# ScottHCL/recommend

Measured on AMD Instinct MI355X. Metric: ranked samples/sec (fwd+bwd) at B=4096 seq=128; AUC parity vs ref, higher is better.
Workload: dtype f32-emulated (fp16-pair / split-bf16); 1 GPU; C2: OneTrans 4L d128 H4 f512 L_NS12 L_S128 (seq 3x42), Criteo-shape 13 dense + 26 ids, replicated tables, fwd+bwd+optimizer; global_batch=4096, per_gpu_batch=4096, seq_len=128, parallelism=dp1

## Files before the change

### include/onetrans_hip.h

```cpp
#ifndef ONETRANS_HIP_H
#define ONETRANS_HIP_H

#include <stddef.h>
#include <stdint.h>

#ifdef __cplusplus
extern "C" {
#endif

#define OT_OK 0
#define OT_ERR_INVALID_ARG 1
#define OT_ERR_UNSUPPORTED 2
#define OT_ERR_HIP 3

#define OT_GEMM_NN 0
#define OT_GEMM_NT 1

#define OT_AX_NONE 0
#define OT_AX_RMSNORM 1
#define OT_AX_GELU 2
#define OT_AX_BF16 4
#define OT_AX_BF16_RMSNORM 5

#define OT_EPI_BIAS 1
#define OT_EPI_GELU_BWD 2
#define OT_EPI_GELU 4
#define OT_EPI_DROPOUT 8
#define OT_EPI_RESIDUAL 16
#define OT_EPI_ACCUMULATE 32
#define OT_EPI_ROW_RSTD 64
#define OT_EPI_ROWDOT 256
#define OT_EPI_RMSNORM_BWD 128
#define OT_EPI_C_BF16 512
#define OT_EPI_AUX_BF16 1024
#define OT_WG_D_BF16 8

int ot_version(void);
const char* ot_get_last_error_string(void);

int ot_gemm_tile_rows(void);
#define OT_MATMUL_F32 0
#define OT_MATMUL_SPLIT_BF16 1
#define OT_MATMUL_BF16 2
int ot_mixed_gemm(int mode, const float* A, int64_t lda, int K, const int32_t* in_rows,
                  int a_xform, const float* a_rstd, const float* a_gamma,
                  const float* W, int64_t w_gstride, int64_t ldw, int N,
                  const int32_t* tile_group, int ntiles,
                  const float* bias, int64_t bias_gstride,
                  float* C, int64_t ldc, const int32_t* out_rows, int epi,
                  const float* res, int64_t ldres, int res_tok,
                  const float* aux, int64_t ldaux,
                  uint32_t seed, uint32_t site, float drop_rate, int tail_K, int tail_I,
                  const int32_t* tail_pos, int precision, void* stream);
typedef struct ot_rms_epilogue {
  size_t struct_size;
  float* rstd_out; float eps;
  const float* x; int64_t ldx;
  const float* gamma; const float* rstd;
  const float* dres; int64_t lddres;
  int dres_tail_K, dres_tail_I;
  const int32_t* dres_tail_inv;
  float* dx_masked; int64_t lddxm;
  float* dgamma; int accumulate_dgamma;
  void* workspace; size_t ws_bytes;
  float* rowdot; int rowdot_n;
  uint16_t* gelu_out; int64_t ldgelu;
  uint16_t* xn_out; int64_t ldxn;
  uint16_t* c16_out; int64_t ldc16;
  float* rowmax_out; int rowmax_n;
  const float* a_rowmax; int a_rowmax_n;
  float* amax_out;
  float* rowabs_out; int rowabs_n;
} ot_rms_epilogue;
size_t ot_mixed_gemm_rms_workspace_size(int ntiles, int N);
int ot_mixed_gemm_rms(int mode, const float* A, int64_t lda, int K, const int32_t* in_rows,
                      int a_xform, const float* a_rstd, const float* a_gamma,
                      const float* W, int64_t w_gstride, int64_t ldw, int N,
                      const int32_t* tile_group, int ntiles,
                      const float* bias, int64_t bias_gstride,
                      float* C, int64_t ldc, const int32_t* out_rows, int epi,
                      const float* res, int64_t ldres, int res_tok,
                      const float* aux, int64_t ldaux,
                      uint32_t seed, uint32_t site, float drop_rate, int tail_K, int tail_I,
                      const int32_t* tail_pos, const ot_rms_epilogue* rms, int precision, void* stream);

size_t ot_wgrad_workspace_size(int nchunks, int K, int N);
int ot_mixed_gemm_wgrad(const float* A, int64_t lda, const int32_t* a_rows, int a_xform,
                        const float* a_rstd, const float* a_gamma,
                        const float* D, int64_t ldd, const int32_t* d_rows, int K, int N,
                        const int32_t* chunks, int nchunks, const int32_t* gchunk, int ngroups,
                        float* dW, int64_t dw_gstride, float* db, int64_t db_gstride,
                        int accumulate, void* workspace, size_t ws_bytes, int precision, void* stream);

int ot_mixed_gemm_wgrad_ex(const float* A, int64_t lda, const int32_t* a_rows, int a_xform,
                           const float* a_rstd, const float* a_gamma,
                           const float* D, int64_t ldd, const int32_t* d_rows, int K, int N,
                           const int32_t* chunks, int nchunks, const int32_t* gchunk, int ngroups,
                           float* dW, int64_t dw_gstride, float* db, int64_t db_gstride,
                           int accumulate, void* workspace, size_t ws_bytes, const float* a_bound,
                           const float* d_bound, int precision, void* stream);

int ot_transpose_banks(const float* src, float* dst, const int64_t* banks_dev, int nbanks, int64_t total_tiles,
                       void* stream);

size_t ot_split_image_elems(int G, int N, int K);
int ot_split_images(const float* base, const int64_t* desc_dev, int ndesc, int64_t total_units, uint16_t* img,
                    int precision, void* stream);
int ot_mixed_gemm_img(int mode, const float* A, int64_t lda, int K, const int32_t* in_rows,
                      int a_xform, const float* a_rstd, const float* a_gamma,
                      const float* W, int64_t w_gstride, int64_t ldw, int N,
                      const int32_t* tile_group, int ntiles,
                      const float* bias, int64_t bias_gstride,
                      float* C, int64_t ldc, const int32_t* out_rows, int epi,
                      const float* res, int64_t ldres, int res_tok,
                      const float* aux, int64_t ldaux,
                      uint32_t seed, uint32_t site, float drop_rate, int tail_K, int tail_I,
                      const int32_t* tail_pos, const uint16_t* b_image, int image_ntn, int image_tn0,
                      int precision, void* stream);
int ot_plane_wide(int on);
int ot_wgrad_wide(int on);
int ot_plane_rowmeta(int on);
int ot_plane_panel(int on);
int ot_plane_panel_launches(void);
int ot_mixed_gemm_rms_img(int mode, const float* A, int64_t lda, int K, const int32_t* in_rows,
                          int a_xform, const float* a_rstd, const float* a_gamma,
                          const float* W, int64_t w_gstride, int64_t ldw, int N,
                          const int32_t* tile_group, int ntiles,
                          const float* bias, int64_t bias_gstride,
                          float* C, int64_t ldc, const int32_t* out_rows, int epi,
                          const float* res, int64_t ldres, int res_tok,
                          const float* aux, int64_t ldaux,
                          uint32_t seed, uint32_t site, float drop_rate, int tail_K, int tail_I,
                          const int32_t* tail_pos, const ot_rms_epilogue* rms, const uint16_t* b_image,
                          int image_ntn, int image_tn0, int precision, void* stream);

typedef struct ot_ffn_fused_args {
  size_t struct_size;
  const float* x1; int64_t ldx1;
  const int32_t* rows;
  const int32_t* tile_group; int ntiles;
  const float* rstd;
  const uint16_t* w1_image; int w1_groups;
  const uint16_t* w2_image; int w2_groups;
  const float* b1; int64_t b1_gstride;
  const float* b2; int64_t b2_gstride;
  int f;
  float* u_out; int64_t ldu;
  float* u_amax;
  float* x2; int64_t ldx2;
  float* rstd_out; float eps;
  uint32_t seed, site; float drop_rate;
  int tail_K, tail_I; const int32_t* tail_pos;
} ot_ffn_fused_args;
int ot_ffn_fused_fwd(const ot_ffn_fused_args* args, void* stream);
int ot_ffn_fused(int on);

int ot_attn_fwd(const float* qkv, int64_t ld, int B, int H, int I, int K, const int32_t* qpos,
                int head_dim, float* out, float* lse, int precision, void* stream);
size_t ot_attn_fwd_fp8_workspace_size(int B, int H, int I, int head_dim);
int ot_attn_fwd_fp8(const float* qkv, int64_t ld, int B, int H, int I, int K, const int32_t* qpos,
                    int head_dim, float* out, float* lse, void* workspace, size_t ws_bytes, void* stream);
#define OT_FP8_DEQUANT 1
#define OT_FP8_TWO_TERM 2
int ot_attn_fwd_fp8_ex(float* qkv, int64_t ld, int B, int H, int I, int K, const int32_t* qpos, int head_dim,
                       float* out, float* lse, void* workspace, size_t ws_bytes, int flags, void* stream);
int ot_attn_fwd_fp8_deq16(const float* qkv, int64_t ld, int B, int H, int I, int K, const int32_t* qpos,
                          int head_dim, float* out, float* lse, void* workspace, size_t ws_bytes, int flags,
                          uint16_t* deq16, void* stream);
size_t ot_attn_bwd_workspace_size(int B, int H, int K);
int ot_attn_bwd(const float* qkv, int64_t ld, const float* out, const float* dout, const float* lse,
                int B, int H, int I, int K, const int32_t* qpos, int head_dim, float* dqkv, float* delta_ws,
                int precision, void* stream);
size_t ot_attn_bwd_ex_workspace_size(int B, int H, int I, int K, int head_dim, int selected, int precision);
int ot_attn_bwd_ex(const float* qkv, int64_t ld, const float* out, const float* dout, const float* lse,
                   int B, int H, int I, int K, const int32_t* qpos, int head_dim, float* dqkv, void* workspace,
                   size_t ws_bytes, int precision, void* stream);
#define OT_ATTN_DQKV_BF16 1
#define OT_ATTN_QKV_BF16 2
#define OT_ATTN_DQ_PART_BF16 4
int ot_attn_bwd_dqkv_bf16_supported(int I, int K, int head_dim, int selected, int precision);
int ot_attn_bwd_bf16_forms(int I, int K, int head_dim, int selected, int precision);
size_t ot_attn_bwd_flags_workspace_size(int B, int H, int I, int K, int head_dim, int selected, int flags, int precision);
int ot_attn_slice_supported(int I, int K, int head_dim, int selected);
int ot_attn_bwd_flags(const float* qkv, int64_t ld, const float* out, const float* dout, const float* lse,
                      int B, int H, int I, int K, const int32_t* qpos, int head_dim, void* dqkv, int flags,
                      void* workspace, size_t ws_bytes, int precision, void* stream);
int ot_attn_amax_supported(int I, int K, int head_dim, int selected, int precision);
int ot_attn_fwd_amax(const float* qkv, int64_t ld, int B, int H, int I, int K, const int32_t* qpos,
                     int head_dim, float* out, float* lse, float* amax, float* rowmax, int precision, void* stream);
int ot_attn_bwd_amax(const float* qkv, int64_t ld, const float* out, const float* dout, const float* lse,
                     int B, int H, int I, int K, const int32_t* qpos, int head_dim, float* dqkv,
                     void* workspace, size_t ws_bytes, float* amax, float* rowmax, int precision, void* stream);

int ot_attn_fwd_cached(const float* qkv, int64_t ld, const float* kv_cache, int64_t ldc, const int32_t* req,
                       int C, int H, int Ic, int n, int Kq, int head_dim, float* out, void* stream);

int ot_attn_fwd_cached_lse(const float* qkv, int64_t ld, const float* kv_cache, int64_t ldc, const int32_t* req,
                           int C, int H, int Ic, int n, int Kq, int head_dim, float* out, float* lse, void* stream);
size_t ot_attn_bwd_cached_workspace_size(int R, int C, int H, int Ic, int n, int Kq, int head_dim);
int ot_attn_bwd_cached(const float* qkv, int64_t ld, const float* kv_cache, int64_t ldc, const int32_t* req_start,
                       int R, int C, int H, int Ic, int n, int Kq, int head_dim, const float* out, const float* dout,
                       const float* lse, float* dqkv, float* dkv_cache, int accumulate, void* workspace,
                       size_t ws_bytes, void* stream);

int ot_attn_fwd_masked(const float* qkv, int64_t ld, int B, int H, int I, int K, const int32_t* qpos, int head_dim,
                       const uint8_t* key_valid, int64_t ldv, float* out, float* lse, int precision, void* stream);
int ot_attn_bwd_masked(const float* qkv, int64_t ld, const float* out, const float* dout, const float* lse, int B,
                       int H, int I, int K, const int32_t* qpos, int head_dim, const uint8_t* key_valid, int64_t ldv,
                       float* dqkv, float* delta_ws, int precision, void* stream);
int ot_attn_fwd_cached_masked(const float* qkv, int64_t ld, const float* kv_cache, int64_t ldc, const int32_t* req,
                              int C, int H, int Ic, int n, int Kq, int head_dim, const uint8_t* cache_valid,
                              int64_t ldcv, float* out, float* lse_or_null, void* stream);
int ot_seq_key_valid(const int32_t* lens, const int32_t* seq_len, const int32_t* seq_off, int nseq, int B, int L0,
                     const int32_t* rank, int64_t ldr, uint8_t* valid0, void* stream);

int ot_kv_pack_bf16(const float* qkv, int64_t ld, int R, int64_t rows_per_req, int d, uint16_t* kv16, int64_t ldc16,
                    int64_t req_stride, int64_t row0, void* stream);
int ot_attn_fwd_cached_kv16(const float* qkv, int64_t ld, const uint16_t* kv16, int64_t ldc16, int64_t req_stride,
                            const int32_t* req, int C, int H, int Ic, int n, int Kq, int head_dim,
                            const uint8_t* cache_valid, int64_t ldcv, float* out, float* lse_or_null, void* stream);

int ot_pyramid_select(const float* score, float score_sign, int B, int I, int K, int nforce,
                      int32_t* pos, int32_t* inv, int32_t* map_rows, int map_per_sample, void* stream);

int ot_rmsnorm_fwd(const float* x, int64_t ldx, const float* gamma, float* y, int64_t ldy, float* rstd,
                   int64_t rows, int d, float eps, void* stream);
size_t ot_rmsnorm_bwd_workspace_size(int64_t rows, int d);
int ot_rmsnorm_bwd(const float* dy, int64_t lddy, const float* x, int64_t ldx, const float* gamma,
                   const float* rstd, const float* dres, int64_t lddres, int dres_tail_K, int dres_tail_I,
                   const int32_t* dres_tail_inv, float* dx, int64_t lddx,
                   float* dx_masked, int64_t lddxm, uint32_t seed, uint32_t site, float drop_rate,
                   int tail_K, int tail_I, const int32_t* tail_pos, float* dgamma, int accumulate_dgamma, int64_t rows, int d,
                   void* workspace, size_t ws_bytes, void* stream);
int ot_dropout_apply(const float* src, int64_t lds, float* dst, int64_t ldd, int64_t rows, int d,
                     uint32_t seed, uint32_t site, float drop_rate, int tail_K, int tail_I,
                     const int32_t* tail_pos, void* stream);
int ot_dropout_rowmax_supported(int d);
int ot_dropout_apply_ex(const float* src, int64_t lds, float* dst, int64_t ldd, int64_t rows, int d,
                        uint32_t seed, uint32_t site, float drop_rate, int tail_K, int tail_I,
                        const int32_t* tail_pos, float* amax, float* rowmax, int rowmax_n, void* stream);
int ot_rows_absmax(const float* x, int64_t ldx, int64_t rows, int d, float* out, int parts, void* stream);
int ot_dropout_apply_bf16(const float* src, int64_t lds, uint16_t* dst, int64_t ldd, int64_t rows, int d,
                          uint32_t seed, uint32_t site, float drop_rate, int tail_K, int tail_I,
                          const int32_t* tail_pos, void* stream);
size_t ot_rows_colsum_workspace_size(int64_t nrows, int ncols);
int ot_rows_colsum(const float* src, int64_t ld, const int32_t* rows, int64_t nrows, int ncols,
                   float* out, int accumulate, void* workspace, size_t ws_bytes, void* stream);

typedef struct {
  const float* dense;
  const int64_t* ids;
  int64_t row_offset;
  int64_t stride;
  int col;
  int width;
} ot_ns_field;
int ot_ns_assemble(const ot_ns_field* fields_dev, int nfields, const float* table, int B, float* out,
                   int64_t ld_out, void* stream);
int ot_ns_grad_pack(const ot_ns_field* fields_dev, int nsparse, int width, const float* dmat, int64_t ld,
                    int B, int64_t* keys, float* grads, void* stream);
int ot_fill_rows(float* dst, int64_t ld, const int32_t* rows, int64_t nrows, const float* vec, int d,
                 void* stream);
int ot_seq_rows(const int64_t* ids, int64_t ids_stride_b, int B, int L, int64_t vocab, int32_t* in_rows,
                void* stream);
int ot_head_fwd(const float* pre1, const float* w2, const float* b2, int T, int B, int dh,
                float* logits, float* probs, void* stream);
size_t ot_head_bwd_workspace_size(int T, int B, int dh);
int ot_head_bwd(const float* pre1, const float* w2, const float* probs, const float* dprobs, int T, int B,
                int dh, float* dpre1, float* dw2, float* db2, int64_t task_stride_w2, int64_t task_stride_b2,
                int accumulate, void* workspace, size_t ws_bytes, void* stream);
int ot_head_bwd_ex(const float* pre1, const float* w2, const float* probs, const float* dprobs, const float* dlogits,
                   int T, int B, int dh, float* dpre1, float* dw2, float* db2, int64_t task_stride_w2,
                   int64_t task_stride_b2, int accumulate, void* workspace, size_t ws_bytes, void* stream);
int ot_task_loss_logits_fwd(const float* logits, const float* probs, const float* labels, int T, int B,
                            unsigned mse_mask, float* loss, void* workspace, size_t ws_bytes, void* stream);
int ot_task_loss_logits_bwd(const float* probs, const float* labels, const float* gscale, int T, int B,
                            unsigned mse_mask, float* dlogits, void* stream);
size_t ot_bce_workspace_size(int T, int B);
int ot_bce_fwd(const float* probs, const float* labels, int T, int B, float* loss, void* workspace,
               size_t ws_bytes, void* stream);
int ot_bce_bwd(const float* probs, const float* labels, const float* gscale, int T, int B, float* dprobs,
               void* stream);
int ot_task_loss_fwd(const float* probs, const float* labels, int T, int B, unsigned mse_mask, float* loss,
                     void* workspace, size_t ws_bytes, void* stream);
int ot_task_loss_bwd(const float* probs, const float* labels, const float* gscale, int T, int B,
                     unsigned mse_mask, float* dprobs, void* stream);

size_t ot_sparse_adagrad_workspace_size(int64_t n, int E);
int ot_sparse_adagrad(float* table, float* accum, int E, int64_t num_rows, const int64_t* keys,
                      const float* grads, int64_t n, float lr, float eps, float clip,
                      void* workspace, size_t ws_bytes, void* stream);
int ot_sparse_grad_dense(int E, int64_t num_rows, const int64_t* keys, const float* grads, int64_t n,
                         float* dense, void* workspace, size_t ws_bytes, void* stream);
size_t ot_dense_adagrad_workspace_size(void);
int ot_dense_adagrad(float* table, float* accum, const float* grad, int64_t num_rows, int E, float lr,
                     float eps, float clip, void* workspace, size_t ws_bytes, void* stream);
int ot_sparse_prepare(int E, int64_t num_rows, const int64_t* keys, const float* grads, int64_t n, float* sumsq_out,
                      void* workspace, size_t ws_bytes, void* stream);
int ot_sparse_finish(float* table, float* accum, int E, int64_t n, float lr, float eps, float clip,
                     const float* sumsq_total, void* workspace, size_t ws_bytes, void* stream);

size_t ot_shard_route_workspace_size(int64_t n);
int ot_shard_route(const int64_t* ids, int64_t n, int64_t num_rows, int world, int32_t* perm, int64_t* send_local,
                   int32_t* counts, void* workspace, size_t ws_bytes, void* stream);
size_t ot_shard_route_unique_workspace_size(int64_t n);
int ot_shard_route_unique(const int64_t* ids, int64_t n, int64_t num_rows, int world, int64_t* uniq_local,
                          int64_t* inv, int32_t* order, int32_t* run_start, int32_t* counts, void* workspace,
                          size_t ws_bytes, void* stream);
int ot_segment_rows_sum(const float* src, const int32_t* order, const int32_t* run_start, int64_t U, int E,
                        float* out, void* stream);
size_t ot_segment_rows_sum_workspace_size(int64_t U, int64_t n, int E);
int ot_segment_rows_sum_ex(const float* src, const int32_t* order, const int32_t* run_start, int64_t U, int64_t n,
                           int E, float* out, void* workspace, size_t ws_bytes, void* stream);
int ot_gather_rows(const float* table, int E, const int64_t* idx, int64_t n, float* out, void* stream);
int ot_permute_rows(const float* src, const int32_t* perm, int64_t n, int E, int inverse, float* dst, void* stream);
int ot_hash_uniform_rows(float* out, int64_t local_rows, int E, int rank, int world, uint32_t seed, float lo,
                         float hi, void* stream);

size_t ot_clip_rmsprop_workspace_size(int nseg, int64_t max_seg_elems);
int ot_clip_rmsprop(float* w, float* g, float* v, float* m, const int64_t* segs_dev, int nseg,
                    int64_t max_seg_elems, float lr, float rho, float eps, float momentum, float clip,
                    void* workspace, size_t ws_bytes, void* stream);
size_t ot_clip_adam_workspace_size(int nseg, int64_t max_seg_elems);
int ot_clip_adam(float* w, float* g, float* m, float* v, const int64_t* segs_dev, int nseg,
                 int64_t max_seg_elems, float lr, float beta1, float beta2, float eps, int64_t step, float clip,
                 void* workspace, size_t ws_bytes, void* stream);

size_t ot_metrics_workspace_size(int T, int B);
int ot_metrics_update(const float* probs, const float* labels, int T, int B, int64_t task_stride,
                      const double* bounds, int nb, int64_t* counts, double* sums, void* workspace,
                      size_t ws_bytes, void* stream);

size_t ot_grouped_auc_workspace_size(int T, int64_t n, int group_bits);
int ot_grouped_auc(const int64_t* groups, const float* scores, const float* labels, int T, int64_t n,
                   int64_t task_stride, int group_bits, uint32_t task_mask, double* agg,
                   int64_t* num_groups, int64_t* group_ids, int64_t* group_stats, void* workspace,
                   size_t ws_bytes, void* stream);

#define OT_RANK_SUM 0
#define OT_RANK_PRODUCT 1
size_t ot_rank_topk_workspace_size(int R, int64_t C, int K);
int ot_rank_topk(const float* probs, int64_t task_stride, int T, const float* weights_host, int mode,
                 const int32_t* req, int64_t C, int R, int K, int32_t* top_idx, float* top_score,
                 int32_t* count, float* fused_out, void* workspace, size_t ws_bytes, void* stream);

typedef struct {
  const int64_t* times;
  int64_t stride_b;
  int32_t L;
  int32_t map_off;
} ot_seq_time;
size_t ot_seq_time_rows_workspace_size(int B, int nseq, int L_S);
int ot_seq_time_rows(const ot_seq_time* seqs, int nseq, int B, int L_S, int64_t row_stride, int32_t* out_rows,
                     int32_t* rank_out, int64_t* last_time, void* workspace, size_t ws_bytes, void* stream);

#define OT_NS_BAG_MAX 32
#define OT_NS_BAG_MAX_WIDTH 256
#define OT_BAG_SUM 0
#define OT_BAG_MEAN 1
typedef struct {
  const float* table;
  const int64_t* ids;
  const float* weights;
  int64_t row_offset;
  int64_t num_rows;
  int64_t ids_stride;
  int64_t weights_stride;
  int32_t width;
  int32_t cap;
  int32_t col;
  int32_t pooling;
} ot_ns_bag;
int ot_ns_bag_pool(const ot_ns_bag* bags, int nbags, int B, float* out, int64_t ld_out, float* coef_out,
                   void* stream);
int ot_ns_bag_grad_pack(const ot_ns_bag* bags, int nbags, int B, const float* dmat, int64_t ld, const float* coef,
                        int64_t* keys, float* grads, void* stream);

#ifdef __cplusplus
}
#endif
#endif
```

### recommend_amd/_lib.py

```python

from __future__ import annotations

import ctypes
import os
from ctypes import c_float, c_int, c_int64, c_size_t, c_uint32, c_void_p, c_char_p

_HERE = os.path.dirname(os.path.abspath(__file__))
LIB_PATH = os.environ.get('ONETRANS_HIP_LIB') or os.path.join(_HERE, 'libonetrans_hip.so')
HEADER = os.path.join(os.path.dirname(_HERE), 'include', 'onetrans_hip.h')

OT_GEMM_NN, OT_GEMM_NT = 0, 1
OT_AX_NONE, OT_AX_RMSNORM, OT_AX_GELU, OT_AX_BF16, OT_AX_BF16_RMSNORM = 0, 1, 2, 4, 5
OT_EPI_BIAS, OT_EPI_GELU_BWD, OT_EPI_GELU = 1, 2, 4
OT_EPI_DROPOUT, OT_EPI_RESIDUAL, OT_EPI_ACCUMULATE = 8, 16, 32
OT_EPI_ROW_RSTD, OT_EPI_RMSNORM_BWD, OT_EPI_ROWDOT = 64, 128, 256
OT_EPI_C_BF16 = 512
OT_EPI_AUX_BF16 = 1024
OT_ATTN_DQKV_BF16 = 1
OT_ATTN_QKV_BF16 = 2
OT_ATTN_DQ_PART_BF16 = 4
OT_WG_D_BF16 = 8
OT_MATMUL_F32, OT_MATMUL_SPLIT_BF16, OT_MATMUL_BF16 = 0, 1, 2
OT_FP8_DEQUANT, OT_FP8_TWO_TERM = 1, 2
OT_RANK_SUM, OT_RANK_PRODUCT = 0, 1
RANK_MODES = {'sum': OT_RANK_SUM, 'product': OT_RANK_PRODUCT}
RANK_MAX_K = 1024
MATMUL_MODES = {'f32': OT_MATMUL_F32, 'split': OT_MATMUL_SPLIT_BF16, 'bf16': OT_MATMUL_BF16}


class RmsEpilogue(ctypes.Structure):
    _fields_ = [('struct_size', c_size_t), ('rstd_out', c_void_p), ('eps', c_float),
                ('x', c_void_p), ('ldx', c_int64), ('gamma', c_void_p), ('rstd', c_void_p),
                ('dres', c_void_p), ('lddres', c_int64), ('dres_tail_K', c_int), ('dres_tail_I', c_int),
                ('dres_tail_inv', c_void_p),
                ('dx_masked', c_void_p), ('lddxm', c_int64),
                ('dgamma', c_void_p), ('accumulate_dgamma', c_int),
                ('workspace', c_void_p), ('ws_bytes', c_size_t),
                ('rowdot', c_void_p), ('rowdot_n', c_int),
                ('gelu_out', c_void_p), ('ldgelu', c_int64),
                ('xn_out', c_void_p), ('ldxn', c_int64),
                ('c16_out', c_void_p), ('ldc16', c_int64),
                ('rowmax_out', c_void_p), ('rowmax_n', c_int),
                ('a_rowmax', c_void_p), ('a_rowmax_n', c_int),
                ('amax_out', c_void_p), ('rowabs_out', c_void_p), ('rowabs_n', c_int)]

class FfnFusedArgs(ctypes.Structure):
    _fields_ = [('struct_size', c_size_t), ('x1', c_void_p), ('ldx1', c_int64), ('rows', c_void_p),
                ('tile_group', c_void_p), ('ntiles', c_int), ('rstd', c_void_p),
                ('w1_image', c_void_p), ('w1_groups', c_int), ('w2_image', c_void_p), ('w2_groups', c_int),
                ('b1', c_void_p), ('b1_gstride', c_int64), ('b2', c_void_p), ('b2_gstride', c_int64),
                ('f', c_int), ('u_out', c_void_p), ('ldu', c_int64), ('u_amax', c_void_p),
                ('x2', c_void_p), ('ldx2', c_int64), ('rstd_out', c_void_p), ('eps', c_float),
                ('seed', c_uint32), ('site', c_uint32), ('drop_rate', c_float),
                ('tail_K', c_int), ('tail_I', c_int), ('tail_pos', c_void_p)]


class SeqTime(ctypes.Structure):
    _fields_ = [('times', c_void_p), ('stride_b', c_int64), ('L', ctypes.c_int32), ('map_off', ctypes.c_int32)]


class NsBag(ctypes.Structure):
    _fields_ = [('table', c_void_p), ('ids', c_void_p), ('weights', c_void_p), ('row_offset', c_int64),
                ('num_rows', c_int64), ('ids_stride', c_int64), ('weights_stride', c_int64),
                ('width', ctypes.c_int32), ('cap', ctypes.c_int32), ('col', ctypes.c_int32),
                ('pooling', ctypes.c_int32)]


OT_BAG_SUM, OT_BAG_MEAN = 0, 1
BAG_POOLINGS = {'sum': OT_BAG_SUM, 'mean': OT_BAG_MEAN}
NS_BAG_MAX = 32
NS_BAG_MAX_WIDTH = 256
SEQ_TIME_MAX_L = 4096
SEQ_TIME_MAX_SEQ = 32

P = c_void_p
I64 = c_int64

SIGNATURES = {
    'ot_version': (c_int, []),
    'ot_get_last_error_string': (c_char_p, []),
    'ot_gemm_tile_rows': (c_int, []),
    'ot_mixed_gemm': (c_int, [c_int, P, I64, c_int, P, c_int, P, P, P, I64, I64, c_int, P, c_int, P, I64,
                              P, I64, P, c_int, P, I64, c_int, P, I64, c_uint32, c_uint32, c_float, c_int,
                              c_int, P, c_int, P]),
    'ot_mixed_gemm_rms_workspace_size': (c_size_t, [c_int, c_int]),
    'ot_mixed_gemm_rms': (c_int, [c_int, P, I64, c_int, P, c_int, P, P, P, I64, I64, c_int, P, c_int, P, I64,
                                  P, I64, P, c_int, P, I64, c_int, P, I64, c_uint32, c_uint32, c_float, c_int,
                                  c_int, P, P, c_int, P]),
    'ot_wgrad_workspace_size': (c_size_t, [c_int, c_int, c_int]),
    'ot_mixed_gemm_wgrad': (c_int, [P, I64, P, c_int, P, P, P, I64, P, c_int, c_int, P, c_int, P, c_int, P,
                                    I64, P, I64, c_int, P, c_size_t, c_int, P]),
    'ot_mixed_gemm_wgrad_ex': (c_int, [P, I64, P, c_int, P, P, P, I64, P, c_int, c_int, P, c_int, P, c_int, P,
                                       I64, P, I64, c_int, P, c_size_t, P, P, c_int, P]),
    'ot_transpose_banks': (c_int, [P, P, P, c_int, I64, P]),
    'ot_mixed_gemm_img': (c_int, [c_int, P, I64, c_int, P, c_int, P, P, P, I64, I64, c_int, P, c_int, P, I64,
                                  P, I64, P, c_int, P, I64, c_int, P, I64, c_uint32, c_uint32, c_float, c_int,
                                  c_int, P, P, c_int, c_int, c_int, P]),
    'ot_mixed_gemm_rms_img': (c_int, [c_int, P, I64, c_int, P, c_int, P, P, P, I64, I64, c_int, P, c_int, P, I64,
                                      P, I64, P, c_int, P, I64, c_int, P, I64, c_uint32, c_uint32, c_float, c_int,
                                      c_int, P, P, P, c_int, c_int, c_int, P]),
    'ot_split_image_elems': (c_size_t, [c_int, c_int, c_int]),
    'ot_plane_wide': (c_int, [c_int]),
    'ot_wgrad_wide': (c_int, [c_int]),
    'ot_plane_rowmeta': (c_int, [c_int]),
    'ot_plane_panel': (c_int, [c_int]),
    'ot_plane_panel_launches': (c_int, []),
    'ot_ffn_fused_fwd': (c_int, [P, P]),
    'ot_ffn_fused': (c_int, [c_int]),
    'ot_split_images': (c_int, [P, P, c_int, I64, P, c_int, P]),
    'ot_attn_fwd': (c_int, [P, I64, c_int, c_int, c_int, c_int, P, c_int, P, P, c_int, P]),
    'ot_attn_fwd_fp8_workspace_size': (c_size_t, [c_int, c_int, c_int, c_int]),
    'ot_attn_fwd_fp8': (c_int, [P, I64, c_int, c_int, c_int, c_int, P, c_int, P, P, P, c_size_t, P]),
    'ot_attn_fwd_fp8_ex': (c_int, [P, I64, c_int, c_int, c_int, c_int, P, c_int, P, P, P, c_size_t, c_int, P]),
    'ot_attn_fwd_fp8_deq16': (c_int, [P, I64, c_int, c_int, c_int, c_int, P, c_int, P, P, P, c_size_t, c_int, P, P]),
    'ot_attn_bwd_workspace_size': (c_size_t, [c_int, c_int, c_int]),
    'ot_attn_bwd': (c_int, [P, I64, P, P, P, c_int, c_int, c_int, c_int, P, c_int, P, P, c_int, P]),
    'ot_attn_bwd_ex_workspace_size': (c_size_t, [c_int, c_int, c_int, c_int, c_int, c_int, c_int]),
    'ot_attn_bwd_ex': (c_int, [P, I64, P, P, P, c_int, c_int, c_int, c_int, P, c_int, P, P, c_size_t, c_int, P]),
    'ot_attn_bwd_dqkv_bf16_supported': (c_int, [c_int, c_int, c_int, c_int, c_int]),
    'ot_attn_bwd_bf16_forms': (c_int, [c_int, c_int, c_int, c_int, c_int]),
    'ot_attn_slice_supported': (c_int, [c_int, c_int, c_int, c_int]),
    'ot_attn_bwd_flags_workspace_size': (c_size_t, [c_int, c_int, c_int, c_int, c_int, c_int, c_int, c_int]),
    'ot_attn_bwd_flags': (c_int, [P, I64, P, P, P, c_int, c_int, c_int, c_int, P, c_int, P, c_int, P, c_size_t, c_int, P]),
    'ot_attn_fwd_cached': (c_int, [P, I64, P, I64, P, c_int, c_int, c_int, c_int, c_int, c_int, P, P]),
    'ot_attn_fwd_cached_lse': (c_int, [P, I64, P, I64, P, c_int, c_int, c_int, c_int, c_int, c_int, P, P, P]),
    'ot_attn_bwd_cached_workspace_size': (c_size_t, [c_int, c_int, c_int, c_int, c_int, c_int, c_int]),
    'ot_attn_bwd_cached': (c_int, [P, I64, P, I64, P, c_int, c_int, c_int, c_int, c_int, c_int, c_int, P, P, P, P, P,
                                   c_int, P, c_size_t, P]),
    'ot_attn_amax_supported': (c_int, [c_int, c_int, c_int, c_int, c_int]),
    'ot_attn_fwd_amax': (c_int, [P, I64, c_int, c_int, c_int, c_int, P, c_int, P, P, P, P, c_int, P]),
    'ot_attn_bwd_amax': (c_int, [P, I64, P, P, P, c_int, c_int, c_int, c_int, P, c_int, P, P, c_size_t, P, P, c_int,
                                 P]),
    'ot_pyramid_select': (c_int, [P, c_float, c_int, c_int, c_int, c_int, P, P, P, c_int, P]),
    'ot_rmsnorm_fwd': (c_int, [P, I64, P, P, I64, P, I64, c_int, c_float, P]),
    'ot_rmsnorm_bwd_workspace_size': (c_size_t, [I64, c_int]),
    'ot_rmsnorm_bwd': (c_int, [P, I64, P, I64, P, P, P, I64, c_int, c_int, P, P, I64, P, I64, c_uint32,
                               c_uint32, c_float, c_int, c_int, P, P, c_int, I64, c_int, P, c_size_t, P]),
    'ot_dropout_apply': (c_int, [P, I64, P, I64, I64, c_int, c_uint32, c_uint32, c_float, c_int, c_int, P, P]),
    'ot_dropout_apply_bf16': (c_int, [P, I64, P, I64, I64, c_int, c_uint32, c_uint32, c_float, c_int, c_int, P, P]),
    'ot_rows_absmax': (c_int, [P, I64, I64, c_int, P, c_int, P]),
    'ot_dropout_rowmax_supported': (c_int, [c_int]),
    'ot_dropout_apply_ex': (c_int, [P, I64, P, I64, I64, c_int, c_uint32, c_uint32, c_float, c_int, c_int, P, P, P,
                                    c_int, P]),
    'ot_rows_colsum_workspace_size': (c_size_t, [I64, c_int]),
    'ot_rows_colsum': (c_int, [P, I64, P, I64, c_int, P, c_int, P, c_size_t, P]),
    'ot_ns_assemble': (c_int, [P, c_int, P, c_int, P, I64, P]),
    'ot_ns_grad_pack': (c_int, [P, c_int, c_int, P, I64, c_int, P, P, P]),
    'ot_fill_rows': (c_int, [P, I64, P, I64, P, c_int, P]),
    'ot_seq_rows': (c_int, [P, I64, c_int, c_int, I64, P, P]),
    'ot_head_fwd': (c_int, [P, P, P, c_int, c_int, c_int, P, P, P]),
    'ot_head_bwd_workspace_size': (c_size_t, [c_int, c_int, c_int]),
    'ot_head_bwd': (c_int, [P, P, P, P, c_int, c_int, c_int, P, P, P, I64, I64, c_int, P, c_size_t, P]),
    'ot_bce_workspace_size': (c_size_t, [c_int, c_int]),
    'ot_bce_fwd': (c_int, [P, P, c_int, c_int, P, P, c_size_t, P]),
    'ot_bce_bwd': (c_int, [P, P, P, c_int, c_int, P, P]),
    'ot_task_loss_fwd': (c_int, [P, P, c_int, c_int, c_uint32, P, P, c_size_t, P]),
    'ot_task_loss_bwd': (c_int, [P, P, P, c_int, c_int, c_uint32, P, P]),
    'ot_task_loss_logits_fwd': (c_int, [P, P, P, c_int, c_int, c_uint32, P, P, c_size_t, P]),
    'ot_task_loss_logits_bwd': (c_int, [P, P, P, c_int, c_int, c_uint32, P, P]),
    'ot_head_bwd_ex': (c_int, [P, P, P, P, P, c_int, c_int, c_int, P, P, P, I64, I64, c_int, P, c_size_t, P]),
    'ot_sparse_adagrad_workspace_size': (c_size_t, [I64, c_int]),
    'ot_sparse_adagrad': (c_int, [P, P, c_int, I64, P, P, I64, c_float, c_float, c_float, P, c_size_t, P]),
    'ot_sparse_grad_dense': (c_int, [c_int, I64, P, P, I64, P, P, c_size_t, P]),
    'ot_dense_adagrad_workspace_size': (c_size_t, []),
    'ot_dense_adagrad': (c_int, [P, P, P, I64, c_int, c_float, c_float, c_float, P, c_size_t, P]),
    'ot_sparse_prepare': (c_int, [c_int, I64, P, P, I64, P, P, c_size_t, P]),
    'ot_sparse_finish': (c_int, [P, P, c_int, I64, c_float, c_float, c_float, P, P, c_size_t, P]),
    'ot_shard_route_workspace_size': (c_size_t, [I64]),
    'ot_shard_route': (c_int, [P, I64, I64, c_int, P, P, P, P, c_size_t, P]),
    'ot_shard_route_unique_workspace_size': (c_size_t, [I64]),
    'ot_shard_route_unique': (c_int, [P, I64, I64, c_int, P, P, P, P, P, P, c_size_t, P]),
    'ot_segment_rows_sum': (c_int, [P, P, P, I64, c_int, P, P]),
    'ot_segment_rows_sum_workspace_size': (c_size_t, [I64, I64, c_int]),
    'ot_segment_rows_sum_ex': (c_int, [P, P, P, I64, I64, c_int, P, P, c_size_t, P]),
    'ot_gather_rows': (c_int, [P, c_int, P, I64, P, P]),
    'ot_permute_rows': (c_int, [P, P, I64, c_int, c_int, P, P]),
    'ot_hash_uniform_rows': (c_int, [P, I64, c_int, c_int, c_int, c_uint32, c_float, c_float, P]),
    'ot_clip_rmsprop_workspace_size': (c_size_t, [c_int, I64]),
    'ot_clip_rmsprop': (c_int, [P, P, P, P, P, c_int, I64, c_float, c_float, c_float, c_float, c_float, P,
                                c_size_t, P]),
    'ot_clip_adam_workspace_size': (c_size_t, [c_int, I64]),
    'ot_clip_adam': (c_int, [P, P, P, P, P, c_int, I64, c_float, c_float, c_float, c_float, I64, c_float, P,
                             c_size_t, P]),
    'ot_metrics_workspace_size': (c_size_t, [c_int, c_int]),
    'ot_metrics_update': (c_int, [P, P, c_int, c_int, I64, P, c_int, P, P, P, c_size_t, P]),
    'ot_grouped_auc_workspace_size': (c_size_t, [c_int, I64, c_int]),
    'ot_grouped_auc': (c_int, [P, P, P, c_int, I64, I64, c_int, c_uint32, P, P, P, P, P, c_size_t, P]),
    'ot_rank_topk_workspace_size': (c_size_t, [c_int, I64, c_int]),
    'ot_rank_topk': (c_int, [P, I64, c_int, P, c_int, P, I64, c_int, c_int, P, P, P, P, P, c_size_t, P]),
    'ot_seq_time_rows_workspace_size': (c_size_t, [c_int, c_int, c_int]),
    'ot_seq_time_rows': (c_int, [P, c_int, c_int, c_int, I64, P, P, P, P, c_size_t, P]),
    'ot_attn_fwd_masked': (c_int, [P, I64, c_int, c_int, c_int, c_int, P, c_int, P, I64, P, P, c_int, P]),
    'ot_attn_bwd_masked': (c_int, [P, I64, P, P, P, c_int, c_int, c_int, c_int, P, c_int, P, I64, P, P, c_int, P]),
    'ot_attn_fwd_cached_masked': (c_int, [P, I64, P, I64, P, c_int, c_int, c_int, c_int, c_int, c_int, P, I64, P, P,
                                          P]),
    'ot_seq_key_valid': (c_int, [P, P, P, c_int, c_int, c_int, P, I64, P, P]),
    'ot_kv_pack_bf16': (c_int, [P, I64, c_int, I64, c_int, P, I64, I64, I64, P]),
    'ot_attn_fwd_cached_kv16': (c_int, [P, I64, P, I64, I64, P, c_int, c_int, c_int, c_int, c_int, c_int, P, I64, P, P,
                                        P]),
    'ot_ns_bag_pool': (c_int, [P, c_int, c_int, P, I64, P, P]),
    'ot_ns_bag_grad_pack': (c_int, [P, c_int, c_int, P, I64, P, P, P, P]),
}

NS_FIELD_BYTES = 40

_lib = None


class OneTransHipError(RuntimeError):
    pass


def load():
    global _lib
    if _lib is not None:
        return _lib
    if not os.path.exists(LIB_PATH):
        raise OneTransHipError(
            f'{LIB_PATH} not found: build it with `python -c "import __graft_entry__ as g; g.build()"` '
            '(there is no CPU fallback)')
    lib = ctypes.CDLL(LIB_PATH)
    for name, (res, args) in SIGNATURES.items():
        fn = getattr(lib, name)
        fn.restype = res
        fn.argtypes = args
    _lib = lib
    return lib


def call(name: str, *args) -> None:
    lib = load()
    rc = getattr(lib, name)(*args)
    if rc != 0:
        msg = lib.ot_get_last_error_string()
        raise OneTransHipError(f'{name} failed ({rc}): {msg.decode() if msg else ""}')


def size(name: str, *args) -> int:
    return int(getattr(load(), name)(*args))


def header_symbols() -> list:
    import re
    txt = open(HEADER).read()
    return sorted(set(re.findall(r'\b(ot_[a-z0-9_]+)\s*\(', txt)))
```

### recommend_amd/kernels.py

```python

from __future__ import annotations

import contextlib
import ctypes
import functools
import os
import threading
from typing import Optional, Tuple, Union

import torch

from . import _lib
from ._lib import call, size

Ptrish = Union[None, torch.Tensor, Tuple[torch.Tensor, int]]


class Probe:

    def __init__(self):
        self.recs = []

    def begin(self):
        ev = torch.cuda.Event(enable_timing=True)
        ev.record()
        return ev

    def end(self, family: str, flops: float, ev0, label: str = '', nbytes: float = 0.0, terms: int = 0) -> None:
        ev1 = torch.cuda.Event(enable_timing=True)
        ev1.record()
        self.recs.append((family, flops, ev0, ev1, label, nbytes, terms))

    def by_label(self, steps: int):
        torch.cuda.synchronize()
        agg = {}
        for rec in self.recs:
            f, fl, a, b, lab = rec[:5]
            d = agg.setdefault(f'{f} {lab}', [0, 0.0, 0.0])
            d[0] += 1
            d[1] += a.elapsed_time(b)
            d[2] += fl
        return {k: (n / steps, 1e3 * ms / n, fl / (ms * 1e-3) / 1e12 if ms > 0 else 0.0)
                for k, (n, ms, fl) in agg.items()}

    def report(self, steps: int, mfma_peak_tflops: float = 0.0, hbm_peak_gbs: float = 0.0, terms_peak=None):
        if torch.cuda.is_available():
            torch.cuda.synchronize()
        fam = {}
        for rec in self.recs:
            f, fl, a, b, _, nb = rec[:6]
            terms = rec[6] if len(rec) > 6 else 0
            d = fam.setdefault(f, {'ms': 0.0, 'flops': 0.0, 'bytes': 0.0, 'n': 0, 'floor': 0.0, 'fl_mfma': 0.0,
                                   'fl_hbm': 0.0, 'mfma_ms': 0.0, 'pair': 0})
            d['ms'] += a.elapsed_time(b)
            d['flops'] += fl
            d['bytes'] += nb
            d['n'] += 1
            d['pair'] += terms == 3
            if mfma_peak_tflops > 0 and hbm_peak_gbs > 0:
                pk = terms_peak(terms) if (terms_peak is not None and terms) else mfma_peak_tflops
                tm, th = fl / (pk * 1e9), nb / (hbm_peak_gbs * 1e6)
                d['mfma_ms'] += tm
                d['floor'] += max(tm, th)
                d['fl_mfma' if tm >= th else 'fl_hbm'] += max(tm, th)
        out = {}
        for f, d in fam.items():
            out[f] = {'ms_per_step': d['ms'] / steps, 'avg_us': 1e3 * d['ms'] / d['n'],
                      'launches_per_step': d['n'] / steps, 'gflop_per_launch': d['flops'] / d['n'] / 1e9,
                      'gbyte_per_launch': d['bytes'] / d['n'] / 1e9,
                      'tflops': d['flops'] / (d['ms'] * 1e-3) / 1e12 if d['ms'] > 0 else 0.0,
                      'gbs': d['bytes'] / (d['ms'] * 1e-3) / 1e9 if d['ms'] > 0 else 0.0,
                      'floor_ms_per_step': d['floor'] / steps, 'floor_mfma_ms_per_step': d['fl_mfma'] / steps,
                      'floor_hbm_ms_per_step': d['fl_hbm'] / steps,
                      'mfma_peak_eff': d['flops'] / (d['mfma_ms'] * 1e9) if d['mfma_ms'] > 0 else 0.0,
                      'pair_launches_per_step': d['pair'] / steps}
        return {'families': out}


_probe = None


def _terms(bimg, a_xform: int, a_rowmax, N: int) -> int:
    mm = matmul_mode()
    if mm != 'split':
        return 1 if mm == 'bf16' else 0
    pair = bimg is not None and N % 128 == 0 and (
        a_xform == _lib.OT_AX_RMSNORM or (a_rowmax is not None and a_xform in (_lib.OT_AX_NONE, _lib.OT_AX_GELU)))
    return 3 if pair else 6


def gemm_bytes(M: int, K: int, N: int, a_xform: int, epi: int) -> float:
    mn = (1 + bool(epi & _lib.OT_EPI_RESIDUAL) + bool(epi & _lib.OT_EPI_GELU_BWD)
          + bool(epi & _lib.OT_EPI_ACCUMULATE))
    a_bytes = 2.0 if a_xform in (_lib.OT_AX_BF16, _lib.OT_AX_BF16_RMSNORM) else 4.0
    c_less = 2.0 * M * N if epi & _lib.OT_EPI_C_BF16 else 0.0
    return a_bytes * M * K + 4.0 * M * (a_xform == _lib.OT_AX_RMSNORM) + 4.0 * M * N * mn - c_less


def set_probe(p) -> None:
    global _probe
    _probe = p


_default_mode = os.environ.get('ONETRANS_MATMUL', 'split')
if _default_mode not in _lib.MATMUL_MODES:
    raise _lib.OneTransHipError(f'ONETRANS_MATMUL={_default_mode!r}: expected one of {sorted(_lib.MATMUL_MODES)}')
_scope = threading.local()


def set_matmul_mode(mode: str) -> str:
    global _default_mode
    if mode not in _lib.MATMUL_MODES:
        raise ValueError(f'matmul mode {mode!r}: expected one of {sorted(_lib.MATMUL_MODES)}')
    old, _default_mode = _default_mode, mode
    return old


def matmul_mode() -> str:
    st = getattr(_scope, 'stack', None)
    return st[-1] if st else _default_mode


@contextlib.contextmanager
def precision(mode: str):
    if mode not in _lib.MATMUL_MODES:
        raise ValueError(f'matmul mode {mode!r}: expected one of {sorted(_lib.MATMUL_MODES)}')
    st = getattr(_scope, 'stack', None)
    if st is None:
        st = _scope.stack = []
    st.append(mode)
    try:
        yield
    finally:
        st.pop()


def _prec() -> int:
    return _lib.MATMUL_MODES[matmul_mode()]


def precision_owner(obj):
    if isinstance(getattr(obj, 'matmul', None), str):
        return obj
    owner = getattr(type(obj), 'precision_model', None)
    if owner is None:
        raise TypeError(f'{type(obj).__name__}: in_model_precision needs a .matmul mode or a precision_model property')
    owner = owner.__get__(obj)
    if not isinstance(getattr(owner, 'matmul', None), str):
        raise TypeError(f'{type(obj).__name__}.precision_model has no matmul mode')
    return owner


def in_model_precision(fn):
    @functools.wraps(fn)
    def wrapped(self, *args, **kw):
        with precision(precision_owner(self).matmul):
            return fn(self, *args, **kw)
    return wrapped


def ptr(x: Ptrish):
    if x is None:
        return None
    if isinstance(x, tuple):
        t, off = x
        return t.data_ptr() + off * t.element_size()
    return x.data_ptr()


def _sel(tail):
    return ptr(tail[2]) if len(tail) > 2 and tail[2] is not None else None


def pyramid_select(B: int, I: int, K: int, pos: torch.Tensor, inv: Optional[torch.Tensor] = None,
                   score: Optional[torch.Tensor] = None, sign: float = 1.0, nforce: int = 0,
                   map_rows: Optional[torch.Tensor] = None, map_per_sample: int = 0) -> None:
    ev = _probe.begin() if _probe is not None else None
    call('ot_pyramid_select', ptr(score), float(sign), B, I, K, nforce, ptr(pos), ptr(inv), ptr(map_rows),
         map_per_sample, stream())
    if ev is not None:
        _probe.end('pyramid', 0.0, ev)


def stream() -> int:
    return torch.cuda.current_stream().cuda_stream


def workspace(nbytes: int, device) -> torch.Tensor:
    return torch.empty(max(int(nbytes), 16), dtype=torch.uint8, device=device)


def gemm(mode: int, A: Ptrish, lda: int, K: int, in_rows: Ptrish, W: Ptrish, w_gstride: int, ldw: int, N: int,
         tile_group: Ptrish, ntiles: int, C: Ptrish, ldc: int, out_rows: Ptrish, *, a_xform: int = 0,
         rstd: Ptrish = None, gamma: Ptrish = None, bias: Ptrish = None, bias_gstride: int = 0, epi: int = 0,
         res: Ptrish = None, ldres: int = 0, res_tok: int = 0, aux: Ptrish = None, ldaux: int = 0,
         seed: int = 0, site: int = 0, drop: float = 0.0, tail: Tuple[int, int] = (1, 1),
         m_rows: int = 0, bimg=None) -> None:
    ev = _probe.begin() if _probe is not None else None
    args = (mode, ptr(A), lda, K, ptr(in_rows), a_xform, ptr(rstd), ptr(gamma), ptr(W), w_gstride,
            ldw, N, ptr(tile_group), ntiles, ptr(bias), bias_gstride, ptr(C), ldc, ptr(out_rows), epi, ptr(res),
            ldres, res_tok, ptr(aux), ldaux, seed & 0xFFFFFFFF, site, float(drop), tail[0], tail[1], _sel(tail))
    if bimg is not None:
        call('ot_mixed_gemm_img', *args, ptr(bimg[0]), bimg[1], bimg[2], _prec(), stream())
    else:
        call('ot_mixed_gemm', *args, _prec(), stream())
    if ev is not None:
        M = m_rows or ntiles * 128
        _probe.end('mixed_gemm', 2.0 * M * K * N, ev, f'gemm mode{mode} ax{a_xform} epi{epi} M{M} K{K} N{N}',
                   gemm_bytes(M, K, N, a_xform, epi), _terms(bimg, a_xform, None, N))


def gemm_rms(mode: int, A: Ptrish, lda: int, K: int, in_rows: Ptrish, W: Ptrish, w_gstride: int, ldw: int,
             N: int, tile_group: Ptrish, ntiles: int, C: Ptrish, ldc: int, out_rows: Ptrish, *, epi: int,
             a_xform: int = 0, rstd: Ptrish = None, gamma: Ptrish = None, bias: Ptrish = None,
             bias_gstride: int = 0, res: Ptrish = None, ldres: int = 0, res_tok: int = 0, seed: int = 0,
             site: int = 0, drop: float = 0.0, tail: Tuple[int, int] = (1, 1), m_rows: int = 0,
             rstd_out: Ptrish = None, eps: float = 1e-6, nx: Ptrish = None, ldnx: int = 0,
             ngamma: Ptrish = None, nrstd: Ptrish = None, dres: Ptrish = None, lddres: int = 0,
             dres_tail: Tuple[int, int] = (0, 0), dx_masked: Ptrish = None, lddxm: int = 0,
             dgamma: Ptrish = None, accumulate_dgamma: bool = False, device=None, bimg=None,
             aux: Ptrish = None, ldaux: int = 0, rowdot: Ptrish = None, rowdot_n: int = 0,
             gelu_out: Ptrish = None, ldgelu: int = 0, xn_out: Ptrish = None, ldxn: int = 0,
             c16_out: Ptrish = None, ldc16: int = 0, rowmax_out: Ptrish = None, rowmax_n: int = 0,
             a_rowmax: Ptrish = None, a_rowmax_n: int = 0, amax_out: Ptrish = None, rowabs_out: Ptrish = None,
             rowabs_n: int = 0) -> None:
    need_ws = dgamma is not None or (rstd_out is not None and N > 128)
    ws = workspace(size('ot_mixed_gemm_rms_workspace_size', ntiles, N) if need_ws else 16,
                   device if device is not None else (C[0] if isinstance(C, tuple) else C).device)
    e = _lib.RmsEpilogue(ctypes.sizeof(_lib.RmsEpilogue), ptr(rstd_out), float(eps), ptr(nx), ldnx, ptr(ngamma), ptr(nrstd), ptr(dres), lddres,
                         dres_tail[0], dres_tail[1], _sel(dres_tail), ptr(dx_masked), lddxm, ptr(dgamma),
                         int(accumulate_dgamma), ptr(ws), ws.numel(), ptr(rowdot), int(rowdot_n),
                         ptr(gelu_out), int(ldgelu), ptr(xn_out), int(ldxn), ptr(c16_out), int(ldc16),
                         ptr(rowmax_out), int(rowmax_n), ptr(a_rowmax), int(a_rowmax_n), ptr(amax_out),
                         ptr(rowabs_out), int(rowabs_n))
    ev = _probe.begin() if _probe is not None else None
    args = (mode, ptr(A), lda, K, ptr(in_rows), a_xform, ptr(rstd), ptr(gamma), ptr(W),
            w_gstride, ldw, N, ptr(tile_group), ntiles, ptr(bias), bias_gstride, ptr(C), ldc, ptr(out_rows), epi,
            ptr(res), ldres, res_tok, ptr(aux), ldaux, seed & 0xFFFFFFFF, site, float(drop), tail[0], tail[1],
            _sel(tail), ctypes.byref(e))
    if bimg is not None:
        call('ot_mixed_gemm_rms_img', *args, ptr(bimg[0]), bimg[1], bimg[2], _prec(), stream())
    else:
        call('ot_mixed_gemm_rms', *args, _prec(), stream())
    if ev is not None:
        M = m_rows or ntiles * 128
        extra = (nx is not None) + (dres is not None) + (dx_masked is not None)
        _probe.end('mixed_gemm', 2.0 * M * K * N, ev, f'gemm_rms mode{mode} ax{a_xform} epi{epi} M{M} K{K} N{N}',
                   gemm_bytes(M, K, N, a_xform, epi) + 4.0 * M * N * extra + 2.0 * M * N * (gelu_out is not None)
                   + 2.0 * M * K * (xn_out is not None)
                   + 4.0 * M * ((rstd_out is not None) + (nrstd is not None)), _terms(bimg, a_xform, a_rowmax, N))


def wgrad(A: Ptrish, lda: int, a_rows: Ptrish, D: Ptrish, ldd: int, d_rows: Ptrish, K: int, N: int, rmap_dev,
          nchunks: int, ngroups: int, dW: Ptrish, dw_gstride: int, db: Ptrish = None, db_gstride: int = 0, *,
          a_xform: int = 0, rstd: Ptrish = None, gamma: Ptrish = None, accumulate: bool = False,
          device=None, m_rows: int = 0, rowmap=None, a_bound: Ptrish = None, d_bound: Ptrish = None) -> None:
    if rowmap is not None and rowmap.group_rows:
        tiles = ((K + 127) // 128) * ((N + 127) // 128)
        ch, gc, nchunks = rowmap.chunks_for(tiles, device)
        rmap_dev = {'chunks': ch, 'gchunk': gc}
    nbytes = size('ot_wgrad_workspace_size', nchunks, K, N)
    ws = workspace(nbytes, device)
    ev = _probe.begin() if _probe is not None else None
    call('ot_mixed_gemm_wgrad_ex', ptr(A), lda, ptr(a_rows), a_xform, ptr(rstd), ptr(gamma), ptr(D), ldd,
         ptr(d_rows), K, N, ptr(rmap_dev['chunks']), nchunks, ptr(rmap_dev['gchunk']), ngroups, ptr(dW),
         dw_gstride, ptr(db), db_gstride, int(accumulate), ptr(ws), ws.numel(), ptr(a_bound), ptr(d_bound), _prec(),
         stream())
    if ev is not None:
        ax = a_xform & ~_lib.OT_WG_D_BF16
        wterms = {'bf16': 1, 'f32': 0}.get(matmul_mode(), 3 if (
            d_bound is not None and not (a_xform & _lib.OT_WG_D_BF16)
            and (ax == _lib.OT_AX_RMSNORM or (a_bound is not None and ax in (_lib.OT_AX_NONE, _lib.OT_AX_GELU))))
            else 6)
        _probe.end('mixed_gemm', 2.0 * m_rows * K * N, ev, f'wgrad ax{a_xform} M{m_rows} K{K} N{N} ch{nchunks}',
                   (2.0 if (a_xform & ~_lib.OT_WG_D_BF16) == _lib.OT_AX_BF16 else 4.0) * m_rows * K
                   + (2.0 if a_xform & _lib.OT_WG_D_BF16 else 4.0) * m_rows * N
                   + 4.0 * m_rows * ((a_xform & ~_lib.OT_WG_D_BF16) == _lib.OT_AX_RMSNORM) + 4.0 * ngroups * K * N,
                   wterms)


def transpose_banks(src, dst, banks_dev, nbanks, total_tiles) -> None:
    call('ot_transpose_banks', ptr(src), ptr(dst), ptr(banks_dev), nbanks, total_tiles, stream())


def split_image_elems(G: int, N: int, K: int) -> int:
    return int(_lib.load().ot_split_image_elems(G, N, K))


def plane_wide(on: int = -1) -> int:
    return _lib.size('ot_plane_wide', int(on))


def wgrad_wide(on: int = -1) -> int:
    return _lib.size('ot_wgrad_wide', int(on))


def plane_rowmeta(on: int = -1) -> int:
    return _lib.size('ot_plane_rowmeta', int(on))


def plane_panel(on: int = -1) -> int:
    return _lib.size('ot_plane_panel', int(on))


def plane_panel_launches() -> int:
    return _lib.size('ot_plane_panel_launches')


def ffn_fused(on: int = -1) -> int:
    return _lib.size('ot_ffn_fused', int(on))


FFN_FUSED_MAX_F = 1024


def ffn_fused_fwd(x1: Ptrish, ldx1: int, rows: Ptrish, tile_group: Ptrish, ntiles: int, rstd: Ptrish, w1_image,
                  w1_groups: int, w2_image, w2_groups: int, b1: Ptrish, b1_gstride: int, b2: Ptrish, b2_gstride: int,
                  f: int, x2: Ptrish, ldx2: int, *, u_out: Ptrish = None, ldu: int = 0, u_amax: Ptrish = None,
                  rstd_out: Ptrish = None, eps: float = 1e-6, seed: int = 0, site: int = 0, drop: float = 0.0,
                  tail: Tuple[int, int] = (1, 1), m_rows: int = 0) -> None:
    a = _lib.FfnFusedArgs(ctypes.sizeof(_lib.FfnFusedArgs), ptr(x1), ldx1, ptr(rows), ptr(tile_group), ntiles,
                          ptr(rstd), ptr(w1_image), int(w1_groups), ptr(w2_image), int(w2_groups), ptr(b1),
                          b1_gstride, ptr(b2), b2_gstride, f, ptr(u_out), ldu, ptr(u_amax), ptr(x2), ldx2,
                          ptr(rstd_out), float(eps), seed & 0xFFFFFFFF, site, float(drop), tail[0], tail[1],
                          _sel(tail))
    ev = _probe.begin() if _probe is not None else None
    call('ot_ffn_fused_fwd', ctypes.byref(a), stream())
    if ev is not None:
        M = m_rows or ntiles * 128
        _probe.end('mixed_gemm', 2.0 * M * 128 * f * 2, ev, f'ffn_fused M{M} f{f} u{int(u_out is not None)}',
                   4.0 * M * 128 * 3 + 4.0 * M * f * (u_out is not None)
                   + 4.0 * M * (1 + (rstd_out is not None)), 3)


def split_images(base, desc_dev, ndesc, total_units, img) -> None:
    call('ot_split_images', ptr(base), ptr(desc_dev), ndesc, total_units, ptr(img), _prec(), stream())


def attn_fwd(qkv: torch.Tensor, ld: int, B: int, H: int, I: int, K: int, hd: int, out: torch.Tensor,
             lse: torch.Tensor, qpos: Optional[torch.Tensor] = None, fp8: bool = False,
             dequant: bool = False, fp8_terms: int = 1, deq16: Optional[torch.Tensor] = None,
             amax: Optional[torch.Tensor] = None, rowmax: Optional[torch.Tensor] = None) -> None:
    if fp8 and fp8_terms not in (1, 2):
        raise ValueError(f'fp8_terms {fp8_terms}: 1 or 2')
    ws = None
    if fp8:
        ws = workspace(size('ot_attn_fwd_fp8_workspace_size', B, H, I, hd), qkv.device)
    ev = _probe.begin() if _probe is not None else None
    if fp8 and deq16 is not None:
        call('ot_attn_fwd_fp8_deq16', ptr(qkv), ld, B, H, I, K, ptr(qpos), hd, ptr(out), ptr(lse), ptr(ws),
             ws.numel(), _lib.OT_FP8_TWO_TERM if fp8_terms == 2 else 0, ptr(deq16), stream())
    elif fp8:
        call('ot_attn_fwd_fp8_ex', ptr(qkv), ld, B, H, I, K, ptr(qpos), hd, ptr(out), ptr(lse), ptr(ws),
             ws.numel(), (_lib.OT_FP8_DEQUANT if dequant else 0) | (_lib.OT_FP8_TWO_TERM if fp8_terms == 2 else 0),
             stream())
    elif amax is not None or rowmax is not None:
        call('ot_attn_fwd_amax', ptr(qkv), ld, B, H, I, K, ptr(qpos), hd, ptr(out), ptr(lse), ptr(amax), ptr(rowmax),
             _prec(), stream())
    else:
        call('ot_attn_fwd', ptr(qkv), ld, B, H, I, K, ptr(qpos), hd, ptr(out), ptr(lse), _prec(), stream())
    if ev is not None:
        _probe.end('attention', 4.0 * (K * I - K * (K - 1) / 2) * hd * H * B, ev,
                   f'fwd{"_fp8" if fp8 else ""} I{I} K{K} hd{hd}')


def attn_bwd_bf16_forms(I, K, hd, qpos=None) -> int:
    return int(_lib.load().ot_attn_bwd_bf16_forms(I, K, hd, int(qpos is not None), _prec()))


def attn_bwd_bf16_supported(I, K, hd, qpos=None) -> bool:
    return bool(_lib.load().ot_attn_bwd_dqkv_bf16_supported(I, K, hd, int(qpos is not None), _prec()))


def attn_amax_supported(I, K, hd, qpos=None, backward: bool = False) -> bool:
    return bool(_lib.load().ot_attn_amax_supported(I, K, hd, int(qpos is not None), _prec()) & (2 if backward else 1))


def attn_bwd(qkv, ld, out, dout, lse, B, H, I, K, hd, dqkv, qpos=None, dq_part_bf16: bool = False,
             amax=None, rowmax=None) -> None:
    flags = ((_lib.OT_ATTN_DQKV_BF16 if dqkv.dtype == torch.int16 else 0)
             | (_lib.OT_ATTN_QKV_BF16 if qkv.dtype == torch.int16 else 0)
             | (_lib.OT_ATTN_DQ_PART_BF16 if dq_part_bf16 and dqkv.dtype == torch.int16
                and attn_bwd_bf16_forms(I, K, hd, qpos) & _lib.OT_ATTN_DQ_PART_BF16 else 0))
    ws = workspace(size('ot_attn_bwd_flags_workspace_size', B, H, I, K, hd, int(qpos is not None), flags, _prec()),
                   qkv.device)
    ev = _probe.begin() if _probe is not None else None
    if amax is not None or rowmax is not None:
        call('ot_attn_bwd_amax', ptr(qkv), ld, ptr(out), ptr(dout), ptr(lse), B, H, I, K, ptr(qpos), hd, ptr(dqkv),
             ptr(ws), ws.numel(), ptr(amax), ptr(rowmax), _prec(), stream())
    else:
        call('ot_attn_bwd_flags', ptr(qkv), ld, ptr(out), ptr(dout), ptr(lse), B, H, I, K, ptr(qpos), hd,
             ptr(dqkv), flags, ptr(ws), ws.numel(), _prec(), stream())
    if ev is not None:
        _probe.end('attention', 8.0 * (K * I - K * (K - 1) / 2) * hd * H * B, ev, f'bwd I{I} K{K} hd{hd}')


def _valid_arg(valid):
    t, off, ldv = valid
    if t.dtype != torch.uint8:
        raise TypeError(f'key_valid: uint8 expected, got {t.dtype}')
    return ptr((t, off)), ldv


def attn_fwd_masked(qkv, ld, B, H, I, K, hd, out, lse, key_valid, qpos=None) -> None:
    kv, ldv = _valid_arg(key_valid)
    ev = _probe.begin() if _probe is not None else None
    call('ot_attn_fwd_masked', ptr(qkv), ld, B, H, I, K, ptr(qpos), hd, kv, ldv, ptr(out), ptr(lse), _prec(),
         stream())
    if ev is not None:
        _probe.end('attention', 4.0 * (K * I - K * (K - 1) / 2) * hd * H * B, ev, f'fwd_masked I{I} K{K} hd{hd}')


def attn_bwd_masked(qkv, ld, out, dout, lse, B, H, I, K, hd, dqkv, key_valid, qpos=None) -> None:
    kv, ldv = _valid_arg(key_valid)
    ws = workspace(size('ot_attn_bwd_workspace_size', B, H, K), qkv.device)
    ev = _probe.begin() if _probe is not None else None
    call('ot_attn_bwd_masked', ptr(qkv), ld, ptr(out), ptr(dout), ptr(lse), B, H, I, K, ptr(qpos), hd, kv, ldv,
         ptr(dqkv), ptr(ws), _prec(), stream())
    if ev is not None:
        _probe.end('attention', 8.0 * (K * I - K * (K - 1) / 2) * hd * H * B, ev, f'bwd_masked I{I} K{K} hd{hd}')


def attn_fwd_cached_masked(qkv, ld, kv_cache, ldc, req, C, H, Ic, n, Kq, hd, out, cache_valid, lse=None) -> None:
    cv, ldcv = _valid_arg(cache_valid) if cache_valid is not None else (None, 0)
    ev = _probe.begin() if _probe is not None else None
    call('ot_attn_fwd_cached_masked', ptr(qkv), ld, ptr(kv_cache), ldc, ptr(req), C, H, Ic, n, Kq, hd, cv, ldcv,
         ptr(out), ptr(lse), stream())
    if ev is not None:
        _probe.end('attention', 4.0 * (Kq * (Ic + n) - Kq * (Kq - 1) / 2) * hd * H * C, ev,
                   f'fwd_cached_masked Ic{Ic} n{n} K{Kq} hd{hd}')


def kv_pack_bf16(qkv, ld, R, rows_per_req, d, kv16, ldc16, req_stride, row0) -> None:
    if kv16.dtype != torch.bfloat16:
        raise TypeError(f'kv_pack_bf16: a bfloat16 cache is expected, got {kv16.dtype}')
    ev = _probe.begin() if _probe is not None else None
    call('ot_kv_pack_bf16', ptr(qkv), ld, R, rows_per_req, d, ptr(kv16), ldc16, req_stride, row0, stream())
    if ev is not None:
        _probe.end('rowwise', 0.0, ev, f'kv_pack_bf16 R{R} rows{rows_per_req} d{d}')


def attn_fwd_cached_kv16(qkv, ld, kv16, ldc16, req_stride, req, C, H, Ic, n, Kq, hd, out, cache_valid=None,
                         lse=None) -> None:
    if kv16 is not None and kv16.dtype != torch.bfloat16:
        raise TypeError(f'attn_fwd_cached_kv16: a bfloat16 cache is expected, got {kv16.dtype}')
    cv, ldcv = _valid_arg(cache_valid) if cache_valid is not None else (None, 0)
    ev = _probe.begin() if _probe is not None else None
    call('ot_attn_fwd_cached_kv16', ptr(qkv), ld, ptr(kv16), ldc16, req_stride, ptr(req), C, H, Ic, n, Kq, hd, cv,
         ldcv, ptr(out), ptr(lse), stream())
    if ev is not None:
        _probe.end('attention', 4.0 * (Kq * (Ic + n) - Kq * (Kq - 1) / 2) * hd * H * C, ev,
                   f'fwd_cached_kv16 Ic{Ic} n{n} K{Kq} hd{hd}')


def seq_key_valid(lens, seq_len, seq_off, B: int, L0: int, valid0, rank=None) -> None:
    n = len(seq_len)
    arr = ctypes.c_int32 * max(1, n)
    sl, so = arr(*seq_len), arr(*seq_off)
    call('ot_seq_key_valid', ptr(lens), ctypes.cast(sl, ctypes.c_void_p), ctypes.cast(so, ctypes.c_void_p), n, B, L0,
         ptr(rank),
         rank.shape[1] if rank is not None else 0, ptr(valid0), stream())


def attn_fwd_cached(qkv, ld, kv_cache, ldc, req, C, H, Ic, n, Kq, hd, out, lse=None) -> None:
    ev = _probe.begin() if _probe is not None else None
    args = (ptr(qkv), ld, ptr(kv_cache), ldc, ptr(req), C, H, Ic, n, Kq, hd, ptr(out))
    if lse is None:
        call('ot_attn_fwd_cached', *args, stream())
    else:
        call('ot_attn_fwd_cached_lse', *args, ptr(lse), stream())
    if ev is not None:
        _probe.end('attention', 4.0 * (Kq * (Ic + n) - Kq * (Kq - 1) / 2) * hd * H * C, ev,
                   f'fwd_cached{"" if lse is None else "_lse"} Ic{Ic} n{n} K{Kq} hd{hd}')


attn_fwd_cached_lse = attn_fwd_cached


def attn_bwd_cached(qkv, ld, kv_cache, ldc, req_start, R, C, H, Ic, n, Kq, hd, out, dout, lse, dqkv, dkv_cache,
                    accumulate: bool = False) -> None:
    ws = workspace(size('ot_attn_bwd_cached_workspace_size', R, C, H, Ic, n, Kq, hd), qkv.device)
    ev = _probe.begin() if _probe is not None else None
    call('ot_attn_bwd_cached', ptr(qkv), ld, ptr(kv_cache), ldc, ptr(req_start), R, C, H, Ic, n, Kq, hd, ptr(out),
         ptr(dout), ptr(lse), ptr(dqkv), ptr(dkv_cache), int(bool(accumulate)), ptr(ws), ws.numel(), stream())
    if ev is not None:
        _probe.end('attention', (8.0 * (Kq * n - Kq * (Kq - 1) / 2) + 14.0 * Kq * Ic) * hd * H * C, ev,
                   f'bwd_cached Ic{Ic} n{n} K{Kq} hd{hd}')


def rmsnorm_fwd(x: Ptrish, ldx: int, rows: int, d: int, rstd: Ptrish, gamma: Ptrish = None, y: Ptrish = None,
                ldy: int = 0, eps: float = 1e-6) -> None:
    ev = _probe.begin() if _probe is not None else None
    call('ot_rmsnorm_fwd', ptr(x), ldx, ptr(gamma), ptr(y), ldy, ptr(rstd), rows, d, eps, stream())
    if ev is not None:
        _probe.end('rowwise', 0.0, ev)


def rmsnorm_bwd(dy: Ptrish, lddy: int, x: Ptrish, ldx: int, gamma: Ptrish, rstd: Ptrish, dx: Ptrish, lddx: int,
                rows: int, d: int, *, dres: Ptrish = None, lddres: int = 0, dres_tail=(0, 0), dx_masked: Ptrish = None,
                lddxm: int = 0, seed: int = 0, site: int = 0, drop: float = 0.0, tail=(1, 1),
                dgamma: Ptrish = None, accumulate: bool = False, device=None) -> None:
    nbytes = size('ot_rmsnorm_bwd_workspace_size', rows, d) if dgamma is not None else 16
    ws = workspace(nbytes, device)
    ev = _probe.begin() if _probe is not None else None
    call('ot_rmsnorm_bwd', ptr(dy), lddy, ptr(x), ldx, ptr(gamma), ptr(rstd), ptr(dres), lddres, dres_tail[0],
         dres_tail[1], _sel(dres_tail), ptr(dx), lddx, ptr(dx_masked), lddxm, seed & 0xFFFFFFFF, site, float(drop),
         tail[0], tail[1], _sel(tail), ptr(dgamma), int(accumulate), rows, d, ptr(ws), ws.numel(), stream())
    if ev is not None:
        _probe.end('rowwise', 0.0, ev)


def dropout_apply(src, lds, dst, ldd, rows, d, seed, site, drop, tail, amax=None, rowmax=None) -> None:
    ev = _probe.begin() if _probe is not None else None
    if amax is not None or rowmax is not None:
        call('ot_dropout_apply_ex', ptr(src), lds, ptr(dst), ldd, rows, d, seed & 0xFFFFFFFF, site, float(drop),
             tail[0], tail[1], _sel(tail), ptr(amax), ptr(rowmax), (d + 255) // 256 if rowmax is not None else 0,
             stream())
    else:
        fn = 'ot_dropout_apply_bf16' if getattr(dst, 'dtype', None) == torch.int16 else 'ot_dropout_apply'
        call(fn, ptr(src), lds, ptr(dst), ldd, rows, d, seed & 0xFFFFFFFF, site, float(drop), tail[0],
             tail[1], _sel(tail), stream())
    if ev is not None:
        _probe.end('rowwise', 0.0, ev)


def dropout_rowmax_supported(d: int) -> bool:
    return bool(_lib.load().ot_dropout_rowmax_supported(d))


def rows_absmax(x, ldx, rows, d, out) -> None:
    ev = _probe.begin() if _probe is not None else None
    call('ot_rows_absmax', ptr(x), ldx, rows, d, ptr(out), (d + 255) // 256, stream())
    if ev is not None:
        _probe.end('rowwise', 0.0, ev)


def rows_colsum(src, ld, rows: Ptrish, nrows: int, ncols: int, out: Ptrish, accumulate=False, device=None) -> None:
    ws = workspace(size('ot_rows_colsum_workspace_size', nrows, ncols), device)
    ev = _probe.begin() if _probe is not None else None
    call('ot_rows_colsum', ptr(src), ld, ptr(rows), nrows, ncols, ptr(out), int(accumulate), ptr(ws), ws.numel(),
         stream())
    if ev is not None:
        _probe.end('rowwise', 0.0, ev)


def ns_assemble(fields_dev, nfields, table, B, out, ld_out) -> None:
    ev = _probe.begin() if _probe is not None else None
    call('ot_ns_assemble', ptr(fields_dev), nfields, ptr(table), B, ptr(out), ld_out, stream())
    if ev is not None:
        _probe.end('embedding', 0.0, ev)


def ns_grad_pack(fields_dev, nsparse, width, dmat, ld, B, keys, grads) -> None:
    ev = _probe.begin() if _probe is not None else None
    call('ot_ns_grad_pack', ptr(fields_dev), nsparse, width, ptr(dmat), ld, B, ptr(keys), ptr(grads), stream())
    if ev is not None:
        _probe.end('embedding', 0.0, ev)


def fill_rows(dst, ld, rows, nrows, vec, d) -> None:
    ev = _probe.begin() if _probe is not None else None
    call('ot_fill_rows', ptr(dst), ld, ptr(rows), nrows, ptr(vec), d, stream())
    if ev is not None:
        _probe.end('embedding', 0.0, ev)


def seq_rows(ids, stride_b, B, L, vocab, in_rows) -> None:
    ev = _probe.begin() if _probe is not None else None
    call('ot_seq_rows', ptr(ids), stride_b, B, L, vocab, ptr(in_rows), stream())
    if ev is not None:
        _probe.end('embedding', 0.0, ev)


def head_fwd(pre1, w2, b2, T, B, dh, logits, probs) -> None:
    ev = _probe.begin() if _probe is not None else None
    call('ot_head_fwd', ptr(pre1), ptr(w2), ptr(b2), T, B, dh, ptr(logits), ptr(probs), stream())
    if ev is not None:
        _probe.end('head_loss', 0.0, ev)


def head_bwd(pre1, w2, probs, dprobs, T, B, dh, dpre1, dw2, db2, sw2, sb2, accumulate=False, device=None,
             dlogits=None) -> None:
    ws = workspace(size('ot_head_bwd_workspace_size', T, B, dh), device)
    ev = _probe.begin() if _probe is not None else None
    call('ot_head_bwd_ex', ptr(pre1), ptr(w2), ptr(probs), ptr(dprobs), ptr(dlogits), T, B, dh, ptr(dpre1), ptr(dw2),
         ptr(db2), sw2, sb2, int(accumulate), ptr(ws), ws.numel(), stream())
    if ev is not None:
        _probe.end('head_loss', 0.0, ev)


def bce_fwd(probs, labels, T, B, loss, device=None, mse_mask: int = 0) -> None:
    ws = workspace(size('ot_bce_workspace_size', T, B), device)
    ev = _probe.begin() if _probe is not None else None
    call('ot_task_loss_fwd', ptr(probs), ptr(labels), T, B, mse_mask, ptr(loss), ptr(ws), ws.numel(), stream())
    if ev is not None:
        _probe.end('head_loss', 0.0, ev)


def bce_bwd(probs, labels, gscale, T, B, dprobs, mse_mask: int = 0) -> None:
    ev = _probe.begin() if _probe is not None else None
    call('ot_task_loss_bwd', ptr(probs), ptr(labels), ptr(gscale), T, B, mse_mask, ptr(dprobs), stream())
    if ev is not None:
        _probe.end('head_loss', 0.0, ev)


def metrics_update(probs, labels, T, B, task_stride, bounds, nb, counts, sums, device=None) -> None:
    ws = workspace(size('ot_metrics_workspace_size', T, B), device)
    ev = _probe.begin() if _probe is not None else None
    call('ot_metrics_update', ptr(probs), ptr(labels), T, B, task_stride, ptr(bounds), nb, ptr(counts), ptr(sums),
         ptr(ws), ws.numel(), stream())
    if ev is not None:
        _probe.end('metrics', 0.0, ev)


def grouped_auc(groups, scores, labels, T, n, task_stride, group_bits, task_mask, agg, num_groups, group_ids=None,
                group_stats=None, device=None) -> None:
    ws = workspace(size('ot_grouped_auc_workspace_size', T, n, group_bits), device)
    ev = _probe.begin() if _probe is not None else None
    call('ot_grouped_auc', ptr(groups), ptr(scores), ptr(labels), T, n, task_stride, group_bits, task_mask, ptr(agg),
         ptr(num_groups), ptr(group_ids), ptr(group_stats), ptr(ws), ws.numel(), stream())
    if ev is not None:
        _probe.end('grouped_auc', 0.0, ev)


def rank_topk(probs, task_stride, T, weights, mode, req, C, R, K, top_idx, top_score, count, fused_out=None,
              device=None) -> None:
    if mode not in _lib.RANK_MODES:
        raise ValueError(f'rank mode {mode!r}: expected one of {sorted(_lib.RANK_MODES)}')
    if len(weights) != T:
        raise ValueError(f'rank_topk: {len(weights)} weights for {T} tasks')
    wts = (ctypes.c_float * max(T, 1))(*[float(w) for w in weights])
    ws = workspace(size('ot_rank_topk_workspace_size', R, C, K), device)
    ev = _probe.begin() if _probe is not None else None
    call('ot_rank_topk', ptr(probs), task_stride, T, wts, _lib.RANK_MODES[mode], ptr(req), C, R, K, ptr(top_idx),
         ptr(top_score), ptr(count), ptr(fused_out), ptr(ws), ws.numel(), stream())
    if ev is not None:
        _probe.end('rank', 0.0, ev)


def ns_bag_descs(bags):
    arr = (_lib.NsBag * max(1, len(bags)))()
    for k, b in enumerate(bags):
        arr[k] = _lib.NsBag(ptr(b['table']), ptr(b['ids']), ptr(b.get('weights')), int(b['row_offset']),
                            int(b['num_rows']), int(b['ids_stride']), int(b.get('weights_stride', 0)),
                            int(b['width']), int(b['cap']), int(b['col']), _lib.BAG_POOLINGS[b['pooling']])
    return arr


def _bag_slice(descs, first: int, nbags: int):
    return ctypes.cast(ctypes.byref(descs, first * ctypes.sizeof(_lib.NsBag)), ctypes.c_void_p) if nbags else None


def ns_bag_pool(descs, nbags: int, B: int, out, ld_out: int, coef_out, first: int = 0) -> None:
    ev = _probe.begin() if _probe is not None else None
    call('ot_ns_bag_pool', _bag_slice(descs, first, nbags), nbags, B, ptr(out), ld_out, ptr(coef_out), stream())
    if ev is not None:
        _probe.end('embedding', 0.0, ev)


def ns_bag_grad_pack(descs, nbags: int, B: int, dmat, ld: int, coef, keys, grads, first: int = 0) -> None:
    ev = _probe.begin() if _probe is not None else None
    call('ot_ns_bag_grad_pack', _bag_slice(descs, first, nbags), nbags, B, ptr(dmat), ld, ptr(coef), ptr(keys),
         ptr(grads), stream())
    if ev is not None:
        _probe.end('embedding', 0.0, ev)


def seq_time_descs(seqs):
    arr = (_lib.SeqTime * max(1, len(seqs)))()
    for k, (t, stride_b, L, off) in enumerate(seqs):
        arr[k] = _lib.SeqTime(ptr(t), int(stride_b), int(L), int(off))
    return arr


def seq_time_rows(descs, nseq: int, B: int, L_S: int, row_stride: int, out_rows, rank_out=None, last_time=None,
                  device=None) -> None:
    ws = workspace(size('ot_seq_time_rows_workspace_size', B, nseq, L_S), device)
    ev = _probe.begin() if _probe is not None else None
    call('ot_seq_time_rows', ctypes.cast(descs, ctypes.c_void_p), nseq, B, L_S, row_stride, ptr(out_rows),
         ptr(rank_out), ptr(last_time), ptr(ws), ws.numel(), stream())
    if ev is not None:
        _probe.end('embedding', 0.0, ev)


def task_loss_logits_fwd(logits, probs, labels, T, B, loss, device=None, mse_mask: int = 0) -> None:
    ws = workspace(size('ot_bce_workspace_size', T, B), device)
    ev = _probe.begin() if _probe is not None else None
    call('ot_task_loss_logits_fwd', ptr(logits), ptr(probs), ptr(labels), T, B, mse_mask, ptr(loss), ptr(ws),
         ws.numel(), stream())
    if ev is not None:
        _probe.end('head_loss', 0.0, ev)


def task_loss_logits_bwd(probs, labels, gscale, T, B, dlogits, mse_mask: int = 0) -> None:
    ev = _probe.begin() if _probe is not None else None
    call('ot_task_loss_logits_bwd', ptr(probs), ptr(labels), ptr(gscale), T, B, mse_mask, ptr(dlogits), stream())
    if ev is not None:
        _probe.end('head_loss', 0.0, ev)


def sparse_adagrad(table, accum, E, num_rows, keys, grads, n, lr, eps, clip, device=None) -> None:
    ws = workspace(size('ot_sparse_adagrad_workspace_size', n, E), device)
    ev = _probe.begin() if _probe is not None else None
    call('ot_sparse_adagrad', ptr(table), ptr(accum), E, num_rows, ptr(keys), ptr(grads), n, float(lr), float(eps),
         float(clip), ptr(ws), ws.numel(), stream())
    if ev is not None:
        _probe.end('embedding', 0.0, ev)


def sparse_grad_dense(E, num_rows, keys, grads, n, dense, device=None) -> None:
    ws = workspace(size('ot_sparse_adagrad_workspace_size', n, E), device)
    ev = _probe.begin() if _probe is not None else None
    call('ot_sparse_grad_dense', E, num_rows, ptr(keys), ptr(grads), n, ptr(dense), ptr(ws), ws.numel(), stream())
    if ev is not None:
        _probe.end('embedding', 0.0, ev)


def dense_adagrad(table, accum, grad, num_rows, E, lr, eps, clip, device=None) -> None:
    ws = workspace(size('ot_dense_adagrad_workspace_size'), device)
    ev = _probe.begin() if _probe is not None else None
    call('ot_dense_adagrad', ptr(table), ptr(accum), ptr(grad), num_rows, E, float(lr), float(eps), float(clip),
         ptr(ws), ws.numel(), stream())
    if ev is not None:
        _probe.end('embedding', 0.0, ev)


def sparse_prepare(E, num_rows, keys, grads, n, sumsq_out, ws) -> None:
    call('ot_sparse_prepare', E, num_rows, ptr(keys), ptr(grads), n, ptr(sumsq_out), ptr(ws), ws.numel(), stream())


def sparse_finish(table, accum, E, n, lr, eps, clip, sumsq_total, ws) -> None:
    call('ot_sparse_finish', ptr(table), ptr(accum), E, n, float(lr), float(eps), float(clip), ptr(sumsq_total),
         ptr(ws), ws.numel(), stream())


def sparse_workspace(n, E, device):
    return workspace(size('ot_sparse_adagrad_workspace_size', n, E), device)


def shard_route(ids, n, num_rows, world, perm, send_local, counts) -> None:
    ws = workspace(size('ot_shard_route_workspace_size', n), ids.device)
    call('ot_shard_route', ptr(ids), n, num_rows, world, ptr(perm), ptr(send_local), ptr(counts), ptr(ws), ws.numel(),
         stream())


def shard_route_unique(ids, n, num_rows, world, uniq_local, inv, order, run_start, counts) -> None:
    ws = workspace(size('ot_shard_route_unique_workspace_size', n), ids.device)
    call('ot_shard_route_unique', ptr(ids), n, num_rows, world, ptr(uniq_local), ptr(inv), ptr(order), ptr(run_start),
         ptr(counts), ptr(ws), ws.numel(), stream())


def segment_rows_sum(src, order, run_start, U, E, out, n: Optional[int] = None) -> None:
    n = int(src.shape[0]) if n is None else int(n)
    n = max(n, int(U))
    ws = workspace(size('ot_segment_rows_sum_workspace_size', U, n, E), src.device)
    call('ot_segment_rows_sum_ex', ptr(src), ptr(order), ptr(run_start), U, n, E, ptr(out), ptr(ws), ws.numel(),
         stream())


def gather_rows(table, E, idx, n, out) -> None:
    call('ot_gather_rows', ptr(table), E, ptr(idx), n, ptr(out), stream())


def permute_rows(src, perm, n, E, inverse, dst) -> None:
    call('ot_permute_rows', ptr(src), ptr(perm), n, E, int(inverse), ptr(dst), stream())


def hash_uniform_rows(out, local_rows, E, rank, world, seed, lo, hi) -> None:
    call('ot_hash_uniform_rows', ptr(out), local_rows, E, rank, world, seed & 0xFFFFFFFF, float(lo), float(hi),
         stream())


def clip_rmsprop(w, g, v, m, segs_dev, nseg, max_seg, lr, rho, eps, momentum, clip, device=None) -> None:
    ws = workspace(size('ot_clip_rmsprop_workspace_size', nseg, max_seg), device)
    ev = _probe.begin() if _probe is not None else None
    call('ot_clip_rmsprop', ptr(w), ptr(g), ptr(v), ptr(m), ptr(segs_dev), nseg, max_seg, float(lr), float(rho),
         float(eps), float(momentum), float(clip), ptr(ws), ws.numel(), stream())
    if ev is not None:
        _probe.end('optimizer', 0.0, ev)


def clip_adam(w, g, m, v, segs_dev, nseg, max_seg, lr, beta1, beta2, eps, step, clip, device=None) -> None:
    ws = workspace(size('ot_clip_adam_workspace_size', nseg, max_seg), device)
    ev = _probe.begin() if _probe is not None else None
    call('ot_clip_adam', ptr(w), ptr(g), ptr(m), ptr(v), ptr(segs_dev), nseg, max_seg, float(lr), float(beta1),
         float(beta2), float(eps), int(step), float(clip), ptr(ws), ws.numel(), stream())
    if ev is not None:
        _probe.end('optimizer', 0.0, ev)
```

### recommend_amd/layout.py

```python

from __future__ import annotations

import os
from typing import Callable, Dict, List, Sequence, Tuple

import numpy as np

from .config import OneTransConfig
from .params import dense_param_shapes, keras_variables

TILE = 128
ALIGN = 64
IMAGE_UNIT_ELEMS = 3 * TILE * 16
_SLOTS_ENV = os.environ.get('ONETRANS_WGRAD_SLOTS')
WGRAD_SLOTS = int(_SLOTS_ENV) if _SLOTS_ENV else 1536
WGRAD_SLOTS_SMALL = int(_SLOTS_ENV) if _SLOTS_ENV else 512
WGRAD_SLOTS_LARGE = int(_SLOTS_ENV) if _SLOTS_ENV else 4096


def wgrad_slots(tiles_per_chunk: int) -> int:
    if tiles_per_chunk >= 32:
        return WGRAD_SLOTS_LARGE
    return WGRAD_SLOTS if tiles_per_chunk >= 8 else WGRAD_SLOTS_SMALL


def round_up(x: int, m: int) -> int:
    return (x + m - 1) // m * m


class FlatLayout:

    def __init__(self, cfg: OneTransConfig, f_ns: int, pair_dgrad: bool = False):
        self.f_ns, self.pair_dgrad = f_ns, pair_dgrad
        self.f_pad = max(4, round_up(f_ns, 4))
        self.shapes = dense_param_shapes(cfg, self.f_pad)
        self.offsets: Dict[str, int] = {}
        off = 0
        for name, shp in self.shapes.items():
            self.offsets[name] = off
            off += round_up(int(np.prod(shp)), ALIGN)
        self.total = off
        segs = []
        for (bank, eoff, rows, cols, stride) in keras_variables(cfg, self.shapes, f_ns=f_ns):
            segs.append((self.offsets[bank] + eoff, rows, cols, stride))
        self.segments = np.array(segs, dtype=np.int64)
        self.max_seg_elems = int((self.segments[:, 1] * self.segments[:, 2]).max())
        d, f, T = cfg.hidden_dim, cfg.ffn_dim, len(cfg.tasks)
        nseq = len(cfg.feature_config['sequence_features'])
        self.gemm_banks = {'tok.ns.kernel': (1, self.f_pad, cfg.num_ns_tokens * d),
                           'tok.seq.kernel': (nseq, cfg.seq_feature_dim, d),
                           'head.w1': (T, d, d // 2)}
        for l in range(cfg.num_layers):
            G = cfg.num_groups
            self.gemm_banks.update({f'blk.{l}.wqkv': (G, d, 3 * d), f'blk.{l}.wo': (1, d, d),
                                    f'blk.{l}.w1': (G, d, f), f'blk.{l}.w2': (G, f, d)})
        recs, tiles = [], 0
        for name, (G, K, N) in self.gemm_banks.items():
            o = self.offsets[name]
            recs.append((o, o, G, K, N, tiles))
            tiles += G * ((K + 31) // 32) * ((N + 31) // 32)
        self.transpose_desc = np.array(recs, dtype=np.int64)
        self.transpose_tiles = tiles
        self.images: Dict[Tuple[str, str], Tuple[int, int, int, int]] = {}
        irecs, units, ioff = [], 0, 0
        self.pair_images = set()
        for name, (G, K, N) in self.gemm_banks.items():
            o = self.offsets[name]
            gamma = None
            if name.endswith('.wqkv'):
                gamma = self.offsets[name[:-len('wqkv')] + 'norm1']
            elif name.endswith('.w1') and name.startswith('blk.'):
                gamma = self.offsets[name[:-len('w1')] + 'norm2']
            for orient, (Nb, Kb, sn, sk) in (('fwd', (N, K, 1, N)), ('dgrad', (K, N, N, 1))):
                if Nb % TILE or Kb % 16:
                    continue
                nu = G * (Nb // TILE) * (Kb // 16)
                pair_w2 = (orient == 'fwd' and name.endswith('.w2') and name.startswith('blk.')
                           and K % TILE == 0 and N % 16 == 0)
                pair_dg = pair_dgrad and name.startswith('blk.') and (
                    (orient == 'dgrad' and name.endswith(('.w1', '.w2', '.wo', '.wqkv')))
                    or (orient == 'fwd' and name.endswith('.wo')))
                kscale = gamma if (orient == 'fwd' and gamma is not None) else (-2 if (pair_w2 or pair_dg) else -1)
                irecs.append((o, sn, sk, K * N, kscale, ioff, units, G, Nb, Kb))
                self.images[(name, orient)] = (ioff, G, Nb, Kb)
                if kscale != -1:
                    self.pair_images.add((name, orient))
                units += nu
                ioff += nu * IMAGE_UNIT_ELEMS
        self.image_desc = np.array(irecs, dtype=np.int64).reshape(-1, 10)
        self.image_units = units
        self.image_elems = ioff

    def tview(self, flatT, name):
        off = self.offsets[name]
        G, K, N = self.gemm_banks[name]
        return flatT[off:off + G * K * N]

    def view(self, flat, name):
        off = self.offsets[name]
        n = int(np.prod(self.shapes[name]))
        return flat[off:off + n].view(self.shapes[name])


class RowMap:

    def __init__(self, rows: List[np.ndarray], tile_group: np.ndarray, chunks: np.ndarray,
                 gchunk: np.ndarray, nrows: int, group_rows=None):
        self.group_rows = list(group_rows) if group_rows is not None else []
        self._chunk_cache = {}
        self.rows = rows
        self.tile_group = tile_group
        self.chunks = chunks
        self.gchunk = gchunk
        self.ntiles = len(tile_group)
        self.nrows = nrows
        self.dev = None

    def to(self, device):
        import torch
        if self.dev is None:
            self.dev = {
                'rows': [torch.from_numpy(r).to(device) for r in self.rows],
                'tile_group': torch.from_numpy(self.tile_group).to(device),
                'chunks': torch.from_numpy(self.chunks).to(device),
                'gchunk': torch.from_numpy(self.gchunk).to(device),
            }
        return self.dev

    def chunks_for(self, tiles_per_chunk: int, device):
        import torch
        key = (tiles_per_chunk, str(device))
        if key not in self._chunk_cache:
            padded = [round_up(n, TILE) for n in self.group_rows]
            ng = sum(1 for p in padded if p > 0)
            if tiles_per_chunk < 8:
                budget = max(ng, wgrad_slots(tiles_per_chunk) // max(1, tiles_per_chunk))
            else:
                budget = max(1, wgrad_slots(tiles_per_chunk) // max(1, tiles_per_chunk)) + ng
            lo, hi = 32, max(32, round_up(max(padded) if padded else 32, 32))
            while lo < hi:
                mid = round_up((lo + hi) // 2, 32)
                if mid >= hi:
                    mid = hi - 32 if hi - 32 >= lo else lo
                n = sum((p + mid - 1) // mid for p in padded if p > 0)
                if n <= budget:
                    hi = mid
                else:
                    lo = mid + 32
            cr = lo
            chunks, gchunk, base = [], [], 0
            for g, p in enumerate(padded):
                first = len(chunks)
                for c0 in range(0, p, cr):
                    chunks.append((g, base + c0, min(cr, p - c0)))
                gchunk.append((first, len(chunks) - first))
                base += p
            ch = np.array(chunks, dtype=np.int32).reshape(-1, 3)
            gc = np.array(gchunk, dtype=np.int32).reshape(-1, 2)
            self._chunk_cache[key] = (torch.from_numpy(ch).to(device), torch.from_numpy(gc).to(device), len(ch))
        return self._chunk_cache[key]


def build_map(per_group: Sequence[Sequence[np.ndarray]], chunk_rows: int = 0) -> RowMap:
    G = len(per_group)
    nspace = len(per_group[0]) if G else 0
    total = sum(len(pg[0]) for pg in per_group)
    if chunk_rows <= 0:
        chunk_rows = max(4 * TILE, round_up(max(1, total // 256), TILE))
    rows = [[] for _ in range(nspace)]
    tile_group, chunks, gchunk = [], [], []
    base = 0
    for g, pg in enumerate(per_group):
        n = len(pg[0])
        npad = round_up(n, TILE)
        for s in range(nspace):
            r = np.full(npad, -1, dtype=np.int32)
            r[:n] = pg[s]
            rows[s].append(r)
        tile_group.extend([g] * (npad // TILE))
        first = len(chunks)
        for c0 in range(0, npad, chunk_rows):
            chunks.append((g, base + c0, min(chunk_rows, npad - c0)))
        gchunk.append((first, len(chunks) - first))
        base += npad
    cat = [np.concatenate(r) if r else np.zeros(0, np.int32) for r in rows]
    return RowMap(cat, np.array(tile_group, dtype=np.int32),
                  np.array(chunks, dtype=np.int32).reshape(-1, 3),
                  np.array(gchunk, dtype=np.int32).reshape(-1, 2), total,
                  group_rows=[len(pg[0]) for pg in per_group])


def layer_maps(cfg: OneTransConfig, B: int, I: int, K: int, p0: int = 0,
               I_full: int = 0) -> Dict[str, RowMap]:
    G = cfg.num_groups
    I_full = I_full or I
    grp = np.array([cfg.group_of_position(p0 + p, I_full) for p in range(I)])
    b = np.arange(B)[:, None]

    def rows_for(positions, fn):
        if len(positions) == 0:
            return np.zeros(0, np.int64)
        return fn(b, np.asarray(positions)[None, :]).reshape(-1)

    all_pg, tail_pg = [], []
    for g in range(G):
        pos = np.nonzero(grp == g)[0]
        all_pg.append([rows_for(pos, lambda bb, pp: bb * I + pp)])
        tpos = pos[pos >= I - K]
        tail_pg.append([rows_for(tpos, lambda bb, pp: bb * I + pp),
                        rows_for(tpos, lambda bb, pp: bb * K + (pp - (I - K)))])
    return {'all': build_map(all_pg), 'tail': build_map(tail_pg)}


def head_map(B: int, T: int) -> RowMap:
    b = np.arange(B)
    return build_map([[b, t * B + b] for t in range(T)])


def identity_map(n: int) -> RowMap:
    r = np.arange(n)
    return build_map([[r, r]])
```

### recommend_amd/model.py

```python

from __future__ import annotations

import json
import os
from typing import Dict, List, Optional, Tuple

import numpy as np
import torch
import torch.nn as nn

from . import _lib
from . import kernels as K
from ._lib import (OT_AX_BF16, OT_AX_BF16_RMSNORM, OT_AX_GELU, OT_AX_RMSNORM, OT_EPI_ACCUMULATE, OT_EPI_AUX_BF16, OT_EPI_BIAS,
                   OT_EPI_C_BF16, OT_EPI_DROPOUT, OT_EPI_GELU_BWD, OT_EPI_RESIDUAL, OT_EPI_RMSNORM_BWD,
                   OT_EPI_ROW_RSTD, OT_EPI_ROWDOT, OT_GEMM_NN, OT_GEMM_NT, OT_WG_D_BF16, NS_FIELD_BYTES)
from .config import (OneTransConfig, check_bag_features, check_padding_mask, check_pyramid_select, check_seq_fusion,
                     get_model_config)
from .layout import TILE, FlatLayout, RowMap, build_map, head_map, identity_map, layer_maps, round_up
from .params import init_params, ns_table_offsets

RMS_EPS = 1e-6


class _Tokenize(torch.autograd.Function):

    @staticmethod
    def forward(ctx, flat, m, plan):
        d = m.config.hidden_dim
        B, L0, L_S = plan['B'], plan['L0'], plan['L_S']
        dev = flat.device
        x0 = torch.empty(B * L0, d, device=dev)
        if plan['ns_fields'] > 0:
            nsm = plan['nsmat']
            if plan['ns_desc_n'] > 0:
                K.ns_assemble(plan['ns_desc'], plan['ns_desc_n'], m.tables.get('emb.ns'), B, nsm, m.layout.f_pad)
            if plan['n_bags'] > 0:
                K.ns_bag_pool(plan['bag_descs'], plan['n_bags'], B, nsm, m.layout.f_pad, plan['bag_coef'])
            mp = plan['ns_map'].to(dev)
            K.gemm(OT_GEMM_NT, nsm, m.layout.f_pad, m.layout.f_pad, mp['rows'][0], m.pT('tok.ns.kernel'), 0,
                   m.layout.f_pad, m.cfg_Lnsd, mp['tile_group'], plan['ns_map'].ntiles, (x0, L_S * d), L0 * d,
                   mp['rows'][0], bias=m.p('tok.ns.bias'), epi=OT_EPI_BIAS, m_rows=B, bimg=m.bimg('tok.ns.kernel'))
        else:
            x0.view(B, L0, d)[:, L_S:].zero_()
        if plan['seq_map'] is not None:
            sm = plan['seq_map'].to(dev)
            A, lda = plan['seq_A'], m.config.seq_feature_dim
            K.gemm(OT_GEMM_NT, A, lda, lda, plan['seq_in'], m.pT('tok.seq.kernel'), lda * d, lda, d, sm['tile_group'],
                   plan['seq_map'].ntiles, x0, d, _seq_out_rows(plan, sm), bias=m.p('tok.seq.bias'), bias_gstride=d,
                   epi=OT_EPI_BIAS, m_rows=plan['seq_M'], bimg=m.bimg('tok.seq.kernel'))
        if plan['n_sep'] > 0:
            K.fill_rows(x0, d, plan['sep_rows'], plan['n_sep'], m.p('tok.sep'), d)
        ctx.m, ctx.plan, ctx.gen = m, plan, plan['gen']
        return x0

    @staticmethod
    def backward(ctx, dx0):
        with K.precision(ctx.m.matmul):
            return _Tokenize._backward(ctx, dx0)

    @staticmethod
    def _backward(ctx, dx0):
        m, plan = ctx.m, ctx.plan
        if plan['gen'] != ctx.gen:
            raise RuntimeError('OneTransModel: a second forward with the same input shapes ran before this '
                               'backward; run backward before the next forward (inputs are staged in place)')
        dx0 = dx0.contiguous()
        d = m.config.hidden_dim
        B, L0, L_S = plan['B'], plan['L0'], plan['L_S']
        dev = dx0.device
        acc = m.accumulate_grads
        m._pending_sparse = []
        if plan['ns_fields'] > 0:
            mp = plan['ns_map'].to(dev)
            nsm = plan['nsmat']
            K.wgrad(nsm, m.layout.f_pad, mp['rows'][0], (dx0, L_S * d), L0 * d, mp['rows'][0], m.layout.f_pad,
                    m.cfg_Lnsd, mp, plan['ns_map'].chunks.shape[0], 1, m.g('tok.ns.kernel'), 0, m.g('tok.ns.bias'),
                    0, accumulate=acc, device=dev, m_rows=B, rowmap=plan['ns_map'])
            if plan['n_sparse'] > 0 or plan['n_bags'] > 0:
                dns = torch.empty(B, m.layout.f_pad, device=dev)
                K.gemm(OT_GEMM_NT, (dx0, L_S * d), L0 * d, m.cfg_Lnsd, mp['rows'][0], m.p('tok.ns.kernel'), 0,
                       m.cfg_Lnsd, m.layout.f_pad, mp['tile_group'], plan['ns_map'].ntiles, dns, m.layout.f_pad,
                       mp['rows'][0], m_rows=B)
                e = m.config.ns_embedding_dim
                n1 = plan['n_sparse'] * B
                n = n1 + plan['bag_ns_slots']
                if n > 0:
                    keys = torch.empty(n, dtype=torch.int64, device=dev)
                    grads = torch.empty(n, e, device=dev)
                    if n1 > 0:
                        K.ns_grad_pack(plan['ns_desc'], plan['n_sparse'], e, dns, m.layout.f_pad, B, keys, grads)
                    if plan['n_bags_ns'] > 0:
                        K.ns_bag_grad_pack(plan['bag_descs'], plan['n_bags_ns'], B, dns, m.layout.f_pad,
                                           plan['bag_coef'], (keys, n1), (grads, n1 * e))
                    m._pending_sparse.append(('emb.ns', keys, grads))
                nq = plan['n_bags'] - plan['n_bags_ns']
                if nq > 0:
                    Eq = m.config.seq_feature_dim
                    nslots = plan['bag_slots'] - plan['bag_ns_slots']
                    keys = torch.empty(nslots, dtype=torch.int64, device=dev)
                    grads = torch.empty(nslots, Eq, device=dev)
                    K.ns_bag_grad_pack(plan['bag_descs'], nq, B, dns, m.layout.f_pad,
                                       (plan['bag_coef'], plan['bag_ns_slots']), keys, grads, first=plan['n_bags_ns'])
                    m._pending_sparse.append(('emb.seq_item', keys, grads))
        elif not acc:
            m.g('tok.ns.kernel').zero_()
            m.g('tok.ns.bias').zero_()
        E = m.config.seq_feature_dim
        if plan['seq_map'] is not None:
            sm = plan['seq_map'].to(dev)
            xrows = _seq_out_rows(plan, sm)
            K.wgrad(plan['seq_A'], E, plan['seq_in'], dx0, d, xrows, E, d, sm,
                    plan['seq_map'].chunks.shape[0], plan['nseq'], m.g('tok.seq.kernel'), E * d,
                    m.g('tok.seq.bias'), d, accumulate=acc, device=dev, m_rows=plan['seq_M'],
                    rowmap=plan['seq_map'])
            if plan['seq_ids'] is not None:
                M = plan['seq_M']
                demb = torch.empty(M, E, device=dev)
                K.gemm(OT_GEMM_NT, dx0, d, d, xrows, m.p('tok.seq.kernel'), E * d, d, E, sm['tile_group'],
                       plan['seq_map'].ntiles, demb, E, sm['rows'][1], m_rows=plan['seq_M'])
                keys = plan['seq_route'] if 'emb.seq_item' in m.sharded else plan['seq_ids']
                m._pending_sparse.append(('emb.seq_item', keys, demb))
        elif not acc:
            m.g('tok.seq.kernel').zero_(); m.g('tok.seq.bias').zero_()
        if plan['n_sep'] > 0:
            K.rows_colsum(dx0, d, plan['sep_rows'], plan['n_sep'], d, m.g('tok.sep'), accumulate=acc, device=dev)
        elif not acc:
            m.g('tok.sep').zero_()
        m.join_side_stream()
        return None, None, None


def _seq_out_rows(plan, sm):
    rows = plan.get('seq_rows_t')
    return rows if rows is not None else sm['rows'][0]


def layer_seed(seed: int, b0: int, I: int, d: int) -> int:
    return (seed + b0 * I * d * 0x9E3779B1) & 0xFFFFFFFF if b0 else seed


def _layer_valid(kvalid, I):
    L0 = kvalid.shape[1]
    return kvalid, L0 - I, L0


def _attn_qpos(cfg, pos):
    return None if getattr(cfg, 'pyramid_select', 'tail') == 'tail' else pos


class PairBounds:
    SLOTS = ('o', 'u', 'dy2', 'du', 'dyo', 'dqkv')

    def __init__(self, layers: int, device):
        self.t, self._taken = torch.zeros(layers, 8, device=device), {}

    @classmethod
    def begin(cls, layers: int, device, mode: str, pair_wgrad: bool) -> Optional['PairBounds']:
        return cls(layers, device) if mode == 'split' and pair_wgrad and torch.is_grad_enabled() else None

    def out(self, l: int, name: str) -> torch.Tensor:
        return self._taken.setdefault((l, name), self.t[l, self.SLOTS.index(name):][:1])

    def get(self, l: int, name: str) -> Optional[torch.Tensor]:
        return self._taken.get((l, name))


def a_row_bounds(on: bool, x, ld: int, rows: int, n: int, reported=None) -> Dict:
    if on and reported is None:
        reported = torch.empty(rows, (n + 255) // 256, device=x.device)
        K.rows_absmax(x, ld, rows, n, reported)
    return dict(a_rowmax=reported, a_rowmax_n=reported.shape[1]) if on else {}


def _block_forward(m, l, x, I, Kq, seed, training, rstd_in=None, select=False, need_out=True, need_u=True,
                   bounds=None, kvalid=None):
    cfg = m.config
    d, f, H = cfg.hidden_dim, cfg.ffn_dim, cfg.num_heads
    hd = d // H
    B = x.shape[0] // I
    dev = x.device
    maps = m.maps(B, I, Kq)
    ma, mt = maps['all'].to(dev), maps['tail'].to(dev)
    na, nt = maps['all'].ntiles, maps['tail'].ntiles
    rate = cfg.dropout_rate if training else 0.0
    dflag = OT_EPI_DROPOUT if rate > 0 else 0
    wqkv, wo = m.pT(f'blk.{l}.wqkv'), m.pT(f'blk.{l}.wo')
    w1, b1, w2, b2 = m.pT(f'blk.{l}.w1'), m.p(f'blk.{l}.b1'), m.pT(f'blk.{l}.w2'), m.p(f'blk.{l}.b2')
    g1, g2 = m.p(f'blk.{l}.norm1'), m.p(f'blk.{l}.norm2')
    fuse = m.fuse_with((f'blk.{l}.wo', 'fwd'), (f'blk.{l}.w2', 'fwd'))
    if rstd_in is not None and rstd_in.numel() == B * I:
        rstd1 = rstd_in
    else:
        rstd1 = torch.empty(B * I, device=dev)
        K.rmsnorm_fwd(x, d, B * I, d, rstd1, eps=RMS_EPS)
    qrows, pos, inv = mt['rows'][0], None, None
    if select:
        pos = torch.empty(B * Kq, dtype=torch.int32, device=dev)
        inv = torch.empty(B * I, dtype=torch.int32, device=dev)
        if cfg.pyramid_select == 'norm':
            nf = min(cfg.num_ns_tokens, Kq)
            qrows = qrows.clone()
            K.pyramid_select(B, I, Kq, pos, inv, score=rstd1, sign=-1.0, nforce=nf, map_rows=qrows,
                             map_per_sample=Kq - nf)
        else:
            K.pyramid_select(B, I, Kq, pos, inv)
    tail = (Kq, I, pos)
    x16 = m.take_x16(l, x) if d % TILE == 0 and need_out else None
    ax1 = OT_AX_BF16_RMSNORM if x16 is not None else OT_AX_RMSNORM
    xa = x16 if x16 is not None else x
    qkv = torch.empty(B * I, 3 * d, device=dev)
    xn_on = (training and K.matmul_mode() == 'bf16' and d % TILE == 0
             and m.bimg(f'blk.{l}.wqkv') is not None)
    xn1 = torch.empty(B * I, d, dtype=torch.int16, device=dev) if xn_on else None
    x1n = torch.empty(B * Kq, d, dtype=torch.int16, device=dev) if xn_on else None
    if xn1 is not None:
        full = Kq == I
        K.gemm_rms(OT_GEMM_NT, xa, d, d, ma['rows'][0], wqkv if full else (wqkv, d * d), 3 * d * d, d,
                   3 * d if full else 2 * d, ma['tile_group'], na, qkv if full else (qkv, d), 3 * d, ma['rows'][0],
                   epi=0, a_xform=ax1, rstd=rstd1, gamma=g1, m_rows=maps['all'].nrows, device=dev,
                   bimg=m.bimg(f'blk.{l}.wqkv') if full else m.bimg(f'blk.{l}.wqkv', tn0=d // TILE),
                   xn_out=xn1, ldxn=d)
        if not full:
            K.gemm(OT_GEMM_NT, xa, d, d, qrows, wqkv, 3 * d * d, d, d, mt['tile_group'], nt, qkv,
                   3 * d, qrows, a_xform=ax1, rstd=rstd1, gamma=g1, m_rows=maps['tail'].nrows,
                   bimg=m.bimg(f'blk.{l}.wqkv'))
    elif Kq == I:
        K.gemm(OT_GEMM_NT, xa, d, d, ma['rows'][0], wqkv, 3 * d * d, d, 3 * d, ma['tile_group'], na, qkv,
               3 * d, ma['rows'][0], a_xform=ax1, rstd=rstd1, gamma=g1, m_rows=maps['all'].nrows,
               bimg=m.bimg(f'blk.{l}.wqkv'))
    else:
        K.gemm(OT_GEMM_NT, xa, d, d, ma['rows'][0], (wqkv, d * d), 3 * d * d, d, 2 * d, ma['tile_group'], na,
               (qkv, d), 3 * d, ma['rows'][0], a_xform=ax1, rstd=rstd1, gamma=g1, m_rows=maps['all'].nrows,
               bimg=m.bimg(f'blk.{l}.wqkv', tn0=d // TILE) if d % TILE == 0 else None)
        K.gemm(OT_GEMM_NT, xa, d, d, qrows, wqkv, 3 * d * d, d, d, mt['tile_group'], nt, qkv,
               3 * d, qrows, a_xform=ax1, rstd=rstd1, gamma=g1, m_rows=maps['tail'].nrows,
               bimg=m.bimg(f'blk.{l}.wqkv'))
    o = torch.empty(B * Kq, d, device=dev)
    lse = torch.empty(B * H * Kq, device=dev)
    qp_f = _attn_qpos(cfg, pos)
    qkv16 = (torch.empty(B * I, 3 * d, dtype=torch.int16, device=dev)
             if m.attn_fp8 and training and K.attn_bwd_bf16_supported(I, Kq, hd, qp_f) else None)
    out = (lambda name: bounds.out(l, name)) if bounds is not None else (lambda name: None)
    pwo_f = m.gemm_pair(f'blk.{l}.wo', 'fwd')
    o_rep = kvalid is None and not m.attn_fp8 and K.attn_amax_supported(I, Kq, hd, qp_f)
    rm_o = torch.empty(B * Kq, H, device=dev) if pwo_f and o_rep else None
    if kvalid is not None:
        K.attn_fwd_masked(qkv, 3 * d, B, H, I, Kq, hd, o, lse, _layer_valid(kvalid, I), qpos=qp_f)
    else:
        K.attn_fwd(qkv, 3 * d, B, H, I, Kq, hd, o, lse, qpos=qp_f, fp8=m.attn_fp8, dequant=m.attn_fp8 and training,
                   fp8_terms=m.fp8_terms, deq16=qkv16, amax=out('o') if o_rep else None, rowmax=rm_o)
    pa_o = a_row_bounds(pwo_f, o, d, B * Kq, d, rm_o)
    if qkv16 is not None:
        qkv = qkv16
    x1 = torch.empty(B * Kq, d, device=dev)
    rstd2 = torch.empty(B * Kq, device=dev)
    x1_16 = None
    if fuse:
        x1_16 = (torch.empty(B * Kq, d, dtype=torch.int16, device=dev)
                 if m.x16_on(d) and m.bimg(f'blk.{l}.w1') is not None else None)
        K.gemm_rms(OT_GEMM_NT, o, d, d, mt['rows'][1], wo, 0, d, d, mt['tile_group'], nt, x1, d, mt['rows'][1],
                   epi=OT_EPI_RESIDUAL | dflag | OT_EPI_ROW_RSTD, res=x, ldres=d, res_tok=1, seed=seed,
                   site=2 * l, drop=rate, tail=tail, m_rows=maps['tail'].nrows, rstd_out=rstd2, eps=RMS_EPS,
                   bimg=m.bimg(f'blk.{l}.wo'), c16_out=x1_16, ldc16=d, device=dev, **pa_o)
    else:
        K.gemm_rms(OT_GEMM_NT, o, d, d, mt['rows'][1], wo, 0, d, d, mt['tile_group'], nt, x1, d, mt['rows'][1],
                   epi=OT_EPI_RESIDUAL | dflag, res=x, ldres=d, res_tok=1, seed=seed, site=2 * l, drop=rate,
                   tail=tail, m_rows=maps['tail'].nrows, bimg=m.bimg(f'blk.{l}.wo'), device=dev, **pa_o)
        K.rmsnorm_fwd(x1, d, B * Kq, d, rstd2, eps=RMS_EPS)
    w2img = m.bimg(f'blk.{l}.w2')
    h = (torch.empty(B * Kq, f, dtype=torch.int16, device=dev)
         if K.matmul_mode() == 'bf16' and w2img is not None
         and m.bimg(f'blk.{l}.w1') is not None and f % TILE == 0 else None)
    u_bf = h is not None and m.fuse_bwd2 and not m.fuse_bwd and f % TILE == 0
    u = torch.empty(B * Kq, f, device=dev, dtype=torch.int16 if u_bf else torch.float32)
    pair_w2 = K.matmul_mode() == 'split' and w2img is not None and (f'blk.{l}.w2', 'fwd') in m.layout.pair_images
    assert not pair_w2 or (h is None and m.bimg(f'blk.{l}.w1') is not None and f % TILE == 0), \
        'the pair-form W2 image needs the FFN1 plane GEMM to write the row maxima of u'
    if (pair_w2 and need_out and d == TILE and f <= K.FFN_FUSED_MAX_F and x1_16 is None and K.ffn_fused()):
        if not need_u:
            u = None
        x2 = torch.empty(B * Kq, d, device=dev)
        rstd_out = torch.empty(B * Kq, device=dev) if fuse else None
        K.ffn_fused_fwd(x1, d, mt['rows'][1], mt['tile_group'], nt, rstd2, m.bimg(f'blk.{l}.w1')[0],
                        m.layout.images[(f'blk.{l}.w1', 'fwd')][1], w2img[0],
                        m.layout.images[(f'blk.{l}.w2', 'fwd')][1], b1, f, b2, d, f, x2, d, u_out=u, ldu=f,
                        u_amax=out('u'), rstd_out=rstd_out, eps=RMS_EPS, seed=seed, site=2 * l + 1, drop=rate,
                        tail=tail, m_rows=maps['tail'].nrows)
        saved = (x, rstd1, qkv, o, lse, x1, rstd2, u, None, xn1, None)
        return x2, rstd_out, saved, pos, inv, rate
    umax = torch.empty(B * Kq, f // TILE, device=dev) if pair_w2 else None
    if h is not None:
        K.gemm_rms(OT_GEMM_NT, x1 if x1_16 is None else x1_16, d, d, mt['rows'][1], w1, d * f, d, f,
                   mt['tile_group'], nt, u, f, mt['rows'][1],
                   a_xform=OT_AX_RMSNORM if x1_16 is None else OT_AX_BF16_RMSNORM, rstd=rstd2, gamma=g2, bias=b1,
                   bias_gstride=f,
                   epi=OT_EPI_BIAS | (OT_EPI_C_BF16 if u_bf else 0),
                   m_rows=maps['tail'].nrows, bimg=m.bimg(f'blk.{l}.w1'), gelu_out=h, ldgelu=f,
                   xn_out=x1n, ldxn=d)
    elif umax is not None:
        K.gemm_rms(OT_GEMM_NT, x1 if x1_16 is None else x1_16, d, d, mt['rows'][1], w1, d * f, d, f, mt['tile_group'],
                   nt, u, f, mt['rows'][1], a_xform=OT_AX_RMSNORM if x1_16 is None else OT_AX_BF16_RMSNORM,
                   rstd=rstd2, gamma=g2, bias=b1, bias_gstride=f, epi=OT_EPI_BIAS, m_rows=maps['tail'].nrows,
                   bimg=m.bimg(f'blk.{l}.w1'), rowmax_out=umax, rowmax_n=umax.shape[1],
                   amax_out=out('u'))
    else:
        K.gemm(OT_GEMM_NT, x1 if x1_16 is None else x1_16, d, d, mt['rows'][1], w1, d * f, d, f, mt['tile_group'],
               nt, u, f, mt['rows'][1], a_xform=OT_AX_RMSNORM if x1_16 is None else OT_AX_BF16_RMSNORM, rstd=rstd2,
               gamma=g2, bias=b1, bias_gstride=f, epi=OT_EPI_BIAS, m_rows=maps['tail'].nrows,
               bimg=m.bimg(f'blk.{l}.w1'))
    if x1n is not None and h is None:
        x1n = None
    saved = (x, rstd1, qkv, o, lse, x1, rstd2, u, h, xn1, x1n)
    if not need_out:
        return None, None, saved, pos, inv, rate
    x2 = torch.empty(B * Kq, d, device=dev)
    rstd_out = None
    a2, ax2 = (h, OT_AX_BF16) if h is not None else (u, OT_AX_GELU)
    pa_u = a_row_bounds(pair_w2, u, f, B * Kq, f, umax)
    if fuse:
        rstd_out = torch.empty(B * Kq, device=dev)
        x2_16 = torch.empty(B * Kq, d, dtype=torch.int16, device=dev) if m.x16_on(d) and w2img is not None else None
        K.gemm_rms(OT_GEMM_NT, a2, f, f, mt['rows'][1], w2, f * d, f, d, mt['tile_group'], nt, x2, d,
                   mt['rows'][1], a_xform=ax2, bias=b2, bias_gstride=d,
                   epi=OT_EPI_BIAS | OT_EPI_RESIDUAL | dflag | OT_EPI_ROW_RSTD, res=x1, ldres=d, res_tok=0,
                   seed=seed, site=2 * l + 1, drop=rate, tail=tail, m_rows=maps['tail'].nrows,
                   rstd_out=rstd_out, eps=RMS_EPS, bimg=w2img, c16_out=x2_16, ldc16=d, **pa_u)
        m.put_x16(l + 1, x2, x2_16)
    elif umax is not None:
        K.gemm_rms(OT_GEMM_NT, a2, f, f, mt['rows'][1], w2, f * d, f, d, mt['tile_group'], nt, x2, d, mt['rows'][1],
                   a_xform=ax2, bias=b2, bias_gstride=d, epi=OT_EPI_BIAS | OT_EPI_RESIDUAL | dflag, res=x1,
                   ldres=d, res_tok=0, seed=seed, site=2 * l + 1, drop=rate, tail=tail,
                   m_rows=maps['tail'].nrows, bimg=w2img, **pa_u)
    else:
        K.gemm(OT_GEMM_NT, a2, f, f, mt['rows'][1], w2, f * d, f, d, mt['tile_group'], nt, x2, d, mt['rows'][1],
               a_xform=ax2, bias=b2, bias_gstride=d, epi=OT_EPI_BIAS | OT_EPI_RESIDUAL | dflag, res=x1,
               ldres=d, res_tok=0, seed=seed, site=2 * l + 1, drop=rate, tail=tail,
               m_rows=maps['tail'].nrows, bimg=w2img)
    return x2, rstd_out, saved, pos, inv, rate


class _Block(torch.autograd.Function):

    @staticmethod
    def forward(ctx, flat, x, m, l, I, Kq, seed, training, rstd_in=None, select=False, bounds=None, kvalid=None):
        x2, rstd_out, saved, pos, inv, rate = _block_forward(
            m, l, x, I, Kq, seed, training, rstd_in, select, bounds=bounds,
            need_u=not m.recompute and any(ctx.needs_input_grad), kvalid=kvalid)
        if m.recompute:
            ctx.save_for_backward(saved[0], saved[1])
            ctx.fwd_args = (training, select)
        else:
            ctx.save_for_backward(*saved)
        ctx.m, ctx.l, ctx.I, ctx.Kq, ctx.seed, ctx.rate = m, l, I, Kq, seed, rate
        ctx.pos, ctx.inv, ctx.bounds, ctx.kvalid = pos, inv, bounds, kvalid
        if rstd_out is None:
            rstd_out = x2.new_empty(0)
        ctx.mark_non_differentiable(rstd_out)
        return x2, rstd_out

    @staticmethod
    def backward(ctx, dx2, _drstd=None):
        with K.precision(ctx.m.matmul):
            return _Block._backward(ctx, dx2, _drstd)

    @staticmethod
    def _backward(ctx, dx2, _drstd=None):
        m, l, I, Kq, seed, rate = ctx.m, ctx.l, ctx.I, ctx.Kq, ctx.seed, ctx.rate
        pos, inv, bounds, kvalid = ctx.pos, ctx.inv, ctx.bounds, ctx.kvalid
        if m.recompute:
            xin, rstd_in = ctx.saved_tensors
            training, select = ctx.fwd_args
            _, _, saved, pos, inv, _ = _block_forward(m, l, xin, I, Kq, seed, training, rstd_in, select,
                                                      need_out=False, bounds=bounds, kvalid=kvalid)
            x, rstd1, qkv, o, lse, x1, rstd2, u, h, xn1, x1n = saved
        else:
            x, rstd1, qkv, o, lse, x1, rstd2, u, h, xn1, x1n = ctx.saved_tensors
        tail = (Kq, I, pos)
        cfg = m.config
        d, f, H = cfg.hidden_dim, cfg.ffn_dim, cfg.num_heads
        hd = d // H
        B = x.shape[0] // I
        dev = x.device
        acc = m.accumulate_grads
        maps = m.maps(B, I, Kq)
        ma, mt = maps['all'].to(dev), maps['tail'].to(dev)
        na, nt = maps['all'].ntiles, maps['tail'].ntiles
        nca, nct = maps['all'].chunks.shape[0], maps['tail'].chunks.shape[0]
        G = cfg.num_groups
        dx2 = dx2.contiguous()
        rowdot = None
        fused2 = m.fuse_bwd2 and not m.fuse_bwd and f % TILE == 0
        du_bf = (fused2 and h is not None and m.bimg(f'blk.{l}.w1', 'dgrad') is not None)
        out = (lambda name: bounds.out(l, name)) if bounds is not None else (lambda name: None)
        b_o, b_u = (bounds.get(l, 'o'), bounds.get(l, 'u')) if bounds is not None else (None, None)
        keep = (bounds.t,) if bounds is not None else ()
        pw2, pw1, pwo = (m.dgrad_pair(f'blk.{l}.{w}') for w in ('w2', 'w1', 'wo'))
        dy2_rep = rate > 0 and not du_bf
        b_dy2 = out('dy2') if dy2_rep else None
        rm_dy2 = (torch.empty(B * Kq, (d + 255) // 256, device=dev)
                  if dy2_rep and pw2 and K.dropout_rowmax_supported(d) else None)
        dy2 = dx2
        if rate > 0:
            dy2 = torch.empty(B * Kq, d, device=dev, dtype=torch.int16 if du_bf else torch.float32)
            K.dropout_apply(dx2, d, dy2, d, B * Kq, d, seed, 2 * l + 1, rate, tail, amax=b_dy2, rowmax=rm_dy2)
        pa2 = a_row_bounds(pw2, dy2, d, B * Kq, d, rm_dy2)
        dy_bf = dy2.dtype == torch.int16
        du = torch.empty(B * Kq, f, device=dev, dtype=torch.int16 if du_bf else torch.float32)
        cbf = OT_EPI_C_BF16 if du_bf else 0
        hbf = (torch.empty(B * Kq, f, dtype=torch.int16, device=dev)
               if h is None and fused2 and K.matmul_mode() == 'bf16' else None)
        if hbf is None:
            with m.side(u if h is None else h, dy2, *keep):
                K.wgrad(u if h is None else h, f, mt['rows'][1], dy2, d, mt['rows'][1], f, d, mt, nct, G,
                        m.g(f'blk.{l}.w2'), f * d, m.g(f'blk.{l}.b2'), d,
                        a_xform=(OT_AX_GELU if h is None else OT_AX_BF16) | (OT_WG_D_BF16 if dy_bf else 0),
                        accumulate=acc, device=dev, m_rows=maps['tail'].nrows, rowmap=maps['tail'],
                        a_bound=b_u if h is None else None, d_bound=b_dy2)
        du_rep = fused2 or (((bounds is not None and not du_bf) or pw2 or pw1) and f % TILE == 0)
        b_du = out('du') if du_rep and not du_bf else None
        rm_du = torch.empty(B * Kq, f // TILE, device=dev) if pw1 and du_rep else None
        rep_du = dict(amax_out=b_du, rowabs_out=rm_du, rowabs_n=f // TILE if rm_du is not None else 0)
        if fused2:
            rowdot = torch.empty(B * Kq, f // TILE, device=dev)
            K.gemm_rms(OT_GEMM_NT, dy2, d, d, mt['rows'][1], m.p(f'blk.{l}.w2'), f * d, d, f, mt['tile_group'], nt,
                       du, f, mt['rows'][1], aux=u, ldaux=f, a_xform=OT_AX_BF16 if dy_bf else 0,
                       epi=OT_EPI_GELU_BWD | OT_EPI_ROWDOT | cbf | (OT_EPI_AUX_BF16 if u.dtype == torch.int16 else 0),
                       bias=m.p(f'blk.{l}.b1'), bias_gstride=f, rowdot=rowdot, rowdot_n=f // TILE,
                       m_rows=maps['tail'].nrows, device=dev, bimg=m.bimg(f'blk.{l}.w2', 'dgrad'),
                       gelu_out=hbf, ldgelu=f, **rep_du, **pa2)
            if hbf is not None:
                with m.side(hbf, dy2):
                    K.wgrad(hbf, f, mt['rows'][1], dy2, d, mt['rows'][1], f, d, mt, nct, G, m.g(f'blk.{l}.w2'),
                            f * d, m.g(f'blk.{l}.b2'), d, a_xform=OT_AX_BF16, accumulate=acc, device=dev,
                            m_rows=maps['tail'].nrows, rowmap=maps['tail'])
        else:
            K.gemm_rms(OT_GEMM_NT, dy2, d, d, mt['rows'][1], m.p(f'blk.{l}.w2'), f * d, d, f, mt['tile_group'], nt, du,
                       f, mt['rows'][1], epi=OT_EPI_GELU_BWD, aux=u, ldaux=f, m_rows=maps['tail'].nrows, device=dev,
                       bimg=m.bimg(f'blk.{l}.w2', 'dgrad'), **rep_du, **pa2)
        pa1 = a_row_bounds(pw1, du, f, B * Kq, f, rm_du)
        a1n = x1n is not None and du_bf
        with m.side(x1n if a1n else x1, du, rstd2, *keep):
            K.wgrad(x1n if a1n else x1, d, mt['rows'][1], du, f, mt['rows'][1], d, f, mt, nct, G, m.g(f'blk.{l}.w1'),
                    d * f, m.g(f'blk.{l}.b1'), f, rstd=rstd2, gamma=m.p(f'blk.{l}.norm2'),
                    a_xform=(OT_AX_BF16 if a1n else OT_AX_RMSNORM) | (OT_WG_D_BF16 if du_bf else 0),
                    accumulate=acc, device=dev, m_rows=maps['tail'].nrows, rowmap=maps['tail'], d_bound=b_du)
        dx1 = torch.empty(B * Kq, d, device=dev)
        dyo = torch.empty(B * Kq, d, device=dev) if rate > 0 else dx1
        dx1_ep = m.fuse_bwd or rowdot is not None
        rm_dyo = torch.empty(B * Kq, (d + TILE - 1) // TILE, device=dev) if pwo and dx1_ep else None
        b_dyo = out('dyo') if dx1_ep else None
        if dx1_ep:
            K.gemm_rms(OT_GEMM_NT, du, f, f, mt['rows'][1], m.p(f'blk.{l}.w1'), d * f, f, d, mt['tile_group'], nt,
                       dx1, d, mt['rows'][1], epi=OT_EPI_RMSNORM_BWD | (OT_EPI_DROPOUT if rate > 0 else 0),
                       a_xform=OT_AX_BF16 if du_bf else 0,
                       seed=seed, site=2 * l, drop=rate, tail=tail, m_rows=maps['tail'].nrows, nx=x1, ldnx=d,
                       ngamma=m.p(f'blk.{l}.norm2'), nrstd=rstd2, dres=dx2, lddres=d,
                       dx_masked=dyo if rate > 0 else None, lddxm=d, dgamma=m.g(f'blk.{l}.norm2'),
                       accumulate_dgamma=acc, device=dev, bimg=m.bimg(f'blk.{l}.w1', 'dgrad'),
                       rowdot=rowdot, rowdot_n=f // TILE if rowdot is not None else 0, amax_out=b_dyo,
                       rowabs_out=rm_dyo, rowabs_n=rm_dyo.shape[1] if rm_dyo is not None else 0, **pa1)
        else:
            dxn2 = torch.empty(B * Kq, d, device=dev)
            K.gemm_rms(OT_GEMM_NT, du, f, f, mt['rows'][1], m.p(f'blk.{l}.w1'), d * f, f, d, mt['tile_group'], nt,
                       dxn2, d, mt['rows'][1], epi=0, m_rows=maps['tail'].nrows, device=dev,
                       bimg=m.bimg(f'blk.{l}.w1', 'dgrad'), **pa1)
            K.rmsnorm_bwd(dxn2, d, x1, d, m.p(f'blk.{l}.norm2'), rstd2, dx1, d, B * Kq, d, dres=dx2, lddres=d,
                          dx_masked=dyo if rate > 0 else None, lddxm=d, seed=seed, site=2 * l, drop=rate,
                          tail=tail, dgamma=m.g(f'blk.{l}.norm2'), accumulate=acc, device=dev)
        with m.side(o, dyo, *keep):
            _wgrad_single(m, o, dyo, d, d, mt, m.g(f'blk.{l}.wo'), acc, dev, maps['tail'].nrows, maps['tail'],
                          a_bound=b_o, d_bound=b_dyo)
        do = torch.empty(B * Kq, d, device=dev)
        K.gemm_rms(OT_GEMM_NT, dyo, d, d, mt['rows'][1], m.p(f'blk.{l}.wo'), 0, d, d, mt['tile_group'], nt, do, d,
                   mt['rows'][1], epi=0, m_rows=maps['tail'].nrows, device=dev, bimg=m.bimg(f'blk.{l}.wo', 'dgrad'),
                   **a_row_bounds(pwo, dyo, d, B * Kq, d, rm_dyo))
        qp = _attn_qpos(cfg, pos)
        dq_bf = (K.matmul_mode() == 'bf16'
                 and K.attn_bwd_bf16_forms(I, Kq, hd, qp) & _lib.OT_ATTN_DQKV_BF16
                 and m.bimg(f'blk.{l}.wqkv', 'dgrad') is not None)
        dqkv = torch.empty(B * I, 3 * d, device=dev, dtype=torch.int16 if dq_bf else torch.float32)
        if Kq < I:
            dqkv[:, :d].zero_()
        bwd_b = kvalid is None and not dq_bf and K.attn_amax_supported(I, Kq, hd, qp, backward=True)
        b_dq = out('dqkv') if bwd_b else None
        pqkv = m.dgrad_pair(f'blk.{l}.wqkv')
        rm_dq = torch.zeros(B * I, 3 * H, device=dev) if pqkv and bwd_b else None
        if kvalid is not None:
            K.attn_bwd_masked(qkv, 3 * d, o, do, lse, B, H, I, Kq, hd, dqkv, _layer_valid(kvalid, I), qpos=qp)
        else:
            K.attn_bwd(qkv, 3 * d, o, do, lse, B, H, I, Kq, hd, dqkv, qpos=qp, dq_part_bf16=True, amax=b_dq,
                       rowmax=rm_dq)
        pa_q = a_row_bounds(pqkv, dqkv, 3 * d, B * I, 3 * d, rm_dq)
        an1 = xn1 is not None and dq_bf
        with m.side(xn1 if an1 else x, dqkv, rstd1, *keep):
            K.wgrad(xn1 if an1 else x, d, ma['rows'][0], dqkv, 3 * d, ma['rows'][0], d, 3 * d, ma, nca, G,
                    m.g(f'blk.{l}.wqkv'), 3 * d * d, None, 0,
                    a_xform=(OT_AX_BF16 if an1 else OT_AX_RMSNORM) | (OT_WG_D_BF16 if dq_bf else 0), rstd=rstd1,
                    gamma=m.p(f'blk.{l}.norm1'), accumulate=acc, device=dev, m_rows=maps['all'].nrows,
                    rowmap=maps['all'], d_bound=b_dq)
        ax_dq = OT_AX_BF16 if dq_bf else 0
        dx = torch.empty(B * I, d, device=dev)
        if m.fuse_bwd:
            K.gemm_rms(OT_GEMM_NT, dqkv, 3 * d, 3 * d, ma['rows'][0], m.p(f'blk.{l}.wqkv'), 3 * d * d, 3 * d, d,
                       ma['tile_group'], na, dx, d, ma['rows'][0], epi=OT_EPI_RMSNORM_BWD, a_xform=ax_dq,
                       m_rows=maps['all'].nrows, nx=x, ldnx=d, ngamma=m.p(f'blk.{l}.norm1'), nrstd=rstd1,
                       dres=dx1, lddres=d, dres_tail=(Kq, I, inv) if Kq < I else (0, 0),
                       dgamma=m.g(f'blk.{l}.norm1'), accumulate_dgamma=acc, device=dev,
                       bimg=m.bimg(f'blk.{l}.wqkv', 'dgrad'), **pa_q)
        else:
            dxn1 = torch.empty(B * I, d, device=dev)
            K.gemm_rms(OT_GEMM_NT, dqkv, 3 * d, 3 * d, ma['rows'][0], m.p(f'blk.{l}.wqkv'), 3 * d * d, 3 * d, d,
                       ma['tile_group'], na, dxn1, d, ma['rows'][0], epi=0, m_rows=maps['all'].nrows, a_xform=ax_dq,
                       bimg=m.bimg(f'blk.{l}.wqkv', 'dgrad'), device=dev, **pa_q)
            K.rmsnorm_bwd(dxn1, d, x, d, m.p(f'blk.{l}.norm1'), rstd1, dx, d, B * I, d, dres=dx1, lddres=d,
                          dres_tail=(Kq, I, inv) if Kq < I else (0, 0), dgamma=m.g(f'blk.{l}.norm1'), accumulate=acc,
                          device=dev)
        m.side_block_done()
        if m.grad_ready is not None:
            m.grad_ready(l)
        return None, dx, None, None, None, None, None, None, None, None, None, None


def _wgrad_single(m, A, D, K_, N, mt, dW, acc, dev, mrows=0, rowmap=None, a_bound=None, d_bound=None):
    if rowmap is not None and rowmap.group_rows:
        ch, _, _ = rowmap.chunks_for(((K_ + 127) // 128) * ((N + 127) // 128), dev)
        mp = m.single_group_chunks({'chunks': ch})
    else:
        mp = m.single_group_chunks(mt)
    K.wgrad(A, K_, mt['rows'][1], D, N, mt['rows'][1], K_, N, mp, mp['chunks'].shape[0], 1, dW, 0, None, 0,
            accumulate=acc, device=dev, m_rows=mrows, a_bound=a_bound, d_bound=d_bound)


class _Head(torch.autograd.Function):

    @staticmethod
    def forward(ctx, flat, x, m):
        cfg = m.config
        d, T = cfg.hidden_dim, len(cfg.tasks)
        dh = d // 2
        B = x.shape[0]
        dev = x.device
        y = torch.empty(B, d, device=dev)
        rstd = torch.empty(B, device=dev)
        K.rmsnorm_fwd(x, d, B, d, rstd, gamma=m.p('out_norm'), y=y, ldy=d, eps=RMS_EPS)
        hm = m.head_rows(B)
        hmd = hm.to(dev)
        pre1 = torch.empty(T * B, dh, device=dev)
        K.gemm(OT_GEMM_NT, y, d, d, hmd['rows'][0], m.pT('head.w1'), d * dh, d, dh, hmd['tile_group'], hm.ntiles,
               pre1, dh, hmd['rows'][1], bias=m.p('head.b1'), bias_gstride=dh, epi=OT_EPI_BIAS, m_rows=hm.nrows)
        logits = torch.empty(T, B, device=dev)
        probs = torch.empty(T, B, device=dev)
        K.head_fwd(pre1, m.p('head.w2'), m.p('head.b2'), T, B, dh, logits, probs)
        ctx.save_for_backward(x, rstd, y, pre1, probs)
        ctx.m = m
        ctx.set_materialize_grads(False)
        m._last_logits = logits
        return probs, logits

    @staticmethod
    def backward(ctx, dprobs, dlogits):
        with K.precision(ctx.m.matmul):
            return _Head._backward(ctx, dprobs, dlogits)

    @staticmethod
    def _backward(ctx, dprobs, dlogits):
        x, rstd, y, pre1, probs = ctx.saved_tensors
        m = ctx.m
        cfg = m.config
        d, T = cfg.hidden_dim, len(cfg.tasks)
        dh = d // 2
        B = x.shape[0]
        dev = x.device
        acc = m.accumulate_grads
        dprobs = dprobs.contiguous() if dprobs is not None else None
        dlogits = dlogits.contiguous() if dlogits is not None else None
        if dprobs is None and dlogits is None:
            return None, None, None
        dpre1 = torch.empty(T * B, dh, device=dev)
        K.head_bwd(pre1, m.p('head.w2'), probs, dprobs, T, B, dh, dpre1, m.g('head.w2'), m.g('head.b2'), dh, 1,
                   accumulate=acc, device=dev, dlogits=dlogits)
        hm = m.head_rows(B)
        hmd = hm.to(dev)
        K.wgrad(y, d, hmd['rows'][0], dpre1, dh, hmd['rows'][1], d, dh, hmd, hm.chunks.shape[0], T, m.g('head.w1'),
                d * dh, m.g('head.b1'), dh, accumulate=acc, device=dev, m_rows=hm.nrows)
        im = m.ident_rows(B).to(dev)
        nti = m.ident_rows(B).ntiles
        dy = torch.empty(B, d, device=dev)
        for t in range(T):
            K.gemm(OT_GEMM_NT, (dpre1, t * B * dh), dh, dh, im['rows'][0], (m.p('head.w1'), t * d * dh), 0, dh, d,
                   im['tile_group'], nti, dy, d, im['rows'][0], epi=OT_EPI_ACCUMULATE if t > 0 else 0, m_rows=B)
        dx = torch.empty(B, d, device=dev)
        K.rmsnorm_bwd(dy, d, x, d, m.p('out_norm'), rstd, dx, d, B, d, dgamma=m.g('out_norm'), accumulate=acc,
                      device=dev)
        if m.grad_ready is not None:
            m.grad_ready('head')
        return None, dx, None


class _TaskLoss(torch.autograd.Function):

    @staticmethod
    def forward(ctx, probs, logits, labels, mse_mask):
        T, B = probs.shape
        loss = torch.empty(1, device=probs.device)
        K.task_loss_logits_fwd(logits, probs, labels, T, B, loss, device=probs.device, mse_mask=mse_mask)
        ctx.save_for_backward(probs, labels)
        ctx.mse_mask = mse_mask
        return loss[0]

    @staticmethod
    def backward(ctx, gl):
        probs, labels = ctx.saved_tensors
        T, B = probs.shape
        dlogits = torch.empty_like(probs)
        gl = gl.reshape(1).contiguous().float()
        K.task_loss_logits_bwd(probs, labels, gl, T, B, dlogits, mse_mask=ctx.mse_mask)
        return None, dlogits, None, None


class _BCE(torch.autograd.Function):

    @staticmethod
    def forward(ctx, probs, labels, mse_mask):
        T, B = probs.shape
        loss = torch.empty(1, device=probs.device)
        K.bce_fwd(probs, labels, T, B, loss, device=probs.device, mse_mask=mse_mask)
        ctx.save_for_backward(probs, labels)
        ctx.mse_mask = mse_mask
        return loss[0]

    @staticmethod
    def backward(ctx, gl):
        probs, labels = ctx.saved_tensors
        T, B = probs.shape
        dprobs = torch.empty_like(probs)
        gl = gl.reshape(1).contiguous().float()
        K.bce_bwd(probs, labels, gl, T, B, dprobs, mse_mask=ctx.mse_mask)
        return dprobs, None, None


BINARY_TASKS = ('ctr', 'cvr')


def task_mse_mask(tasks) -> int:
    if len(tasks) > 32:
        raise ValueError('at most 32 tasks')
    return sum(1 << i for i, t in enumerate(tasks) if t not in BINARY_TASKS)


def keras_bce_loss(labels: torch.Tensor, probs: torch.Tensor, tasks=None, label_rank: int = 2) -> torch.Tensor:
    mask = task_mse_mask(tasks) if tasks is not None else 0
    z = getattr(probs, '_ot_logits', None) if label_rank >= 2 else None
    if z is not None:
        return _TaskLoss.apply(probs, z, labels, mask)
    return _BCE.apply(probs, labels, mask)


in_model_precision = K.in_model_precision


class OneTransModel(nn.Module):

    def __init__(self, config: OneTransConfig, device=None, seed: int = 0, init: Optional[Dict] = None):
        super().__init__()
        _lib.load()
        if not torch.cuda.is_available():
            raise _lib.OneTransHipError('OneTransModel needs a ROCm GPU (no CPU fallback)')
        self.config = config
        self.device = torch.device(device) if device is not None else torch.device('cuda', torch.cuda.current_device())
        cfg = config
        if cfg.hidden_dim % cfg.num_heads or (cfg.hidden_dim // cfg.num_heads) not in (16, 32, 64, 128):
            raise ValueError('head_dim must be 16, 32, 64 or 128')
        check_pyramid_select(cfg)
        check_seq_fusion(cfg)
        check_bag_features(cfg)
        check_padding_mask(cfg)
        self.padding_mask = bool(getattr(cfg, 'seq_padding_mask', False))
        self.time_fusion = getattr(cfg, 'seq_fusion', 'sep') == 'time'
        if getattr(cfg, 'compute_dtype', 'fp32') not in ('fp32', 'bf16', 'fp8attn'):
            raise ValueError(f"compute_dtype {cfg.compute_dtype!r}: expected 'fp32', 'bf16' or 'fp8attn'")
        if getattr(cfg, 'compute_dtype', 'fp32') in ('bf16', 'fp8attn'):
            self.matmul = 'bf16'
        elif K.matmul_mode() == 'bf16':
            raise ValueError("compute_dtype 'fp32' with the process default matmul 'bf16' (ONETRANS_MATMUL / "
                             "kernels.set_matmul_mode): set config.compute_dtype = 'bf16' for the bf16 arithmetic")
        else:
            self.matmul = K.matmul_mode()
        self.recompute = bool(getattr(cfg, 'recompute_blocks', False))
        self.attn_fp8 = getattr(cfg, 'compute_dtype', 'fp32') == 'fp8attn'
        if self.attn_fp8 and cfg.hidden_dim // cfg.num_heads not in (64, 128):
            raise ValueError('fp8 attention needs head_dim 64 or 128')
        self.fp8_terms = int(getattr(cfg, 'fp8_terms', 2))
        if self.fp8_terms not in (1, 2):
            raise ValueError(f'fp8_terms {self.fp8_terms}: 1 or 2')
        self.f_ns = cfg.ns_input_width()
        self.layout = FlatLayout(cfg, self.f_ns, pair_dgrad=os.environ.get('ONETRANS_PAIR_DGRAD', '1') != '0')
        self.cfg_Lnsd = cfg.num_ns_tokens * cfg.hidden_dim
        self.flat = nn.Parameter(torch.zeros(self.layout.total, device=self.device))
        self.flat.grad = torch.zeros_like(self.flat)
        self.flatT = torch.zeros(self.layout.total, device=self.device)
        self._tdesc = torch.from_numpy(self.layout.transpose_desc.reshape(-1)).to(self.device)
        self.img = torch.zeros(max(1, self.layout.image_elems), dtype=torch.int16, device=self.device)
        self._img_valid, self._img_mode = False, None
        self._idesc = (torch.from_numpy(self.layout.image_desc.reshape(-1)).to(self.device)
                       if self.layout.image_units else None)
        self.tables: Dict[str, torch.Tensor] = {}
        self.accumulate_grads = False
        self.grad_ready = None
        self.fuse_norms = config.hidden_dim % TILE == 0
        self.fuse_bwd = self.fuse_norms and config.hidden_dim == TILE
        self.fuse_bwd2 = self.fuse_norms
        self._x16 = None
        self.overlap_wgrad = True
        self.pair_wgrad = os.environ.get('ONETRANS_PAIR_WGRAD', '1') != '0'
        self._side = None
        self._side_used = False
        self._side_keep: List[torch.Tensor] = []
        self._side_fifo: List = []
        self.kv_cache = None
        self._pending_sparse: List = []
        self._plans: Dict = {}
        self._maps: Dict = {}
        self._aux_maps: Dict = {}
        self._step = 0
        self.dropout_seed = 0x5EED0000 ^ seed
        self.sample_offset: Optional[int] = None
        self.inputs_ready = None
        self.sharded: Dict[str, 'ShardedTable'] = {}
        self._pending_route = None
        self.last_table_ids: Dict[str, torch.Tensor] = {}
        shard_seq = self._shard_seq_table()
        params = init if init is not None else init_params(cfg, self.f_ns, seed=seed, with_tables=False)
        if shard_seq:
            from .sharded import ShardedTable
            import torch.distributed as dist
            full = params.get('emb.seq_item') if init is not None else None
            params = {k: v for k, v in params.items() if k != 'emb.seq_item'}
            dist_on = dist.is_available() and dist.is_initialized()
            st = ShardedTable('emb.seq_item', cfg.seq_item_vocab, cfg.seq_feature_dim,
                              dist.get_world_size() if dist_on else 1, dist.get_rank() if dist_on else 0,
                              self.device, seed=seed + 2, full_init=full, route_stream=self.comm_stream())
            self.sharded['emb.seq_item'] = st
            self.tables['emb.seq_item'] = st.table
        self.load_param_dict(params)
        if init is None or not any(k.startswith('emb.') for k in init):
            self._init_tables_device(seed + 1)

    def p(self, name):
        return self.layout.view(self.flat.data, name)

    def g(self, name):
        return self.layout.view(self.flat.grad, name)

    def pT(self, name):
        return self.layout.tview(self.flatT, name)

    @in_model_precision
    def refresh_shadow(self) -> None:
        K.transpose_banks(self.flat.data, self.flatT, self._tdesc, self.layout.transpose_desc.shape[0],
                          self.layout.transpose_tiles)
        self._img_valid = False
        if self._idesc is not None and K.matmul_mode() in ('split', 'bf16'):
            self._build_images()

    def _build_images(self) -> None:
        K.split_images(self.flat.data, self._idesc, self.layout.image_desc.shape[0], self.layout.image_units,
                       self.img)
        self._img_valid = True
        self._img_mode = K.matmul_mode()

    def fuse_with(self, *images) -> bool:
        if not self.fuse_norms:
            return False
        if self.config.hidden_dim == TILE:
            return True
        return all(self.bimg(n, o) is not None for (n, o) in images)

    @property
    def pair_dgrad(self) -> bool:
        return self.layout.pair_dgrad

    def gemm_pair(self, name: str, orient: str) -> bool:
        return (K.matmul_mode() == 'split' and (name, orient) in self.layout.pair_images
                and self.bimg(name, orient) is not None and not (orient == 'fwd' and not name.endswith('.wo')))

    def dgrad_pair(self, name: str) -> bool:
        return self.gemm_pair(name, 'dgrad')

    def x16_on(self, d: int) -> bool:
        return d % TILE == 0 and K.matmul_mode() == 'bf16'

    def put_x16(self, layer: int, x: torch.Tensor, x16: Optional[torch.Tensor]) -> None:
        self._x16 = (layer, x, x.data_ptr(), x.numel(), x16) if x16 is not None else None

    def take_x16(self, layer: int, x: torch.Tensor) -> Optional[torch.Tensor]:
        c, self._x16 = self._x16, None
        if (c is None or c[0] != layer or not self.x16_on(x.shape[-1]) or c[2] != x.data_ptr()
                or c[3] != x.numel()):
            return None
        return c[4]

    def bimg(self, name: str, orient: str = 'fwd', tn0: int = 0):
        e = self.layout.images.get((name, orient))
        if e is None:
            return None
        mode = K.matmul_mode()
        if mode not in ('split', 'bf16'):
            return None
        if not self._img_valid or self._img_mode != mode:
            self._build_images()
        off, G, N, K_ = e
        return ((self.img, off), N // TILE, tn0)

    def load_param_dict(self, params: Dict[str, np.ndarray]) -> None:
        with torch.no_grad():
            for name, arr in params.items():
                if name in self.sharded:
                    st = self.sharded[name]
                    arr = np.asarray(arr)
                    if arr.shape != (st.num_rows, st.E):
                        raise ValueError(f'{name}: loaded shape {arr.shape} != ({st.num_rows}, {st.E})')
                    st.table[:st.local_rows].copy_(torch.as_tensor(arr[st.rank::st.world], dtype=torch.float32))
                    self.tables[name] = st.table
                    continue
                if name.startswith('emb.'):
                    want = self._table_shape(name)
                    if want is not None and tuple(np.shape(arr)) != want:
                        raise ValueError(f'{name}: loaded shape {tuple(np.shape(arr))} != {want} of this config')
                    self.tables[name] = torch.as_tensor(np.asarray(arr), dtype=torch.float32).to(self.device).contiguous()
                    continue
                dst = self.p(name)
                src = torch.as_tensor(np.asarray(arr), dtype=torch.float32)
                if name == 'tok.ns.kernel' and src.shape[0] != dst.shape[0]:
                    dst.zero_()
                    dst[:src.shape[0]].copy_(src)
                else:
                    dst.copy_(src.reshape(dst.shape))
        self.refresh_shadow()

    def _table_shape(self, name: str):
        cfg = self.config
        if name == 'emb.ns':
            return (ns_table_offsets(cfg)['__total__'], cfg.ns_embedding_dim)
        if name == 'emb.seq_item':
            return (cfg.seq_item_vocab, cfg.seq_feature_dim)
        return None

    def param_dict(self) -> Dict[str, np.ndarray]:
        out = {}
        for name in self.layout.shapes:
            v = self.p(name).detach().cpu().numpy().copy()
            if name == 'tok.ns.kernel':
                v = v[:self.f_ns]
            out[name] = v
        for k, t in self.tables.items():
            src = self.sharded[k].full_table() if k in self.sharded else t
            out[k] = src.detach().cpu().numpy().copy()
        return out

    def _shard_seq_table(self) -> bool:
        import torch.distributed as dist
        cfg = self.config
        mode = os.environ.get('ONETRANS_TABLE_SHARDING', getattr(cfg, 'table_sharding', 'auto'))
        if not cfg.seq_item_vocab or mode == 'none':
            return False
        if mode == 'row':
            return True
        if not (dist.is_available() and dist.is_initialized() and dist.get_world_size() > 1):
            return False
        return cfg.seq_item_vocab * cfg.seq_feature_dim * 4 > 2 ** 30

    def _init_tables_device(self, seed: int) -> None:
        cfg = self.config
        gen = torch.Generator(device=self.device)
        gen.manual_seed(seed)
        total = ns_table_offsets(cfg)['__total__']
        if total:
            t = torch.empty(total, cfg.ns_embedding_dim, device=self.device)
            t.uniform_(-0.05, 0.05, generator=gen)
            self.tables['emb.ns'] = t
        if cfg.seq_item_vocab and 'emb.seq_item' not in self.sharded:
            t = torch.empty(cfg.seq_item_vocab, cfg.seq_feature_dim, device=self.device)
            t.uniform_(-0.05, 0.05, generator=gen)
            self.tables['emb.seq_item'] = t

    @property
    def trainable_variables(self):
        return [self.flat] + list(self.tables.values())

    def maps(self, B, I, Kq, p0=0, I_full=0):
        key = (B, I, Kq) if p0 == 0 and I_full in (0, I) else (B, I, Kq, p0, I_full)
        if key not in self._maps:
            self._maps[key] = layer_maps(self.config, B, I, Kq, p0=p0, I_full=I_full)
        return self._maps[key]

    def head_rows(self, B):
        key = ('head', B)
        if key not in self._aux_maps:
            self._aux_maps[key] = head_map(B, len(self.config.tasks))
        return self._aux_maps[key]

    def ident_rows(self, B):
        key = ('ident', B)
        if key not in self._aux_maps:
            self._aux_maps[key] = identity_map(B)
        return self._aux_maps[key]

    def single_group_chunks(self, mt_dev):
        key = ('single', mt_dev['chunks'].data_ptr())
        if key not in self._aux_maps:
            ch = mt_dev['chunks'].clone()
            ch[:, 0] = 0
            g = torch.tensor([[0, ch.shape[0]]], dtype=torch.int32, device=ch.device)
            self._aux_maps[key] = {'chunks': ch, 'gchunk': g}
        return self._aux_maps[key]

    def _plan(self, ns: Dict[str, torch.Tensor], seq: Dict[str, torch.Tensor], training: bool = False):
        cfg = self.config
        d = cfg.hidden_dim
        dev = self.device
        B = next(iter(ns.values())).shape[0] if ns else next(iter(seq.values())).shape[0]
        seq_names = cfg.feature_config['sequence_features']
        present = [(i, n, int(seq[n].shape[1])) for i, n in enumerate(seq_names) if n in seq]
        ns_present = tuple(n for n in cfg.ns_feature_names() if n in ns)
        id_seq = bool(cfg.seq_item_vocab) and bool(present) and not torch.is_floating_point(torch.as_tensor(seq[present[0][1]]))
        bags = self._bag_inputs(ns, ns_present, B) if cfg.bag_features else ()
        key = (B, tuple(present), ns_present, id_seq) + ((tuple((n, cap, w is not None) for n, cap, _, w in bags),)
                                                         if bags else ())
        times = self._seq_times(seq, present, B) if self.time_fusion and present else None
        lens = self._seq_lengths(seq, present, B) if self.padding_mask else None
        plan = self._plans.get(key)
        if plan is None:
            plan = self._build_plan(B, present, ns_present, id_seq, bags)
            self._plans[key] = plan
        plan['gen'] += 1
        if plan['ns_fields'] > 0:
            if plan['n_dense'] > 0:
                plan['dense_buf'].copy_(torch.cat([ns[n].reshape(B, 1).to(dev, torch.float32)
                                                   for n in plan['dense_names']], 1))
            if plan['n_sparse'] > 0:
                plan['ids_buf'].copy_(torch.cat([ns[n].reshape(B, 1).to(dev, torch.int64)
                                                 for n in plan['sparse_names']], 1))
            for (n, cap, ids, w), (ids_buf, w_buf) in zip(bags, plan['bag_bufs']):
                ids_buf.copy_(ids)
                if w_buf is not None:
                    w_buf.copy_(w)
            for k, tname in enumerate(plan.get('bag_tables', ())):
                plan['bag_descs'][k].table = self.tables[tname].data_ptr()
        if plan['seq_map'] is not None:
            if self.time_fusion:
                for buf, t in zip(plan['time_bufs'], times):
                    buf.copy_(t)
                K.seq_time_rows(plan['time_descs'], len(present), B, plan['L_S'], plan['L0'], plan['seq_rows_t'],
                                rank_out=plan['seq_rank'], last_time=plan['last_time'], device=dev)
            if self.padding_mask:
                self._stage_valid(plan, lens, B)
            if id_seq and 'emb.seq_item' in self.sharded:
                st = self.sharded['emb.seq_item']
                srcs = [seq[n] for (_, n, _) in present]
                ids = [s_ if isinstance(s_, torch.Tensor) else torch.from_numpy(np.ascontiguousarray(s_)) for s_ in srcs]
                routed = None
                if training and self._pending_route is not None:
                    routed, self._pending_route = self._pending_route, None
                plan['seq_A'] = st.lookup(ids, ready=self.inputs_ready, routed=routed, srcs=srcs)
                plan['seq_ids'] = st.last_ids
                plan['seq_route'] = st.last_route
            elif id_seq:
                ids = [seq[n].to(dev, torch.int64).contiguous() for (_, n, _) in present]
                for (i, n, L), t, off in zip(present, ids, plan['seq_seg_off']):
                    K.seq_rows(t, L, B, L, cfg.seq_item_vocab, (plan['seq_in'], off))
                plan['seq_ids'] = torch.cat([t.reshape(-1) for t in ids])
                self.last_table_ids = {'emb.seq_item': plan['seq_ids']}
                plan['seq_A'] = self.tables['emb.seq_item']
            else:
                buf = plan['seq_buf']
                o = 0
                for (i, n, L) in present:
                    buf[o:o + B * L].copy_(seq[n].reshape(B * L, -1).to(dev, torch.float32))
                    o += B * L
                plan['seq_A'] = buf
                plan['seq_ids'] = None
        if self.padding_mask and plan['seq_map'] is None:
            self._stage_valid(plan, [], B)
        return plan

    def _seq_lengths(self, seq, present, B) -> List[torch.Tensor]:
        sfx = self.config.seq_len_suffix
        out = []
        for (_, n, L) in present:
            if n + sfx not in seq:
                raise ValueError(f'seq_padding_mask: sequence {n!r} has no lengths ({n + sfx!r} is missing from '
                                 'seq_features)')
            t = seq[n + sfx]
            t = t if isinstance(t, torch.Tensor) else torch.from_numpy(np.ascontiguousarray(t))
            if t.is_floating_point() or t.is_complex() or t.dtype == torch.bool:
                raise TypeError(f'seq_padding_mask: the lengths of sequence {n!r} ({n + sfx!r}) are {t.dtype}; '
                                'integers are expected')
            if tuple(t.shape) not in ((B,), (B, 1)):
                raise ValueError(f'seq_padding_mask: the lengths of sequence {n!r} ({n + sfx!r}) have shape '
                                 f'{tuple(t.shape)}, expected {(B,)} or {(B, 1)}')
            if t.device.type == 'cpu' and B and (int(t.min()) < 0 or int(t.max()) > L):
                raise ValueError(f'seq_padding_mask: the lengths of sequence {n!r} ({n + sfx!r}) leave [0, {L}]')
            out.append(t.reshape(B))
        return out

    def _stage_valid(self, plan, lens, B) -> None:
        dev = self.device
        groups = plan.get('seq_groups', []) if lens else []
        if lens:
            buf = plan['len_buf']
            for k, (t, (_, _, L)) in enumerate(zip(lens, groups)):
                buf[k].copy_(t.clamp(0, L))
        valid0 = torch.empty(B, plan['L0'], dtype=torch.uint8, device=dev)
        K.seq_key_valid(plan['len_buf'] if lens else None, [L for (_, _, L) in groups], [p0 for (_, p0, _) in groups],
                        B, plan['L0'], valid0, rank=plan.get('seq_rank') if lens else None)
        plan['valid0'] = valid0

    def _bag_inputs(self, ns, ns_present, B):
        cfg = self.config
        out = []
        for n in ns_present:
            if n not in cfg.bag_features:
                continue
            ids = ns[n]
            ids = ids if isinstance(ids, torch.Tensor) else torch.from_numpy(np.ascontiguousarray(ids))
            if ids.is_floating_point() or ids.is_complex() or ids.dtype == torch.bool:
                raise TypeError(f'bag feature {n!r}: integer ids are expected, got {ids.dtype}')
            if ids.dim() != 2 or ids.shape[0] != B or ids.shape[1] < 1:
                raise ValueError(f'bag feature {n!r}: ids of shape [B, cap] with cap >= 1 are expected, got '
                                 f'{tuple(ids.shape)} (B = {B})')
            w = ns.get(n + '_weight')
            if w is not None:
                if cfg.bag_pooling(n) != 'sum':
                    raise ValueError(f"bag feature {n!r}: per-slot weights need pooling 'sum' (it is "
                                     f'{cfg.bag_pooling(n)!r})')
                w = w if isinstance(w, torch.Tensor) else torch.from_numpy(np.ascontiguousarray(w))
                if tuple(w.shape) != tuple(ids.shape) or not w.is_floating_point():
                    raise ValueError(f'bag feature {n!r}: weights must be floats of the ids\' shape '
                                     f'{tuple(ids.shape)}, got {w.dtype} {tuple(w.shape)}')
            out.append((n, int(ids.shape[1]), ids, w))
        return tuple(out)

    def _seq_times(self, seq, present, B) -> List[torch.Tensor]:
        sfx = self.config.seq_time_suffix
        out = []
        for (_, n, L) in present:
            if n + sfx not in seq:
                raise ValueError(f"seq_fusion='time': sequence {n!r} has no times ({n + sfx!r} is missing from "
                                 'seq_features)')
            t = seq[n + sfx]
            t = t if isinstance(t, torch.Tensor) else torch.from_numpy(np.ascontiguousarray(t))
            if t.is_floating_point() or t.is_complex() or t.dtype == torch.bool:
                raise TypeError(f'seq_fusion=\'time\': the times of sequence {n!r} ({n + sfx!r}) are {t.dtype}; '
                                'integer timestamps are expected (they are widened to int64)')
            if tuple(t.shape) != (B, L):
                raise ValueError(f"seq_fusion='time': the times of sequence {n!r} ({n + sfx!r}) have shape "
                                 f'{tuple(t.shape)}, expected {(B, L)}')
            out.append(t)
        return out

    def _build_plan(self, B, present, ns_present, id_seq, bags=()):
        cfg = self.config
        d = cfg.hidden_dim
        dev = self.device
        nseq_cfg = len(cfg.feature_config['sequence_features'])
        plan = {'B': B, 'gen': 0}
        if self.time_fusion and present and id_seq and 'emb.seq_item' in self.sharded:
            raise NotImplementedError("seq_fusion='time' with a row-sharded emb.seq_item table is not supported: the "
                                      "sharded lookup delivers rows through a static token-order route; use "
                                      "table_sharding='none' or seq_fusion='sep'")
        pos = 0
        seq_groups, sep_pos = [], []
        for (i, n, L) in present:
            seq_groups.append((i, pos, L))
            pos += L
            if i < nseq_cfg - 1 and not self.time_fusion:
                sep_pos.append(pos)
                pos += 1
        L_S = pos
        L0 = L_S + cfg.num_ns_tokens
        plan.update(L_S=L_S, L0=L0, nseq=nseq_cfg)
        b = np.arange(B)
        if sep_pos:
            sep_rows = (b[:, None] * L0 + np.array(sep_pos)[None, :]).reshape(-1).astype(np.int32)
            plan['sep_rows'] = torch.from_numpy(sep_rows).to(dev)
        else:
            plan['sep_rows'] = None
        plan['n_sep'] = B * len(sep_pos)
        if present:
            per_group = [[np.zeros(0, np.int64), np.zeros(0, np.int64), np.zeros(0, np.int64)]
                         for _ in range(nseq_cfg)]
            cmp_off = 0
            flat_off = 0
            for (i, p0, L) in seq_groups:
                m_ = np.arange(B * L)
                bb, pp = m_ // L, m_ % L
                per_group[i] = [bb * L0 + p0 + pp, cmp_off + m_, flat_off + m_]
                cmp_off += B * L
                flat_off += B * L
            rm = build_map(per_group)
            plan['seq_map'] = rm
            plan['seq_M'] = cmp_off
            offs = []
            starts = np.concatenate([[0], np.cumsum([round_up(len(pg[0]), TILE) for pg in per_group])])
            for (i, p0, L) in seq_groups:
                offs.append(int(starts[i]))
            plan['seq_seg_off'] = offs
            seq_in = torch.from_numpy(rm.rows[2].copy()).to(dev)
            plan['seq_in'] = seq_in
            if self.padding_mask:
                plan['seq_groups'] = seq_groups
                plan['len_buf'] = torch.zeros(len(seq_groups), B, dtype=torch.int32, device=dev)
            if not id_seq:
                plan['seq_buf'] = torch.empty(cmp_off, cfg.seq_feature_dim, device=dev)
            if self.time_fusion:
                if L_S > _lib.SEQ_TIME_MAX_L:
                    raise ValueError(f"seq_fusion='time': {L_S} events per sample, at most {_lib.SEQ_TIME_MAX_L}")
                plan['time_bufs'] = [torch.empty(B, L, dtype=torch.int64, device=dev) for (_, _, L) in seq_groups]
                plan['time_descs'] = K.seq_time_descs([(t, L, L, off) for t, (_, _, L), off
                                                       in zip(plan['time_bufs'], seq_groups, offs)])
                plan['seq_rows_t'] = torch.from_numpy(rm.rows[0].copy()).to(dev)
                plan['seq_rank'] = torch.empty(B, L_S, dtype=torch.int32, device=dev)
                plan['last_time'] = torch.empty(B, dtype=torch.int64, device=dev)
        else:
            plan['seq_map'] = None
        offs = ns_table_offsets(cfg)
        dense_names = [n for n in ns_present if n not in cfg.sparse_features and n not in cfg.bag_features]
        sparse_names = [n for n in ns_present if n in cfg.sparse_features]
        plan.update(dense_names=dense_names, sparse_names=sparse_names, n_dense=len(dense_names),
                    n_sparse=len(sparse_names), ns_fields=len(ns_present),
                    ns_desc_n=len(dense_names) + len(sparse_names), n_bags=0, n_bags_ns=0, bag_bufs=[],
                    bag_slots=0, bag_ns_slots=0)
        plan['nsmat'] = torch.zeros(B, self.layout.f_pad, device=dev)
        if ns_present:
            plan['dense_buf'] = torch.zeros(B, max(1, len(dense_names)), device=dev)
            plan['ids_buf'] = torch.zeros(B, max(1, len(sparse_names)), dtype=torch.int64, device=dev)
            col = {}
            c = 0
            for n in ns_present:
                col[n] = c
                c += cfg.ns_feature_width(n)
            recs = np.zeros(max(1, plan['ns_desc_n']),
                            dtype=np.dtype([('dense', '<u8'), ('ids', '<u8'), ('row_offset', '<i8'),
                                            ('stride', '<i8'), ('col', '<i4'), ('width', '<i4')]))
            assert recs.dtype.itemsize == NS_FIELD_BYTES
            k = 0
            for j, n in enumerate(sparse_names):
                recs[k] = (0, plan['ids_buf'].data_ptr() + 8 * j, offs[n], len(sparse_names), col[n],
                           cfg.ns_embedding_dim)
                k += 1
            for j, n in enumerate(dense_names):
                recs[k] = (plan['dense_buf'].data_ptr() + 4 * j, 0, 0, len(dense_names), col[n], 1)
                k += 1
            plan['ns_desc'] = torch.from_numpy(recs.view(np.uint8).copy()).to(dev)
            plan['ns_map'] = identity_map(B)
            if bags:
                self._plan_bags(plan, B, bags, col, offs)
        return plan

    def _plan_bags(self, plan, B, bags, col, offs) -> None:
        cfg, dev = self.config, self.device
        import torch.distributed as dist
        if dist.is_available() and dist.is_initialized() and dist.get_world_size() > 1:
            raise NotImplementedError('bag_features: data-parallel runs (world size > 1) are not supported (the '
                                      'sparse all-gather and the early dense exchange are not exercised with bags)')
        if len(bags) > _lib.NS_BAG_MAX:
            raise ValueError(f'bag_features: {len(bags)} bag features in one batch, at most {_lib.NS_BAG_MAX}')
        is_seq = lambda n: cfg.bag_features[n].get('table') == 'seq_item'
        if any(is_seq(n) for n, _, _, _ in bags) and 'emb.seq_item' in self.sharded:
            raise NotImplementedError("bag_features: a 'seq_item' bag with a row-sharded emb.seq_item table is not "
                                      "supported (the bag gathers local rows); use table_sharding='none'")
        order = sorted(range(len(bags)), key=lambda i: is_seq(bags[i][0]))
        bufs = [None] * len(bags)
        recs = []
        for i in order:
            n, cap, _, w = bags[i]
            E = cfg.ns_feature_width(n)
            if E % 4 or E > _lib.NS_BAG_MAX_WIDTH:
                raise ValueError(f'bag feature {n!r}: row width {E} must be a multiple of 4, at most '
                                 f'{_lib.NS_BAG_MAX_WIDTH}')
            ids_buf = torch.full((B, cap), -1, dtype=torch.int64, device=dev)
            w_buf = torch.zeros(B, cap, device=dev) if w is not None else None
            bufs[i] = (ids_buf, w_buf)
            recs.append(dict(table=self.tables['emb.seq_item' if is_seq(n) else 'emb.ns'], ids=ids_buf, weights=w_buf,
                             row_offset=0 if is_seq(n) else offs[n], num_rows=cfg.bag_rows(n), ids_stride=cap,
                             weights_stride=cap, width=E, cap=cap, col=col[n], pooling=cfg.bag_pooling(n)))
        n_ns = sum(1 for i in order if not is_seq(bags[i][0]))
        slots = [B * r['cap'] for r in recs]
        plan.update(n_bags=len(bags), n_bags_ns=n_ns, bag_bufs=bufs, bag_slots=sum(slots),
                    bag_ns_slots=sum(slots[:n_ns]), bag_descs=K.ns_bag_descs(recs),
                    bag_tables=['emb.seq_item' if is_seq(bags[i][0]) else 'emb.ns' for i in order],
                    bag_coef=torch.zeros(max(1, sum(slots)), device=dev))

    def forward(self, non_seq_features, seq_features=None, training: bool = False,
                use_kv_cache: bool = False):
        if seq_features is None and isinstance(non_seq_features, (tuple, list)) and len(non_seq_features) == 2:
            non_seq_features, seq_features = non_seq_features
        seq_features = seq_features or {}
        training = bool(training)
        probs = self.forward_probs(non_seq_features, seq_features, training)
        return {t: probs[i].view(-1, 1) for i, t in enumerate(self.config.tasks)}

    @in_model_precision
    def forward_probs(self, ns, seq, training: bool) -> torch.Tensor:
        plan = self._plan(ns, seq, training)
        bounds = PairBounds.begin(self.config.num_layers, self.device, K.matmul_mode(), self.pair_wgrad)
        seed = 0
        if training:
            self._step += 1
            seed = (self.dropout_seed + 0x9E3779B9 * self._step) & 0xFFFFFFFF
        x = _Tokenize.apply(self.flat, self, plan)
        sched = self.config.pyramid_schedule(plan['L0'])
        nl = len(sched)
        b0 = self.batch_offset(plan['B']) if training else 0
        rstd = None
        for l, s in enumerate(sched):
            Kq = s['keep'] if l < nl - 1 else 1
            select = l < nl - 1 and Kq < s['in_len']
            x, rstd = _Block.apply(self.flat, x, self, l, s['in_len'], Kq, layer_seed(seed, b0, s['in_len'],
                                   self.config.hidden_dim), training, rstd, select, bounds, plan.get('valid0'))
        probs, logits = _Head.apply(self.flat, x, self)
        probs._ot_logits = logits
        return probs

    def forward_requests(self, non_seq_features, seq_features, req, training: bool = False, validate: bool = True):
        probs = self.forward_probs_requests(non_seq_features, seq_features, req, bool(training), validate)
        return {t: probs[i].view(-1, 1) for i, t in enumerate(self.config.tasks)}

    @in_model_precision
    def forward_probs_requests(self, ns, seq, req, training: bool = False, validate: bool = True) -> torch.Tensor:
        from . import request_train
        return request_train.forward_probs_requests(self, ns, seq, req, training, validate)

    def route_ahead(self, seq_features: Dict) -> None:
        if 'emb.seq_item' not in self.sharded or not seq_features:
            return
        names = [n for n in self.config.feature_config['sequence_features'] if n in seq_features]
        if not names or torch.is_floating_point(torch.as_tensor(seq_features[names[0]])):
            return
        srcs = [seq_features[n] for n in names]
        ids = [s_ if isinstance(s_, torch.Tensor) else torch.from_numpy(np.ascontiguousarray(s_)) for s_ in srcs]
        self._pending_route = self.sharded['emb.seq_item'].route(ids, ready=self.inputs_ready, srcs=srcs)

    def batch_offset(self, B: int) -> int:
        if self.sample_offset is not None:
            return int(self.sample_offset)
        import torch.distributed as dist
        if dist.is_available() and dist.is_initialized() and dist.get_world_size() > 1:
            return dist.get_rank() * B
        return 0

    def comm_stream(self):
        if getattr(self, '_comm', None) is None:
            self._comm = torch.cuda.Stream(device=self.device)
        return self._comm

    def side(self, *tensors):
        import contextlib
        if not self.overlap_wgrad:
            return contextlib.nullcontext()
        main = torch.cuda.current_stream(self.device)
        if self._side is None:
            self._side = torch.cuda.Stream(device=self.device)
        self._side.wait_stream(main)
        self._side_keep.extend(tensors)
        self._side_used = True
        return torch.cuda.stream(self._side)

    def side_block_done(self, depth: int = 2):
        if self._side is None or not self._side_keep:
            return
        ev = torch.cuda.Event()
        ev.record(self._side)
        self._side_fifo.append((ev, self._side_keep))
        self._side_keep = []
        while len(self._side_fifo) > depth:
            ev0, _ = self._side_fifo.pop(0)
            torch.cuda.current_stream(self.device).wait_event(ev0)

    def join_side_stream(self):
        if self._side is not None and self._side_used:
            torch.cuda.current_stream(self.device).wait_stream(self._side)
            self._side_used = False
        self._side_keep = []
        self._side_fifo = []

    def reset_kv_cache(self):
        self.kv_cache = None

    def get_model_info(self) -> Dict:
        n = int(sum(r * c for (_, r, c, _) in self.layout.segments))
        return {'total_parameters': n, 'num_layers': self.config.num_layers,
                'hidden_dim': self.config.hidden_dim, 'num_heads': self.config.num_heads,
                'embedding_rows': {k: int(v.shape[0]) for k, v in self.tables.items()}}

    def save_weights(self, path: str) -> None:
        params = self.param_dict()
        if self.sharded and self._rank() != 0:
            return
        os.makedirs(os.path.dirname(os.path.abspath(path)), exist_ok=True)
        np.savez(path, **params)

    @staticmethod
    def _rank() -> int:
        import torch.distributed as dist
        return dist.get_rank() if dist.is_available() and dist.is_initialized() else 0

    def load_weights(self, path: str) -> None:
        with np.load(path, allow_pickle=False) as z:
            self.load_param_dict({k: z[k] for k in z.files})


def create_onetrans_model(model_type: str = 'default', device=None) -> OneTransModel:
    return OneTransModel(get_model_config(model_type), device=device)
```

Measured before the change: 200,700 samples/s.

## Fold K/V projections into last-layer single-query attention for shared-weight rows

When the final layer has a single query token (Kq==1), new fused kernels compute attention scores and outputs by multiplying the query through the shared K/V weights. This replaces projecting every group-0 token to K and V, so the qkv GEMM only covers the group-specific rows and the last token. Backward gets matching fused kernels that produce dx, dgamma partials and K/V weight gradients from pooled vectors, and the dqkv GEMM and wgrad run over the smaller folded row map. This cuts the large per-token GEMM work in the last layer, at the cost of new custom kernels with per-block matvecs and an extra dW reduction pass, gated by an environment flag.

```diff
diff --git a/include/onetrans_hip.h b/include/onetrans_hip.h
--- a/include/onetrans_hip.h
+++ b/include/onetrans_hip.h
@@ -203,6 +203,24 @@
                        const float* lse, float* dqkv, float* dkv_cache, int accumulate, void* workspace,
                        size_t ws_bytes, void* stream);
 
+int ot_attn_fold_supported(int d, int H);
+int ot_attn_fold_rows(int I, int ded0, int ded1);
+int ot_attn_fold_fwd(const float* x, int64_t ldx, const float* rstd, const float* gamma, const float* w, int64_t ldw,
+                     const float* wT, int64_t ldwT, const float* qkv, int64_t ldqkv, int B, int H, int I,
+                     int head_dim, int ded0, int ded1, float* o, float* lse, float* y, void* stream);
+int ot_attn_fold_bwd(const float* x, int64_t ldx, const float* rstd, const float* gamma, const float* w, int64_t ldw,
+                     const float* wT, int64_t ldwT, const float* qkv, int64_t ldqkv, int B, int H, int I,
+                     int head_dim, int ded0, int ded1, const float* o, const float* dout, const float* lse,
+                     const float* y, const float* dx1, float* dx, int64_t lddx, float* dqkv, int64_t lddqkv, float* z,
+                     float* dgpart, void* stream);
+size_t ot_attn_fold_workspace_size(int B, int d);
+int ot_attn_fold_dw(const float* z, const float* y, const float* qkv, int64_t ldqkv, const float* dout,
+                    const float* gamma, int B, int H, int I, int head_dim, float* dW, int64_t lddw, int accumulate,
+                    void* workspace, size_t ws_bytes, void* stream);
+int ot_attn_fold_dgamma(const float* dgpart, int B, int d, float* dgamma, int accumulate, void* workspace,
+                        size_t ws_bytes, void* stream);
+int ot_last_fold(int on);
+
 int ot_attn_fwd_masked(const float* qkv, int64_t ld, int B, int H, int I, int K, const int32_t* qpos, int head_dim,
                        const uint8_t* key_valid, int64_t ldv, float* out, float* lse, int precision, void* stream);
 int ot_attn_bwd_masked(const float* qkv, int64_t ld, const float* out, const float* dout, const float* lse, int B,
diff --git a/recommend_amd/_lib.py b/recommend_amd/_lib.py
--- a/recommend_amd/_lib.py
+++ b/recommend_amd/_lib.py
@@ -198,6 +198,16 @@
     'ot_kv_pack_bf16': (c_int, [P, I64, c_int, I64, c_int, P, I64, I64, I64, P]),
     'ot_attn_fwd_cached_kv16': (c_int, [P, I64, P, I64, I64, P, c_int, c_int, c_int, c_int, c_int, c_int, P, I64, P, P,
                                         P]),
+    'ot_attn_fold_supported': (c_int, [c_int, c_int]),
+    'ot_attn_fold_rows': (c_int, [c_int, c_int, c_int]),
+    'ot_attn_fold_fwd': (c_int, [P, I64, P, P, P, I64, P, I64, P, I64, c_int, c_int, c_int, c_int, c_int, c_int, P, P,
+                                 P, P]),
+    'ot_attn_fold_bwd': (c_int, [P, I64, P, P, P, I64, P, I64, P, I64, c_int, c_int, c_int, c_int, c_int, c_int, P, P,
+                                 P, P, P, P, I64, P, I64, P, P, P]),
+    'ot_attn_fold_workspace_size': (c_size_t, [c_int, c_int]),
+    'ot_attn_fold_dw': (c_int, [P, P, P, I64, P, P, c_int, c_int, c_int, c_int, P, I64, c_int, P, c_size_t, P]),
+    'ot_attn_fold_dgamma': (c_int, [P, c_int, c_int, P, c_int, P, c_size_t, P]),
+    'ot_last_fold': (c_int, [c_int]),
     'ot_ns_bag_pool': (c_int, [P, c_int, c_int, P, I64, P, P]),
     'ot_ns_bag_grad_pack': (c_int, [P, c_int, c_int, P, I64, P, P, P, P]),
 }
diff --git a/recommend_amd/csrc/attention_fold.hip b/recommend_amd/csrc/attention_fold.hip
--- /dev/null
+++ b/recommend_amd/csrc/attention_fold.hip
@@ -0,0 +1,476 @@
+#include <atomic>
+#include <cstdlib>
+
+#include "gemm.h"
+
+namespace ot {
+namespace fold {
+
+constexpr int FD = 128;
+constexpr int NHW = 8;
+constexpr int DW_ROWS = 32;
+
+struct FoldArgs {
+  const float* x; int64_t ldx; const float* rstd; const float* gamma;
+  const float* w; int64_t ldw;
+  const float* wT; int64_t ldwT;
+  const float* qkv; int64_t ldqkv;
+  int B, I, ded0, ded1; float scale;
+  float* o; float* lse; float* y;
+  const float* dout; const float* dx1;
+  float* dx; int64_t lddx; float* dqkv; int64_t lddqkv; int nf; float* z; float* dgpart;
+};
+
+__device__ __forceinline__ float half_sum(float v) {
+  v += __int_as_float(__builtin_amdgcn_update_dpp(0, __float_as_int(v), 0xB1, 0xF, 0xF, false));
+  v += __int_as_float(__builtin_amdgcn_update_dpp(0, __float_as_int(v), 0x4E, 0xF, 0xF, false));
+  v += __int_as_float(__builtin_amdgcn_update_dpp(0, __float_as_int(v), 0x141, 0xF, 0xF, false));
+  v += __int_as_float(__builtin_amdgcn_update_dpp(0, __float_as_int(v), 0x140, 0xF, 0xF, false));
+  const auto a = __builtin_amdgcn_permlane16_swap(__float_as_uint(v), __float_as_uint(v), false, false);
+  return __uint_as_float(a[0]) + __uint_as_float(a[1]);
+}
+__device__ __forceinline__ float dot4(f32x4 a, f32x4 b) { return a.x * b.x + a.y * b.y + a.z * b.z + a.w * b.w; }
+__device__ __forceinline__ f32x4 ld4(const float* p) { return *reinterpret_cast<const f32x4*>(p); }
+__device__ __forceinline__ void st4(float* p, f32x4 v) { *reinterpret_cast<f32x4*>(p) = v; }
+
+template <int H>
+__device__ __forceinline__ void head_matvec_T(const float* wT, int64_t ldwT, int col0, const float* v,
+                                              float (*out)[FD], int t) {
+  constexpr int HD = FD / H;
+  for (int idx = t; idx < H * FD; idx += 256) {
+    const int h = idx / FD, k = idx % FD;
+    const float* wk = wT + (int64_t)(col0 + h * HD) * ldwT + k;
+    float a = 0.f;
+#pragma unroll 8
+    for (int c = 0; c < HD; ++c) a = fmaf(wk[(int64_t)c * ldwT], v[h * HD + c], a);
+    out[h][k] = a;
+  }
+}
+
+template <int H>
+__device__ __forceinline__ void head_matvec(const float* w, int64_t ldw, int col0, const float (*gv)[FD],
+                                            float (*part)[FD], int t) {
+  constexpr int HD = FD / H;
+  const int n = t & (FD - 1), half = t >> 7, h = n / HD;
+  const float* wn = w + (int64_t)(half * 64) * ldw + col0 + n;
+  float a = 0.f;
+#pragma unroll 8
+  for (int k = 0; k < 64; ++k) a = fmaf(wn[(int64_t)k * ldw], gv[h][half * 64 + k], a);
+  part[half][n] = a;
+}
+
+template <int H>
+__global__ __launch_bounds__(256) void attn_fold_fwd_kernel(FoldArgs p) {
+  constexpr int HD = FD / H, LPH = 32 / H;
+  __shared__ __attribute__((aligned(16))) float qs[FD];
+  __shared__ __attribute__((aligned(16))) float qt[H][FD];
+  __shared__ float rm[NHW][H], rl[NHW][H];
+  __shared__ __attribute__((aligned(16))) float ry[NHW][H][FD];
+  __shared__ __attribute__((aligned(16))) float ro[NHW][FD];
+  __shared__ float gy[H][FD];
+  __shared__ float po[2][FD];
+  const int b = blockIdx.x, t = threadIdx.x, hw = t >> 5, lane = t & 31, myh = lane / LPH;
+  const int64_t row0 = (int64_t)b * p.I;
+  if (t < FD) qs[t] = p.qkv[(row0 + p.I - 1) * p.ldqkv + t];
+  __syncthreads();
+  head_matvec_T<H>(p.wT, p.ldwT, FD, qs, qt, t);
+  __syncthreads();
+  const f32x4 gam = ld4(p.gamma + 4 * lane);
+  const f32x4 q4 = ld4(qs + 4 * lane);
+  f32x4 qth[H], yv[H];
+  float m[H], l[H];
+#pragma unroll
+  for (int h = 0; h < H; ++h) {
+    qth[h] = ld4(&qt[h][4 * lane]) * gam;
+    yv[h] = f32x4{0.f, 0.f, 0.f, 0.f};
+    m[h] = -1e30f;
+    l[h] = 0.f;
+  }
+  f32x4 od = {0.f, 0.f, 0.f, 0.f};
+  f32x4 xn = {0.f, 0.f, 0.f, 0.f};
+  float rn = 0.f;
+  if (hw < p.I && !(hw >= p.ded0 && hw < p.ded1)) {
+    xn = ld4(p.x + (row0 + hw) * p.ldx + 4 * lane);
+    rn = p.rstd[row0 + hw];
+  }
+  for (int j = hw; j < p.I; j += NHW) {
+    const int64_t r = row0 + j;
+    const f32x4 xc = xn;
+    const float rc = rn;
+    const int jn = j + NHW;
+    if (jn < p.I && !(jn >= p.ded0 && jn < p.ded1)) {
+      xn = ld4(p.x + (row0 + jn) * p.ldx + 4 * lane);
+      rn = p.rstd[row0 + jn];
+    }
+    if (j >= p.ded0 && j < p.ded1) {
+      const f32x4 kv = ld4(p.qkv + r * p.ldqkv + FD + 4 * lane);
+      const f32x4 vv = ld4(p.qkv + r * p.ldqkv + 2 * FD + 4 * lane);
+      const float dt = dot4(kv, q4);
+#pragma unroll
+      for (int h = 0; h < H; ++h) {
+        const float s = half_sum(myh == h ? dt : 0.f) * p.scale;
+        const float mn = fmaxf(m[h], s);
+        const float corr = __expf(m[h] - mn), pe = __expf(s - mn);
+        l[h] = l[h] * corr + pe;
+        m[h] = mn;
+        yv[h] = yv[h] * corr;
+        if (myh == h) od = od * corr + vv * pe;
+      }
+    } else {
+      const f32x4 xv = xc * rc;
+#pragma unroll
+      for (int h = 0; h < H; ++h) {
+        const float s = half_sum(dot4(xv, qth[h])) * p.scale;
+        const float mn = fmaxf(m[h], s);
+        const float corr = __expf(m[h] - mn), pe = __expf(s - mn);
+        l[h] = l[h] * corr + pe;
+        m[h] = mn;
+        yv[h] = yv[h] * corr + xv * pe;
+        if (myh == h) od = od * corr;
+      }
+    }
+  }
+#pragma unroll
+  for (int h = 0; h < H; ++h) {
+    st4(&ry[hw][h][4 * lane], yv[h]);
+    if (lane == 0) { rm[hw][h] = m[h]; rl[hw][h] = l[h]; }
+  }
+  st4(&ro[hw][4 * lane], od);
+  __syncthreads();
+  for (int idx = t; idx < H * FD; idx += 256) {
+    const int h = idx / FD, k = idx % FD;
+    float M = rm[0][h];
+#pragma unroll
+    for (int w = 1; w < NHW; ++w) M = fmaxf(M, rm[w][h]);
+    float L = 0.f, a = 0.f;
+#pragma unroll
+    for (int w = 0; w < NHW; ++w) {
+      const float e = __expf(rm[w][h] - M);
+      L += rl[w][h] * e;
+      a += ry[w][h][k] * e;
+    }
+    a /= L;
+    p.y[((int64_t)b * H + h) * FD + k] = a;
+    gy[h][k] = a * p.gamma[k];
+    if (k == 0) p.lse[(int64_t)b * H + h] = M + __logf(L);
+  }
+  __syncthreads();
+  head_matvec<H>(p.w, p.ldw, 2 * FD, gy, po, t);
+  __syncthreads();
+  if (t < FD) {
+    const int h = t / HD;
+    float M = rm[0][h];
+#pragma unroll
+    for (int w = 1; w < NHW; ++w) M = fmaxf(M, rm[w][h]);
+    float L = 0.f, a = 0.f;
+#pragma unroll
+    for (int w = 0; w < NHW; ++w) {
+      const float e = __expf(rm[w][h] - M);
+      L += rl[w][h] * e;
+      a += ro[w][t] * e;
+    }
+    p.o[(int64_t)b * FD + t] = (po[0][t] + po[1][t]) + a / L;
+  }
+}
+
+template <int H>
+__global__ __launch_bounds__(256) void attn_fold_bwd_kernel(FoldArgs p) {
+  constexpr int HD = FD / H, LPH = 32 / H;
+  __shared__ __attribute__((aligned(16))) float qs[FD];
+  __shared__ __attribute__((aligned(16))) float dos[FD];
+  __shared__ __attribute__((aligned(16))) float ab[2][H][FD];
+  __shared__ __attribute__((aligned(16))) float rz[NHW][H][FD];
+  __shared__ __attribute__((aligned(16))) float rq[NHW][FD];
+  __shared__ float gz[H][FD];
+  __shared__ float po[2][FD];
+  const int b = blockIdx.x, t = threadIdx.x, hw = t >> 5, lane = t & 31, myh = lane / LPH;
+  const int64_t row0 = (int64_t)b * p.I;
+  if (t < FD) {
+    qs[t] = p.qkv[(row0 + p.I - 1) * p.ldqkv + t];
+    dos[t] = p.dout[(int64_t)b * FD + t];
+  }
+  __syncthreads();
+  head_matvec_T<H>(p.wT, p.ldwT, FD, qs, ab[0], t);
+  head_matvec_T<H>(p.wT, p.ldwT, 2 * FD, dos, ab[1], t);
+  __syncthreads();
+  const f32x4 gam = ld4(p.gamma + 4 * lane);
+  const f32x4 q4 = ld4(qs + 4 * lane), do4 = ld4(dos + 4 * lane);
+  f32x4 qth[H], ch[H], zv[H];
+  float lse[H], delta[H];
+  const float od = dot4(ld4(p.o + (int64_t)b * FD + 4 * lane), do4);
+#pragma unroll
+  for (int h = 0; h < H; ++h) {
+    qth[h] = ld4(&ab[0][h][4 * lane]) * gam;
+    ch[h] = ld4(&ab[1][h][4 * lane]) * gam;
+    zv[h] = f32x4{0.f, 0.f, 0.f, 0.f};
+    lse[h] = p.lse[(int64_t)b * H + h];
+    delta[h] = half_sum(myh == h ? od : 0.f);
+  }
+  f32x4 dqd = {0.f, 0.f, 0.f, 0.f};
+  const f32x4 zero4 = {0.f, 0.f, 0.f, 0.f};
+  const bool q_ded = p.I - 1 >= p.ded0 && p.I - 1 < p.ded1;
+  f32x4 xn = zero4;
+  float rn = 0.f;
+  if (hw < p.I && !(hw >= p.ded0 && hw < p.ded1)) {
+    xn = ld4(p.x + (row0 + hw) * p.ldx + 4 * lane);
+    rn = p.rstd[row0 + hw];
+  }
+  for (int j = hw; j < p.I; j += NHW) {
+    const int64_t r = row0 + j;
+    const bool isq = j == p.I - 1;
+    const f32x4 xc = xn;
+    const float rc = rn;
+    const int jn = j + NHW;
+    if (jn < p.I && !(jn >= p.ded0 && jn < p.ded1)) {
+      xn = ld4(p.x + (row0 + jn) * p.ldx + 4 * lane);
+      rn = p.rstd[row0 + jn];
+    }
+    const f32x4 res = (isq && p.dx1) ? ld4(p.dx1 + (int64_t)b * FD + 4 * lane) : zero4;
+    if (j >= p.ded0 && j < p.ded1) {
+      const f32x4 kv = ld4(p.qkv + r * p.ldqkv + FD + 4 * lane);
+      const f32x4 vv = ld4(p.qkv + r * p.ldqkv + 2 * FD + 4 * lane);
+      const float dt = dot4(kv, q4), dtv = dot4(vv, do4);
+      float dsm = 0.f, pm = 0.f;
+#pragma unroll
+      for (int h = 0; h < H; ++h) {
+        const float s = half_sum(myh == h ? dt : 0.f) * p.scale;
+        const float pr = __expf(s - lse[h]);
+        const float dp = half_sum(myh == h ? dtv : 0.f);
+        const float ds = pr * (dp - delta[h]) * p.scale;
+        if (myh == h) { dsm = ds; pm = pr; }
+      }
+      dqd = dqd + kv * dsm;
+      float* crow = p.dqkv + ((int64_t)b * p.nf + (j - p.ded0)) * p.lddqkv + 4 * lane;
+      if (!isq) st4(crow, zero4);
+      st4(crow + FD, q4 * dsm);
+      st4(crow + 2 * FD, do4 * pm);
+      st4(p.dx + r * p.lddx + 4 * lane, res);
+    } else {
+      const float rs = rc;
+      const f32x4 xv = xc * rs;
+      f32x4 g = zero4;
+#pragma unroll
+      for (int h = 0; h < H; ++h) {
+        const float s = half_sum(dot4(xv, qth[h])) * p.scale;
+        const float pr = __expf(s - lse[h]);
+        const float dp = half_sum(dot4(xv, ch[h]));
+        const float ds = pr * (dp - delta[h]) * p.scale;
+        zv[h] = zv[h] + xv * ds;
+        g = g + qth[h] * ds + ch[h] * pr;
+      }
+      const float gx = half_sum(dot4(g, xv)) * (1.f / FD);
+      st4(p.dx + r * p.lddx + 4 * lane, (g - xv * gx) * rs + res);
+    }
+  }
+#pragma unroll
+  for (int h = 0; h < H; ++h) st4(&rz[hw][h][4 * lane], zv[h]);
+  st4(&rq[hw][4 * lane], dqd);
+  __syncthreads();
+  for (int idx = t; idx < H * FD; idx += 256) {
+    const int h = idx / FD, k = idx % FD;
+    float a = 0.f;
+#pragma unroll
+    for (int w = 0; w < NHW; ++w) a += rz[w][h][k];
+    p.z[((int64_t)b * H + h) * FD + k] = a;
+    gz[h][k] = a * p.gamma[k];
+    rz[0][h][k] = a;
+  }
+  __syncthreads();
+  head_matvec<H>(p.w, p.ldw, FD, gz, po, t);
+  if (t < FD) {
+    float a = 0.f;
+#pragma unroll
+    for (int h = 0; h < H; ++h)
+      a += rz[0][h][t] * ab[0][h][t] + p.y[((int64_t)b * H + h) * FD + t] * ab[1][h][t];
+    p.dgpart[(int64_t)b * FD + t] = a;
+  }
+  __syncthreads();
+  if (t < FD) {
+    float a = 0.f;
+#pragma unroll
+    for (int w = 0; w < NHW; ++w) a += rq[w][t];
+    float* crow = p.dqkv + ((int64_t)b * p.nf + (q_ded ? p.I - 1 - p.ded0 : p.ded1 - p.ded0)) * p.lddqkv;
+    crow[t] = (po[0][t] + po[1][t]) + a;
+    if (!q_ded) { crow[FD + t] = 0.f; crow[2 * FD + t] = 0.f; }
+  }
+}
+
+template <int H>
+__global__ __launch_bounds__(256) void attn_fold_dw_kernel(const float* z, const float* y, const float* qkv,
+                                                           int64_t ldqkv, const float* dout, int B, int I,
+                                                           float* part) {
+  constexpr int HD = FD / H, HPH = 64 / HD;
+  __shared__ __attribute__((aligned(16))) float dsm[DW_ROWS][FD];
+  const int t = threadIdx.x, kv = blockIdx.y, b0 = blockIdx.x * DW_ROWS;
+  const int nb = min(DW_ROWS, B - b0);
+  const float* A = kv ? y : z;
+  for (int idx = t; idx < nb * FD; idx += 256) {
+    const int64_t bb = b0 + idx / FD;
+    const int n = idx % FD;
+    dsm[idx / FD][n] = kv ? dout[bb * FD + n] : qkv[(bb * I + I - 1) * ldqkv + n];
+  }
+  __syncthreads();
+  const int k = t & (FD - 1), half = t >> 7;
+  float acc[64];
+#pragma unroll
+  for (int c = 0; c < 64; ++c) acc[c] = 0.f;
+#pragma unroll 2
+  for (int bb = 0; bb < nb; ++bb) {
+#pragma unroll
+    for (int hh = 0; hh < HPH; ++hh) {
+      const int h = half * HPH + hh;
+      const float a = A[((int64_t)(b0 + bb) * H + h) * FD + k];
+#pragma unroll
+      for (int c = 0; c < HD; c += 4) {
+        const f32x4 dv = ld4(&dsm[bb][h * HD + c]);
+        acc[hh * HD + c + 0] = fmaf(a, dv.x, acc[hh * HD + c + 0]);
+        acc[hh * HD + c + 1] = fmaf(a, dv.y, acc[hh * HD + c + 1]);
+        acc[hh * HD + c + 2] = fmaf(a, dv.z, acc[hh * HD + c + 2]);
+        acc[hh * HD + c + 3] = fmaf(a, dv.w, acc[hh * HD + c + 3]);
+      }
+    }
+  }
+  float* out = part + (((int64_t)blockIdx.x * 2 + kv) * FD + k) * FD + half * 64;
+#pragma unroll
+  for (int c = 0; c < 64; c += 4) st4(out + c, f32x4{acc[c], acc[c + 1], acc[c + 2], acc[c + 3]});
+}
+
+__global__ __launch_bounds__(256) void attn_fold_dw_reduce_kernel(const float* part, int nchunk, const float* gamma,
+                                                                  float* dW, int64_t lddw, int accumulate) {
+  const int idx = blockIdx.x * 256 + threadIdx.x;
+  const int kv = idx / (FD * FD), k = (idx / FD) % FD, n = idx % FD;
+  float a = 0.f;
+#pragma unroll 8
+  for (int c = 0; c < nchunk; ++c) a += part[((int64_t)c * 2 + kv) * FD * FD + k * FD + n];
+  a *= gamma[k];
+  float* dst = dW + (int64_t)k * lddw + FD + kv * FD + n;
+  *dst = accumulate ? *dst + a : a;
+}
+
+static int last_fold_initial() {
+  const char* e = getenv("ONETRANS_LAST_FOLD");
+  return e && *e ? (atoi(e) != 0) : 1;
+}
+static std::atomic<int> g_last_fold{last_fold_initial()};
+
+static bool a16(const void* p) { return (reinterpret_cast<uintptr_t>(p) & 15) == 0; }
+
+static int check_common(const char* fn, const float* x, int64_t ldx, const float* rstd, const float* gamma,
+                        const float* w, int64_t ldw, const float* wT, int64_t ldwT, const float* qkv, int64_t ldqkv,
+                        int B, int H, int I, int head_dim, int ded0, int ded1) {
+  OT_REQUIRE(x && rstd && gamma && w && wT && qkv, "%s: null operand", fn);
+  OT_REQUIRE(B >= 0 && I >= 1 && (int64_t)B * I < (int64_t)1 << 31, "%s: bad B / I", fn);
+  if (!ot_attn_fold_supported(H * head_dim, H))
+    return fail(OT_ERR_UNSUPPORTED, "%s: width %d with %d heads is not built (128 with 2 or 4 heads)", fn,
+                H * head_dim, H);
+  OT_REQUIRE(0 <= ded0 && ded0 <= ded1 && ded1 <= I, "%s: dedicated range [%d, %d) outside [0, %d]", fn, ded0, ded1,
+             I);
+  OT_REQUIRE(ldx >= FD && ldx % 4 == 0 && ldqkv >= 3 * FD && ldqkv % 4 == 0 && ldw >= 3 * FD && ldwT >= FD,
+             "%s: leading dimensions", fn);
+  OT_REQUIRE(a16(x) && a16(gamma) && a16(qkv), "%s: x, gamma and qkv must be 16-byte aligned", fn);
+  return OT_OK;
+}
+
+}
+}
+
+using namespace ot;
+using namespace ot::fold;
+
+extern "C" int ot_last_fold(int on) {
+  const int old = g_last_fold.load(std::memory_order_relaxed);
+  if (on >= 0) g_last_fold.store(on ? 1 : 0, std::memory_order_relaxed);
+  return old;
+}
+
+extern "C" int ot_attn_fold_supported(int d, int H) { return d == FD && (H == 2 || H == 4); }
+
+extern "C" int ot_attn_fold_fwd(const float* x, int64_t ldx, const float* rstd, const float* gamma, const float* w,
+                                int64_t ldw, const float* wT, int64_t ldwT, const float* qkv, int64_t ldqkv, int B,
+                                int H, int I, int head_dim, int ded0, int ded1, float* o, float* lse, float* y,
+                                void* stream) {
+  OT_TRY(check_common("ot_attn_fold_fwd", x, ldx, rstd, gamma, w, ldw, wT, ldwT, qkv, ldqkv, B, H, I, head_dim, ded0,
+                      ded1));
+  OT_REQUIRE(o && lse && y, "ot_attn_fold_fwd: null output");
+  if (B == 0) return OT_OK;
+  FoldArgs p{};
+  p.x = x; p.ldx = ldx; p.rstd = rstd; p.gamma = gamma; p.w = w; p.ldw = ldw; p.wT = wT; p.ldwT = ldwT;
+  p.qkv = qkv; p.ldqkv = ldqkv; p.B = B; p.I = I; p.ded0 = ded0; p.ded1 = ded1;
+  p.scale = 1.0f / sqrtf((float)head_dim);
+  p.o = o; p.lse = lse; p.y = y;
+  if (H == 2) hipLaunchKernelGGL(attn_fold_fwd_kernel<2>, dim3(B), dim3(256), 0, (hipStream_t)stream, p);
+  else hipLaunchKernelGGL(attn_fold_fwd_kernel<4>, dim3(B), dim3(256), 0, (hipStream_t)stream, p);
+  OT_LAUNCH_CHECK("ot_attn_fold_fwd");
+  return OT_OK;
+}
+
+extern "C" int ot_attn_fold_bwd(const float* x, int64_t ldx, const float* rstd, const float* gamma, const float* w,
+                                int64_t ldw, const float* wT, int64_t ldwT, const float* qkv, int64_t ldqkv, int B,
+                                int H, int I, int head_dim, int ded0, int ded1, const float* o, const float* dout,
+                                const float* lse, const float* y, const float* dx1, float* dx, int64_t lddx,
+                                float* dqkv, int64_t lddqkv, float* z, float* dgpart, void* stream) {
+  OT_TRY(check_common("ot_attn_fold_bwd", x, ldx, rstd, gamma, w, ldw, wT, ldwT, qkv, ldqkv, B, H, I, head_dim, ded0,
+                      ded1));
+  OT_REQUIRE(o && dout && lse && y && dx && dqkv && z && dgpart, "ot_attn_fold_bwd: null operand");
+  OT_REQUIRE(lddx >= FD && lddx % 4 == 0 && lddqkv >= 3 * FD && lddqkv % 4 == 0, "ot_attn_fold_bwd: leading dimensions");
+  OT_REQUIRE(a16(o) && a16(dx) && a16(dqkv) && (!dx1 || a16(dx1)),
+             "ot_attn_fold_bwd: o, dx, dqkv and dx1 must be 16-byte aligned");
+  if (B == 0) return OT_OK;
+  FoldArgs p{};
+  p.x = x; p.ldx = ldx; p.rstd = rstd; p.gamma = gamma; p.w = w; p.ldw = ldw; p.wT = wT; p.ldwT = ldwT;
+  p.qkv = qkv; p.ldqkv = ldqkv; p.B = B; p.I = I; p.ded0 = ded0; p.ded1 = ded1;
+  p.scale = 1.0f / sqrtf((float)head_dim);
+  p.o = const_cast<float*>(o); p.lse = const_cast<float*>(lse); p.y = const_cast<float*>(y);
+  p.dout = dout; p.dx1 = dx1; p.dx = dx; p.lddx = lddx; p.dqkv = dqkv; p.lddqkv = lddqkv;
+  p.nf = ot_attn_fold_rows(I, ded0, ded1);
+  p.z = z; p.dgpart = dgpart;
+  if (H == 2) hipLaunchKernelGGL(attn_fold_bwd_kernel<2>, dim3(B), dim3(256), 0, (hipStream_t)stream, p);
+  else hipLaunchKernelGGL(attn_fold_bwd_kernel<4>, dim3(B), dim3(256), 0, (hipStream_t)stream, p);
+  OT_LAUNCH_CHECK("ot_attn_fold_bwd");
+  return OT_OK;
+}
+
+extern "C" int ot_attn_fold_rows(int I, int ded0, int ded1) {
+  return (ded1 - ded0) + ((I - 1 >= ded0 && I - 1 < ded1) ? 0 : 1);
+}
+
+extern "C" size_t ot_attn_fold_workspace_size(int B, int d) {
+  const int64_t nchunk = ceil_div(B, DW_ROWS);
+  const int64_t dw = nchunk * 2 * d * d, dg = colsum_scratch_floats(B, d);
+  return (size_t)(dw > dg ? dw : dg) * sizeof(float);
+}
+
+extern "C" int ot_attn_fold_dw(const float* z, const float* y, const float* qkv, int64_t ldqkv, const float* dout,
+                               const float* gamma, int B, int H, int I, int head_dim, float* dW, int64_t lddw,
+                               int accumulate, void* workspace, size_t ws_bytes, void* stream) {
+  OT_REQUIRE(z && y && qkv && dout && gamma && dW, "ot_attn_fold_dw: null operand");
+  if (!ot_attn_fold_supported(H * head_dim, H))
+    return fail(OT_ERR_UNSUPPORTED, "ot_attn_fold_dw: width %d with %d heads is not built", H * head_dim, H);
+  OT_REQUIRE(B >= 0 && I >= 1 && ldqkv >= 3 * FD && lddw >= 3 * FD, "ot_attn_fold_dw: bad sizes");
+  OT_REQUIRE(workspace && ws_bytes >= ot_attn_fold_workspace_size(B, FD) && a16(workspace),
+             "ot_attn_fold_dw: workspace too small");
+  const unsigned nchunk = ceil_div(B, DW_ROWS);
+  float* part = (float*)workspace;
+  if (nchunk > 0) {
+    if (H == 2)
+      hipLaunchKernelGGL(attn_fold_dw_kernel<2>, dim3(nchunk, 2), dim3(256), 0, (hipStream_t)stream, z, y, qkv, ldqkv,
+                         dout, B, I, part);
+    else
+      hipLaunchKernelGGL(attn_fold_dw_kernel<4>, dim3(nchunk, 2), dim3(256), 0, (hipStream_t)stream, z, y, qkv, ldqkv,
+                         dout, B, I, part);
+    OT_LAUNCH_CHECK("ot_attn_fold_dw");
+  }
+  hipLaunchKernelGGL(attn_fold_dw_reduce_kernel, dim3(2 * FD * FD / 256), dim3(256), 0, (hipStream_t)stream, part,
+                     (int)nchunk, gamma, dW, lddw, accumulate);
+  OT_LAUNCH_CHECK("ot_attn_fold_dw(reduce)");
+  return OT_OK;
+}
+
+extern "C" int ot_attn_fold_dgamma(const float* dgpart, int B, int d, float* dgamma, int accumulate, void* workspace,
+                                   size_t ws_bytes, void* stream) {
+  OT_REQUIRE(dgpart && dgamma && B >= 0 && d > 0, "ot_attn_fold_dgamma: bad args");
+  OT_REQUIRE(workspace && ws_bytes >= ot_attn_fold_workspace_size(B, d), "ot_attn_fold_dgamma: workspace too small");
+  launch_colsum_reduce(dgpart, B, d, dgamma, accumulate, (hipStream_t)stream, (float*)workspace);
+  OT_LAUNCH_CHECK("ot_attn_fold_dgamma");
+  return OT_OK;
+}
diff --git a/recommend_amd/kernels.py b/recommend_amd/kernels.py
--- a/recommend_amd/kernels.py
+++ b/recommend_amd/kernels.py
@@ -395,6 +395,61 @@
         _probe.end('attention', 8.0 * (K * I - K * (K - 1) / 2) * hd * H * B, ev, f'bwd I{I} K{K} hd{hd}')
 
 
+def last_fold(on: int = -1) -> int:
+    return _lib.size('ot_last_fold', int(on))
+
+
+def attn_fold_supported(d: int, H: int) -> bool:
+    return bool(_lib.size('ot_attn_fold_supported', int(d), int(H)))
+
+
+def attn_fold_rows(I: int, ded0: int, ded1: int) -> int:
+    return _lib.size('ot_attn_fold_rows', int(I), int(ded0), int(ded1))
+
+
+def _fold_common(x, ldx, rstd, gamma, w, ldw, wT, ldwT, qkv, ldqkv, B, H, I, hd, ded):
+    return (ptr(x), ldx, ptr(rstd), ptr(gamma), ptr(w), ldw, ptr(wT), ldwT, ptr(qkv), ldqkv, B, H, I, hd, ded[0],
+            ded[1])
+
+
+def attn_fold_fwd(x, ldx, rstd, gamma, w, ldw, wT, ldwT, qkv, ldqkv, B, H, I, hd, ded, o, lse, y) -> None:
+    ev = _probe.begin() if _probe is not None else None
+    call('ot_attn_fold_fwd', *_fold_common(x, ldx, rstd, gamma, w, ldw, wT, ldwT, qkv, ldqkv, B, H, I, hd, ded),
+         ptr(o), ptr(lse), ptr(y), stream())
+    if ev is not None:
+        d = H * hd
+        _probe.end('attention', 4.0 * I * d * H * B, ev, f'fold_fwd I{I} hd{hd}', 4.0 * B * I * (d + 1))
+
+
+def attn_fold_bwd(x, ldx, rstd, gamma, w, ldw, wT, ldwT, qkv, ldqkv, B, H, I, hd, ded, o, dout, lse, y, dx1, dx, lddx,
+                  dqkv, lddqkv, z, dgpart) -> None:
+    ev = _probe.begin() if _probe is not None else None
+    call('ot_attn_fold_bwd', *_fold_common(x, ldx, rstd, gamma, w, ldw, wT, ldwT, qkv, ldqkv, B, H, I, hd, ded),
+         ptr(o), ptr(dout), ptr(lse), ptr(y), ptr(dx1), ptr(dx), lddx, ptr(dqkv), lddqkv, ptr(z), ptr(dgpart),
+         stream())
+    if ev is not None:
+        d = H * hd
+        _probe.end('attention', 10.0 * I * d * H * B, ev, f'fold_bwd I{I} hd{hd}', 8.0 * B * I * (d + 1))
+
+
+def attn_fold_dw(z, y, qkv, ldqkv, dout, gamma, B, H, I, hd, dW, lddw, accumulate: bool = False) -> None:
+    ws = workspace(size('ot_attn_fold_workspace_size', B, H * hd), z.device)
+    ev = _probe.begin() if _probe is not None else None
+    call('ot_attn_fold_dw', ptr(z), ptr(y), ptr(qkv), ldqkv, ptr(dout), ptr(gamma), B, H, I, hd, ptr(dW), lddw,
+         int(accumulate), ptr(ws), ws.numel(), stream())
+    if ev is not None:
+        d = H * hd
+        _probe.end('attention', 4.0 * B * d * d, ev, f'fold_dw B{B}', 8.0 * B * d * (H + 1))
+
+
+def attn_fold_dgamma(dgpart, B, d, dgamma, accumulate: bool = False) -> None:
+    ws = workspace(size('ot_attn_fold_workspace_size', B, d), dgpart.device)
+    ev = _probe.begin() if _probe is not None else None
+    call('ot_attn_fold_dgamma', ptr(dgpart), B, d, ptr(dgamma), int(accumulate), ptr(ws), ws.numel(), stream())
+    if ev is not None:
+        _probe.end('attention', 0.0, ev, f'fold_dgamma B{B}', 4.0 * B * d)
+
+
 def _valid_arg(valid):
     t, off, ldv = valid
     if t.dtype != torch.uint8:
diff --git a/recommend_amd/layout.py b/recommend_amd/layout.py
--- a/recommend_amd/layout.py
+++ b/recommend_amd/layout.py
@@ -209,7 +209,27 @@
         tpos = pos[pos >= I - K]
         tail_pg.append([rows_for(tpos, lambda bb, pp: bb * I + pp),
                         rows_for(tpos, lambda bb, pp: bb * K + (pp - (I - K)))])
-    return {'all': build_map(all_pg), 'tail': build_map(tail_pg)}
+    maps = {'all': build_map(all_pg), 'tail': build_map(tail_pg)}
+    if K == 1 and p0 == 0 and I_full == I:
+        maps['fold'] = build_map(fold_rows(grp, B, I, G))
+    return maps
+
+
+def fold_positions(grp: np.ndarray, I: int) -> np.ndarray:
+    return np.union1d(np.nonzero(grp != 0)[0], [I - 1])
+
+
+def fold_rows(grp: np.ndarray, B: int, I: int, G: int):
+    fpos = fold_positions(grp, I)
+    nf = len(fpos)
+    b = np.arange(B)
+    per_group = []
+    for g in range(G):
+        idx = np.nonzero(grp[fpos] == g)[0]
+        tok = (b[:, None] * I + fpos[idx][None, :]).reshape(-1)
+        cmp_ = (b[:, None] * nf + idx[None, :]).reshape(-1)
+        per_group.append([tok, cmp_])
+    return per_group
 
 
 def head_map(B: int, T: int) -> RowMap:
diff --git a/recommend_amd/model.py b/recommend_amd/model.py
--- a/recommend_amd/model.py
+++ b/recommend_amd/model.py
@@ -213,6 +213,8 @@
              and m.bimg(f'blk.{l}.wqkv') is not None)
     xn1 = torch.empty(B * I, d, dtype=torch.int16, device=dev) if xn_on else None
     x1n = torch.empty(B * Kq, d, dtype=torch.int16, device=dev) if xn_on else None
+    fold = m.fold_gate(I, Kq, select, kvalid)
+    yf = None
     if xn1 is not None:
         full = Kq == I
         K.gemm_rms(OT_GEMM_NT, xa, d, d, ma['rows'][0], wqkv if full else (wqkv, d * d), 3 * d * d, d,
@@ -229,8 +231,9 @@
                3 * d, ma['rows'][0], a_xform=ax1, rstd=rstd1, gamma=g1, m_rows=maps['all'].nrows,
                bimg=m.bimg(f'blk.{l}.wqkv'))
     else:
-        K.gemm(OT_GEMM_NT, xa, d, d, ma['rows'][0], (wqkv, d * d), 3 * d * d, d, 2 * d, ma['tile_group'], na,
-               (qkv, d), 3 * d, ma['rows'][0], a_xform=ax1, rstd=rstd1, gamma=g1, m_rows=maps['all'].nrows,
+        mkv, kvm = (maps['fold'].to(dev), maps['fold']) if fold is not None else (ma, maps['all'])
+        K.gemm(OT_GEMM_NT, xa, d, d, mkv['rows'][0], (wqkv, d * d), 3 * d * d, d, 2 * d, mkv['tile_group'],
+               kvm.ntiles, (qkv, d), 3 * d, mkv['rows'][0], a_xform=ax1, rstd=rstd1, gamma=g1, m_rows=kvm.nrows,
                bimg=m.bimg(f'blk.{l}.wqkv', tn0=d // TILE) if d % TILE == 0 else None)
         K.gemm(OT_GEMM_NT, xa, d, d, qrows, wqkv, 3 * d * d, d, d, mt['tile_group'], nt, qkv,
                3 * d, qrows, a_xform=ax1, rstd=rstd1, gamma=g1, m_rows=maps['tail'].nrows,
@@ -242,9 +245,13 @@
              if m.attn_fp8 and training and K.attn_bwd_bf16_supported(I, Kq, hd, qp_f) else None)
     out = (lambda name: bounds.out(l, name)) if bounds is not None else (lambda name: None)
     pwo_f = m.gemm_pair(f'blk.{l}.wo', 'fwd')
-    o_rep = kvalid is None and not m.attn_fp8 and K.attn_amax_supported(I, Kq, hd, qp_f)
+    o_rep = kvalid is None and not m.attn_fp8 and fold is None and K.attn_amax_supported(I, Kq, hd, qp_f)
     rm_o = torch.empty(B * Kq, H, device=dev) if pwo_f and o_rep else None
-    if kvalid is not None:
+    if fold is not None:
+        yf = torch.empty(B * H, d, device=dev)
+        K.attn_fold_fwd(x, d, rstd1, g1, m.p(f'blk.{l}.wqkv'), 3 * d, wqkv, d, qkv, 3 * d, B, H, I, hd, fold, o, lse,
+                        yf)
+    elif kvalid is not None:
         K.attn_fwd_masked(qkv, 3 * d, B, H, I, Kq, hd, o, lse, _layer_valid(kvalid, I), qpos=qp_f)
     else:
         K.attn_fwd(qkv, 3 * d, B, H, I, Kq, hd, o, lse, qpos=qp_f, fp8=m.attn_fp8, dequant=m.attn_fp8 and training,
@@ -286,7 +293,7 @@
                         m.layout.images[(f'blk.{l}.w2', 'fwd')][1], b1, f, b2, d, f, x2, d, u_out=u, ldu=f,
                         u_amax=out('u'), rstd_out=rstd_out, eps=RMS_EPS, seed=seed, site=2 * l + 1, drop=rate,
                         tail=tail, m_rows=maps['tail'].nrows)
-        saved = (x, rstd1, qkv, o, lse, x1, rstd2, u, None, xn1, None)
+        saved = (x, rstd1, qkv, o, lse, x1, rstd2, u, None, xn1, None, yf)
         return x2, rstd_out, saved, pos, inv, rate
     umax = torch.empty(B * Kq, f // TILE, device=dev) if pair_w2 else None
     if h is not None:
@@ -310,7 +317,7 @@
                bimg=m.bimg(f'blk.{l}.w1'))
     if x1n is not None and h is None:
         x1n = None
-    saved = (x, rstd1, qkv, o, lse, x1, rstd2, u, h, xn1, x1n)
+    saved = (x, rstd1, qkv, o, lse, x1, rstd2, u, h, xn1, x1n, yf)
     if not need_out:
         return None, None, saved, pos, inv, rate
     x2 = torch.empty(B * Kq, d, device=dev)
@@ -372,9 +379,9 @@
             training, select = ctx.fwd_args
             _, _, saved, pos, inv, _ = _block_forward(m, l, xin, I, Kq, seed, training, rstd_in, select,
                                                       need_out=False, bounds=bounds, kvalid=kvalid)
-            x, rstd1, qkv, o, lse, x1, rstd2, u, h, xn1, x1n = saved
+            x, rstd1, qkv, o, lse, x1, rstd2, u, h, xn1, x1n, yf = saved
         else:
-            x, rstd1, qkv, o, lse, x1, rstd2, u, h, xn1, x1n = ctx.saved_tensors
+            x, rstd1, qkv, o, lse, x1, rstd2, u, h, xn1, x1n, yf = ctx.saved_tensors
         tail = (Kq, I, pos)
         cfg = m.config
         d, f, H = cfg.hidden_dim, cfg.ffn_dim, cfg.num_heads
@@ -474,6 +481,12 @@
         K.gemm_rms(OT_GEMM_NT, dyo, d, d, mt['rows'][1], m.p(f'blk.{l}.wo'), 0, d, d, mt['tile_group'], nt, do, d,
                    mt['rows'][1], epi=0, m_rows=maps['tail'].nrows, device=dev, bimg=m.bimg(f'blk.{l}.wo', 'dgrad'),
                    **a_row_bounds(pwo, dyo, d, B * Kq, d, rm_dyo))
+        if yf is not None:
+            dx = _fold_backward(m, l, x, rstd1, qkv, o, lse, yf, do, dx1, B, I, maps['fold'], acc, dev)
+            m.side_block_done()
+            if m.grad_ready is not None:
+                m.grad_ready(l)
+            return None, dx, None, None, None, None, None, None, None, None, None, None
         qp = _attn_qpos(cfg, pos)
         dq_bf = (K.matmul_mode() == 'bf16'
                  and K.attn_bwd_bf16_forms(I, Kq, hd, qp) & _lib.OT_ATTN_DQKV_BF16
@@ -519,6 +532,34 @@
         if m.grad_ready is not None:
             m.grad_ready(l)
         return None, dx, None, None, None, None, None, None, None, None, None, None
+
+
+def _fold_backward(m, l, x, rstd1, qkv, o, lse, yf, do, dx1, B, I, fmap, acc, dev):
+    cfg = m.config
+    d, H, G = cfg.hidden_dim, cfg.num_heads, cfg.num_groups
+    hd = d // H
+    ded = m.fold_ded(I)
+    mf = fmap.to(dev)
+    nf = K.attn_fold_rows(I, *ded)
+    g1, w = m.p(f'blk.{l}.norm1'), m.p(f'blk.{l}.wqkv')
+    dqkv = torch.empty(B * nf, 3 * d, device=dev)
+    dx = torch.empty(B * I, d, device=dev)
+    zf = torch.empty(B * H, d, device=dev)
+    dgp = torch.empty(B, d, device=dev)
+    K.attn_fold_bwd(x, d, rstd1, g1, w, 3 * d, m.pT(f'blk.{l}.wqkv'), d, qkv, 3 * d, B, H, I, hd, ded, o, do, lse, yf,
+                    dx1, dx, d, dqkv, 3 * d, zf, dgp)
+    pa_q = a_row_bounds(m.dgrad_pair(f'blk.{l}.wqkv'), dqkv, 3 * d, B * nf, 3 * d)
+    K.gemm_rms(OT_GEMM_NT, dqkv, 3 * d, 3 * d, mf['rows'][1], w, 3 * d * d, 3 * d, d, mf['tile_group'], fmap.ntiles,
+               dx, d, mf['rows'][0], epi=OT_EPI_RMSNORM_BWD, m_rows=fmap.nrows, nx=x, ldnx=d, ngamma=g1, nrstd=rstd1,
+               dres=dx, lddres=d, dgamma=m.g(f'blk.{l}.norm1'), accumulate_dgamma=acc, device=dev,
+               bimg=m.bimg(f'blk.{l}.wqkv', 'dgrad'), **pa_q)
+    K.attn_fold_dgamma(dgp, B, d, m.g(f'blk.{l}.norm1'), accumulate=True)
+    with m.side(x, dqkv, rstd1, zf, yf, qkv, do):
+        K.wgrad(x, d, mf['rows'][0], dqkv, 3 * d, mf['rows'][1], d, 3 * d, mf, fmap.chunks.shape[0], G,
+                m.g(f'blk.{l}.wqkv'), 3 * d * d, None, 0, a_xform=OT_AX_RMSNORM, rstd=rstd1, gamma=g1, accumulate=acc,
+                device=dev, m_rows=fmap.nrows, rowmap=fmap)
+        K.attn_fold_dw(zf, yf, qkv, 3 * d, do, g1, B, H, I, hd, m.g(f'blk.{l}.wqkv'), 3 * d, accumulate=True)
+    return dx
 
 
 def _wgrad_single(m, A, D, K_, N, mt, dW, acc, dev, mrows=0, rowmap=None, a_bound=None, d_bound=None):
@@ -893,6 +934,22 @@
         if key not in self._maps:
             self._maps[key] = layer_maps(self.config, B, I, Kq, p0=p0, I_full=I_full)
         return self._maps[key]
+
+    def fold_ded(self, I: int):
+        key = ('fold', I)
+        if key not in self._aux_maps:
+            ded = [p for p in range(I) if self.config.group_of_position(p, I) != 0]
+            run = (ded[0], ded[-1] + 1) if ded else (0, 0)
+            self._aux_maps[key] = run if ded == list(range(*run)) else None
+        return self._aux_maps[key]
+
+    def fold_gate(self, I: int, Kq: int, select: bool, kvalid):
+        cfg = self.config
+        if (Kq != 1 or I < 2 or select or kvalid is not None or self.attn_fp8 or not self.fuse_bwd
+                or K.matmul_mode() not in ('split', 'f32') or not K.last_fold()
+                or not K.attn_fold_supported(cfg.hidden_dim, cfg.num_heads)):
+            return None
+        return self.fold_ded(I)
 
     def head_rows(self, B):
         key = ('head', B)
```

New measurement: 208,000 samples/s (median of 6 runs). 1.04x the previous value.
